# JiLiBIT/LIO-SLAM

Hardware: AMD Instinct MI355X
Metric: scan-to-map registrations/sec, 64x1800 scan vs 200-keyframe map; pose RMSE (higher is better)
Workload: dtype f32

## Files before the change

### include/liogpu.h

```cpp
#ifndef LIOGPU_H
#define LIOGPU_H

#include <stddef.h>
#include <stdint.h>

#ifdef __cplusplus
extern "C" {
#endif

#define LIO_VERSION 102
#define LIO_MAX_ITERS 32

enum {
    LIO_OK               = 0,
    LIO_TOO_FEW_POINTS   = 1,
    LIO_TOO_FEW_CORR     = 2,
    LIO_ERR_ARG          = -1,
    LIO_ERR_HIP          = -2,
    LIO_ERR_CAPACITY     = -3,
    LIO_ERR_NO_MAP       = -4,
    LIO_ERR_NO_DEVICE    = -5
};

typedef struct lio_s2m_config {
    int32_t k;
    float   max_sq_dist;
    double  plane_tol;
    double  weight;
    double  min_s;
    int32_t min_corr;
    int32_t max_iters;
    float   eig_thresh;
    double  conv_deg;
    double  conv_cm;
    int32_t min_scan_pts;
    int32_t jacobian_mode;
    int32_t force_all_iters;
    int32_t device_id;
    float   cell_size;
    int32_t max_batch;
    int32_t max_scan_pts;
    int32_t record_corr_iter;
    int32_t kernel_variant;
    int32_t profile;
    int32_t lookahead;
    int32_t use_lds;
    int32_t sort_scan;
    int32_t cell_div;
    int32_t xcd_remap;
    float   tile_size;
    int32_t use_graph;
    int32_t graph_iters;
    int32_t sort_batch;
    int32_t nn_cache;
    int32_t pipeline;
    int32_t n_devices;
    int32_t device_ids[8];
    int32_t x_sub;
    int32_t tight_rows;
} lio_s2m_config;

typedef struct lio_s2m_result {
    int32_t status;
    int32_t iters;
    int32_t converged;
    int32_t is_degenerate;
    int32_t n_corr_last;
    int32_t n_corr_iter[LIO_MAX_ITERS];
    float   matP[36];
    float   AtA[36];
    float   AtB[6];
    float   pose_iter[LIO_MAX_ITERS][6];
} lio_s2m_result;

typedef struct lio_s2m_profile {
    float   map_build_ms;
    float   map_upload_ms;
    int32_t n_launches;
    int32_t n_units;
    int32_t unit_iters;
    float   launch_ms[LIO_MAX_ITERS];
    int32_t launch_active[LIO_MAX_ITERS];
    int64_t point_iters;
    int64_t n_map;
    int64_t n_cells;
    int32_t pipeline;
    int32_t multi_iterations;
    int32_t multi_stream_syncs;
    int32_t multi_event_waits;
    int32_t multi_exchange;
    int32_t persist_fallbacks;
    int32_t map_x_sub;
    int32_t map_tight_tables;
    int32_t map_first_try;
    float   map_pts_per_cell;
} lio_s2m_profile;

typedef struct lio_s2m_handle lio_s2m_handle;

int  lio_version(void);
void lio_s2m_default_config(lio_s2m_config *cfg);
const char *lio_last_error(void);

int  lio_s2m_create(const lio_s2m_config *cfg, lio_s2m_handle **out);
void lio_s2m_destroy(lio_s2m_handle *h);

int  lio_s2m_set_map(lio_s2m_handle *h, const void *pts, size_t n, size_t stride_bytes);

int  lio_s2m_register(lio_s2m_handle *h, const void *scan, size_t n, size_t stride_bytes,
                      float pose[6], lio_s2m_result *res);

int  lio_s2m_batch_upload(lio_s2m_handle *h, int32_t n_scans, const void *const *scans,
                          const size_t *n_pts, size_t stride_bytes);
int  lio_s2m_batch_set_poses(lio_s2m_handle *h, const float *poses );
int  lio_s2m_batch_run(lio_s2m_handle *h);
int  lio_s2m_batch_sync(lio_s2m_handle *h);
int  lio_s2m_batch_results(lio_s2m_handle *h, float *poses ,
                           lio_s2m_result *results );

int   lio_s2m_share_map(lio_s2m_handle *h, lio_s2m_handle *map_owner);
int   lio_s2m_batch_upload_async(lio_s2m_handle *h, int32_t n_scans, const void *const *scans,
                                 const size_t *n_pts, size_t stride_bytes);
void *lio_host_alloc(size_t bytes);
void  lio_host_free(void *p);
int   lio_host_register(void *p, size_t bytes);
int   lio_host_unregister(void *p);
void *lio_device_alloc(int32_t device_id, size_t bytes);
void  lio_device_free(int32_t device_id, void *p);
int   lio_device_upload(int32_t device_id, void *dst, const void *src, size_t bytes);

int  lio_s2m_set_degeneracy(lio_s2m_handle *h, int32_t scan, const float matP[36], int32_t is_degenerate);

int  lio_s2m_get_correspondences(lio_s2m_handle *h, int32_t scan, uint8_t *flag,
                                 float *coeff4, int32_t *nn_idx5);

int  lio_s2m_set_corner_map(lio_s2m_handle *h, const void *pts, size_t n, size_t stride_bytes);
int  lio_s2m_batch_upload_corners(lio_s2m_handle *h, int32_t n_scans, const void *const *scans,
                                  const size_t *n_pts, size_t stride_bytes);
int  lio_s2m_register_cs(lio_s2m_handle *h, const void *corner_scan, size_t n_corner,
                         const void *surf_scan, size_t n_surf, size_t stride_bytes,
                         float pose[6], lio_s2m_result *res);
int  lio_s2m_get_corner_correspondences(lio_s2m_handle *h, int32_t scan, uint8_t *flag,
                                        float *coeff4, int32_t *nn_idx5);

int  lio_s2m_get_profile(lio_s2m_handle *h, lio_s2m_profile *out);
int  lio_s2m_kernel_variant(const lio_s2m_handle *h);
int  lio_s2m_launch_forms(const lio_s2m_handle *h, int32_t *n_full, int32_t *n_looped);
int  lio_s2m_debug_persist_spin(lio_s2m_handle *h, int32_t spin_max, int32_t withhold_wg);

int  lio_debug_plane_fit(int32_t device_id, const float *sets, size_t n, double plane_tol, uint32_t *out);
int  lio_debug_fast_f32_ops(int32_t device_id, int32_t op, int32_t raw, const uint32_t *patterns, uint64_t first, uint64_t count,
                            uint32_t *values, uint64_t *n_diff, uint32_t *first_diff, int32_t *n_first);
float lio_debug_threshold_f32(double t);
int  lio_s2m_debug_stamps(lio_s2m_handle *h, long long *out, size_t cap_entries);

int  lio_s2m_set_stream(lio_s2m_handle *h, void *hip_stream);
int  lio_s2m_set_global_grid(lio_s2m_handle *h, const float origin[3], const int32_t dims[3]);
int  lio_s2m_set_shard(lio_s2m_handle *h, int32_t axis, int32_t lo, int32_t hi);
int  lio_s2m_set_shard_plan(lio_s2m_handle *h, int32_t axis, int32_t n_ranks, int32_t rank, const int32_t *bounds,
                            int32_t halo_cells);
int  lio_s2m_set_scan_shard(lio_s2m_handle *h, int32_t rank, int32_t world);
int  lio_s2m_batch_begin(lio_s2m_handle *h);
int  lio_s2m_batch_iter_partial(lio_s2m_handle *h, double *d_sums );
int  lio_s2m_batch_iter_apply(lio_s2m_handle *h, const double *d_sums);
int  lio_s2m_batch_n_active(lio_s2m_handle *h, int32_t *n_active);
int  lio_s2m_batch_poll_active(lio_s2m_handle *h, int32_t iteration, int32_t *n_active);

void lio_transform_update(float pose[6], int32_t imu_available, int32_t imu_type,
                          float imu_roll_init, float imu_pitch_init, float imu_rpy_weight,
                          float rotation_tollerance, float z_tollerance);

typedef struct lio_deskew_config {
    int32_t N_SCAN;
    int32_t downsampleRate;
    int32_t point_filter_num;
    float   lidarMinFront, lidarMinBack, lidarMinLeft, lidarMinRight;
    float   lidarMaxRange;
    float   lidarMaxIntensity;
    int32_t deskew_flag;
    int32_t device_id;
} lio_deskew_config;

void lio_deskew_default_config(lio_deskew_config *cfg);

int  lio_imu_deskew_info(const double *stamp, const double *gyro_x, const double *gyro_y,
                         const double *gyro_z, int32_t n_imu,
                         double time_scan_cur, double time_scan_end,
                         double *imuTime, double *imuRotX, double *imuRotY, double *imuRotZ);

int  lio_deskew(const lio_deskew_config *cfg, const void *pts, size_t n, size_t stride_bytes,
                double time_scan_cur,
                const double *imuTime, const double *imuRotX, const double *imuRotY,
                const double *imuRotZ, int32_t imuPointerCur,
                void *out, size_t out_stride_bytes, size_t *n_out);

enum { LIO_PC2_UINT8 = 2, LIO_PC2_UINT16 = 4, LIO_PC2_INT32 = 5 };
enum { LIO_PC2_TIME_F32_SECONDS = 0,
       LIO_PC2_TIME_U32_NS      = 1,
       LIO_PC2_TIME_U32_RAW     = 2,
       LIO_PC2_TIME_F64_STAMP   = 3 };
typedef struct lio_pc2_layout {
    uint32_t point_step;
    uint32_t off_x;
    int32_t  off_intensity;
    int32_t  off_ring;
    int32_t  ring_type;
    int32_t  off_time;
    int32_t  time_type;
    int32_t  pin_host;
} lio_pc2_layout;

int  lio_s2m_register_pc2(lio_s2m_handle *h, const void *data, size_t n_points, const lio_pc2_layout *layout,
                          float pose[6], lio_s2m_result *res);
int  lio_s2m_register_raw(lio_s2m_handle *h, const void *data, size_t n_points, const lio_pc2_layout *layout, float leaf,
                          float pose[6], lio_s2m_result *res, void *ds_out, size_t ds_out_stride, size_t *n_ds);
int  lio_deskew_pc2(const lio_deskew_config *cfg, const void *data, size_t n_points, const lio_pc2_layout *layout,
                    double time_scan_cur,
                    const double *imuTime, const double *imuRotX, const double *imuRotY,
                    const double *imuRotZ, int32_t imuPointerCur,
                    void *out, size_t out_stride_bytes, size_t *n_out);

typedef struct lio_range_image_config {
    int32_t N_SCAN, Horizon_SCAN, downsampleRate;
    float   lidarMinRange, lidarMaxRange;
    int32_t deskew_flag;
    int32_t device_id;
} lio_range_image_config;
void lio_range_image_default_config(lio_range_image_config *cfg);
int  lio_range_image(const lio_range_image_config *cfg, const void *pts, size_t n, size_t stride_bytes,
                     double time_scan_cur,
                     const double *imuTime, const double *imuRotX, const double *imuRotY,
                     const double *imuRotZ, int32_t imuPointerCur,
                     void *out, size_t out_stride_bytes, size_t *n_out,
                     int32_t *startRingIndex, int32_t *endRingIndex,
                     int32_t *pointColInd, float *pointRange);

int  lio_curvature(int32_t device_id, const float *range, size_t n, float *curvature,
                   int32_t *neighbor_picked, int32_t *label);

typedef struct lio_feature_config {
    int32_t N_SCAN;
    float   edgeThreshold;
    float   surfThreshold;
    float   surfLeafSize;
    int32_t device_id;
} lio_feature_config;
void lio_feature_default_config(lio_feature_config *cfg);
int  lio_extract_features(const lio_feature_config *cfg, const void *cloud, size_t n, size_t stride_bytes,
                          const int32_t *startRingIndex, const int32_t *endRingIndex,
                          const int32_t *pointColInd, const float *pointRange,
                          void *corner_out, size_t *n_corner, void *surface_out, size_t *n_surface,
                          size_t out_stride_bytes, float *curvature, int32_t *neighbor_picked, int32_t *label);

int  lio_voxel_grid(int32_t device_id, const void *pts, size_t n, size_t stride_bytes, float leaf,
                    void *out, size_t out_stride_bytes, size_t *n_out);

int  lio_assemble_map(lio_s2m_handle *h, int32_t device_id, int32_t n_keyframes, const void *const *clouds,
                      const size_t *n_pts, size_t stride_bytes, const float *poses, float leaf,
                      void *out, size_t out_stride_bytes, size_t *n_out);

typedef struct lio_kf_store lio_kf_store;
int  lio_kf_store_create(int32_t device_id, lio_kf_store **out);
void lio_kf_store_destroy(lio_kf_store *s);
int  lio_kf_store_add(lio_kf_store *s, const void *cloud, size_t n, size_t stride_bytes, int32_t *id_out);
int  lio_kf_store_count(const lio_kf_store *s);
size_t lio_kf_store_points(const lio_kf_store *s, int32_t id);
int  lio_kf_store_add_device(lio_kf_store *s, const void *d_cloud, size_t n, size_t stride_bytes, int32_t *id_out);
int  lio_kf_store_add_from_handle(lio_kf_store *s, lio_s2m_handle *h, int32_t scan, int32_t *id_out);
int  lio_assemble_map_resident(lio_s2m_handle *h, lio_kf_store *s, int32_t n_selected, const int32_t *ids,
                               const float *poses, float leaf, void *out, size_t out_stride_bytes, size_t *n_out);

typedef struct lio_nearby_config {
    float  search_radius;
    float  pose_density;
    double recent_window_s;
} lio_nearby_config;
void lio_nearby_default_config(lio_nearby_config *cfg);

int  lio_kf_store_set_poses(lio_kf_store *s, int32_t first, int32_t n, const float *poses, const double *times);

int  lio_assemble_map_nearby(lio_s2m_handle *h, lio_kf_store *s, const lio_nearby_config *cfg, double time_cur, float leaf,
                             int32_t *ids_out, int32_t ids_cap, int32_t *n_ids, void *out, size_t out_stride_bytes,
                             size_t out_cap, size_t *n_out);

#define LIO_ICP_MAX_ITERS 1000
enum {
    LIO_ICP_NOT_CONVERGED      = 0,
    LIO_ICP_ITERATIONS         = 1,
    LIO_ICP_TRANSFORM          = 2,
    LIO_ICP_ABS_MSE            = 3,
    LIO_ICP_REL_MSE            = 4,
    LIO_ICP_NO_CORRESPONDENCES = 5
};
typedef struct lio_icp_config {
    double  max_corr_dist;
    double  transform_eps;
    double  fitness_eps;
    double  rel_mse_eps;
    double  rotation_threshold;
    double  fitness_max;
// ... 262 lines not shown
```

### lio-slam_amd/api.py

```python
import ctypes as C
import os
import subprocess

import numpy as np

_HERE = os.path.dirname(os.path.abspath(__file__))
LIO_MAX_ITERS = 32
STATUS_NAMES = {0: "OK", 1: "TOO_FEW_POINTS", 2: "TOO_FEW_CORR", -1: "ERR_ARG", -2: "ERR_HIP",
                -3: "ERR_CAPACITY", -4: "ERR_NO_MAP", -5: "ERR_NO_DEVICE"}


class LioError(RuntimeError):
    pass


class S2MConfig(C.Structure):
    _fields_ = [
        ("k", C.c_int32), ("max_sq_dist", C.c_float),
        ("plane_tol", C.c_double), ("weight", C.c_double), ("min_s", C.c_double),
        ("min_corr", C.c_int32), ("max_iters", C.c_int32), ("eig_thresh", C.c_float),
        ("conv_deg", C.c_double), ("conv_cm", C.c_double),
        ("min_scan_pts", C.c_int32), ("jacobian_mode", C.c_int32), ("force_all_iters", C.c_int32),
        ("device_id", C.c_int32), ("cell_size", C.c_float), ("max_batch", C.c_int32),
        ("max_scan_pts", C.c_int32), ("record_corr_iter", C.c_int32), ("kernel_variant", C.c_int32),
# ... 70 lines not shown

class IcpResult(C.Structure):
    _fields_ = [("status", C.c_int32), ("converged", C.c_int32), ("state", C.c_int32), ("iters", C.c_int32),
                ("n_corr_last", C.c_int32), ("accepted", C.c_int32), ("n_source", C.c_int32), ("n_target", C.c_int32),
                ("n_launches", C.c_int32), ("pad", C.c_int32), ("fitness", C.c_double), ("T", C.c_float * 16),
                ("pose_corrected", C.c_float * 6)]


class IcpClouds(C.Structure):
    _fields_ = [("source", C.c_void_p), ("target", C.c_void_p), ("closed", C.c_void_p),
                ("cap_source", C.c_size_t), ("cap_target", C.c_size_t), ("cap_closed", C.c_size_t),
                ("n_source", C.c_size_t), ("n_target", C.c_size_t), ("n_closed", C.c_size_t), ("stride", C.c_size_t)]


SC_MAX_CANDIDATES = 16


class ScConfig(C.Structure):
    _fields_ = [("max_radius", C.c_double), ("lidar_height", C.c_double), ("search_ratio", C.c_double), ("dist_thres", C.c_double),
                ("num_rings", C.c_int32), ("num_sectors", C.c_int32), ("num_exclude_recent", C.c_int32),
                ("num_candidates", C.c_int32), ("tree_period", C.c_int32), ("pad", C.c_int32)]


class ScResult(C.Structure):
    _fields_ = [("status", C.c_int32), ("loop_id", C.c_int32), ("align", C.c_int32), ("nn_idx", C.c_int32),
                ("n_searched", C.c_int32), ("n_candidates", C.c_int32), ("yaw_diff_rad", C.c_float), ("pad", C.c_int32),
                ("min_dist", C.c_double), ("cand_idx", C.c_int32 * SC_MAX_CANDIDATES), ("cand_ring_d2", C.c_float * SC_MAX_CANDIDATES),
                ("cand_dist", C.c_double * SC_MAX_CANDIDATES), ("cand_align", C.c_int32 * SC_MAX_CANDIDATES)]


class LocalMapConfig(C.Structure):
    _fields_ = [("n_keyframes", C.c_int32), ("front", C.c_float), ("left", C.c_float), ("back", C.c_float), ("right", C.c_float),
                ("remove_outliers", C.c_int32), ("mean_k", C.c_int32), ("stddev_mul", C.c_float), ("downsample", C.c_int32),
                ("leaf", C.c_float)]


class LocalMapInfo(C.Structure):
    _fields_ = [("first_keyframe", C.c_int32), ("n_keyframes", C.c_int32), ("n_summed", C.c_int32), ("n_cropped", C.c_int32),
                ("n_inliers", C.c_int32), ("n_out", C.c_int32), ("voxel_passthrough", C.c_int32), ("pad", C.c_int32),
                ("sor_mean", C.c_double), ("sor_stddev", C.c_double), ("sor_threshold", C.c_double)]


class HeightMapConfig(C.Structure):
    _fields_ = [("roll", C.c_float), ("pitch", C.c_float), ("level_and_ego_filter", C.c_int32), ("remove_outliers", C.c_int32),
                ("mean_k", C.c_int32), ("stddev_mul", C.c_float), ("downsample", C.c_int32), ("voxel", C.c_float * 3),
                ("resolution", C.c_double), ("min_points_per_cell", C.c_int32), ("max_points_per_cell", C.c_int32),
                ("use_cluster", C.c_int32), ("cluster_tolerance", C.c_float), ("cluster_min_points", C.c_int32),
                ("cluster_max_points", C.c_int32), ("use_max_height", C.c_int32), ("fill_holes", C.c_int32)]


class HeightMapInfo(C.Structure):
    _fields_ = [("rows", C.c_int32), ("cols", C.c_int32), ("length", C.c_double * 2), ("position", C.c_double * 2),
                ("n_in", C.c_int32), ("n_inliers", C.c_int32), ("n_filtered", C.c_int32), ("n_binned", C.c_int32),
                ("n_valid_cells", C.c_int32), ("n_filled_cells", C.c_int32), ("voxel_passthrough", C.c_int32), ("pad", C.c_int32)]


TERRAIN_LAYERS = ("smooth", "normal_x", "normal_y", "normal_z", "slope", "roughness", "edges", "traversability")


class TerrainConfig(C.Structure):
    _fields_ = [("normal_method", C.c_int32), ("normal_axis", C.c_int32), ("normal_radius", C.c_double), ("smooth_radius", C.c_double),
                ("edge_window_size", C.c_int32), ("edge_window_length", C.c_double), ("slope_critical", C.c_float),
                ("roughness_critical", C.c_float), ("slope_weight", C.c_float), ("roughness_weight", C.c_float), ("layers", C.c_uint32)]


class TerrainInfo(C.Structure):
    _fields_ = [("rows", C.c_int32), ("cols", C.c_int32), ("n_valid_cells", C.c_int32), ("normal_method_used", C.c_int32),
                ("n_normal_cells", C.c_int32), ("n_few_points", C.c_int32), ("n_degenerate", C.c_int32), ("edge_window_size", C.c_int32)]


class GlobalMapConfig(C.Structure):
    _fields_ = [("search_radius", C.c_float), ("pose_density", C.c_float), ("leaf", C.c_float)]


class GlobalMapInfo(C.Structure):
    _fields_ = [("n_keyframes", C.c_int32), ("n_summed", C.c_int32), ("n_out", C.c_int32), ("voxel_passthrough", C.c_int32)]


class ExportConfig(C.Structure):
    _fields_ = [("resolution", C.c_float), ("chunk_points", C.c_int32)]


class OgmConfig(C.Structure):
    _fields_ = [("z_min", C.c_float), ("z_max", C.c_float), ("z_negative", C.c_int32), ("remove_outliers", C.c_int32),
                ("radius", C.c_float), ("min_neighbors", C.c_int32), ("resolution", C.c_double), ("whole_box", C.c_int32)]


class OgmInfo(C.Structure):
    _fields_ = [("width", C.c_int32), ("height", C.c_int32), ("origin", C.c_double * 2), ("n_in", C.c_int32), ("n_slice", C.c_int32),
                ("n_inliers", C.c_int32), ("n_binned", C.c_int32), ("n_occupied", C.c_int32), ("pad", C.c_int32)]


class SdfConfig(C.Structure):
    _fields_ = [("min_height", C.c_double), ("max_height", C.c_double), ("nan_policy", C.c_int32), ("pad", C.c_int32)]


class SdfInfo(C.Structure):
    _fields_ = [("rows", C.c_int32), ("cols", C.c_int32), ("layers", C.c_int32), ("n_nan", C.c_int32), ("origin", C.c_double * 3),
                ("resolution", C.c_double), ("layer_min", C.c_float), ("layer_max", C.c_float), ("n_all_obstacle", C.c_int32),
                ("n_all_free", C.c_int32), ("n_mixed", C.c_int32), ("pad", C.c_int32)]


SDF_NODE_LIMIT = 1 << 25
STAGED_DS, STAGED_RAW = 0, 1

ICP_STATES = {0: "NOT_CONVERGED", 1: "ITERATIONS", 2: "TRANSFORM", 3: "ABS_MSE", 4: "REL_MSE", 5: "NO_CORRESPONDENCES"}


def lib_path():
    return os.environ.get("LIOGPU_LIB") or os.path.join(_HERE, "libliogpu.so")


def build_library(verbose=False):
    out = subprocess.run(["make", "-j8", "-C", os.path.join(_HERE, "csrc")], capture_output=True, text=True)
    if out.returncode != 0:
        raise LioError("building libliogpu.so failed:\n" + out.stdout + out.stderr)
    if verbose:
        print(out.stdout)
    return lib_path()


_LIB = None

EXPORTS = [
    "lio_version", "lio_s2m_default_config", "lio_last_error", "lio_s2m_create", "lio_s2m_destroy",
    "lio_s2m_set_map", "lio_s2m_register", "lio_s2m_batch_upload", "lio_s2m_batch_set_poses",
    "lio_s2m_batch_run", "lio_s2m_batch_sync", "lio_s2m_batch_results", "lio_s2m_set_degeneracy",
    "lio_s2m_get_correspondences", "lio_s2m_get_profile", "lio_s2m_set_stream",
    "lio_s2m_set_global_grid", "lio_s2m_set_shard", "lio_s2m_batch_begin",
    "lio_s2m_batch_iter_partial", "lio_s2m_batch_iter_apply", "lio_s2m_batch_n_active",
    "lio_transform_update", "lio_deskew_default_config", "lio_imu_deskew_info", "lio_deskew",
    "lio_curvature", "lio_s2m_debug_stamps", "lio_s2m_batch_poll_active", "lio_voxel_grid", "lio_assemble_map", "lio_kf_store_create", "lio_kf_store_destroy", "lio_kf_store_add",
    "lio_kf_store_count", "lio_kf_store_points", "lio_assemble_map_resident", "lio_s2m_set_scan_shard",
    "lio_s2m_set_corner_map", "lio_s2m_batch_upload_corners", "lio_s2m_register_cs",
    "lio_s2m_get_corner_correspondences", "lio_feature_default_config", "lio_extract_features",
    "lio_range_image_default_config", "lio_range_image",
    "lio_s2m_share_map", "lio_s2m_batch_upload_async", "lio_host_alloc", "lio_host_free", "lio_host_register",
    "lio_host_unregister", "lio_s2m_set_shard_plan", "lio_s2m_register_pc2", "lio_deskew_pc2", "lio_kf_store_add_device", "lio_kf_store_add_from_handle",
    "lio_s2m_register_raw", "lio_s2m_debug_persist_spin", "lio_device_alloc", "lio_device_free", "lio_device_upload",
    "lio_nearby_default_config", "lio_kf_store_set_poses", "lio_assemble_map_nearby", "lio_debug_plane_fit",
    "lio_icp_default_config", "lio_icp_align", "lio_kf_store_loop_icp", "lio_kf_store_detect_loop", "lio_icp_debug_trace",
    "lio_sc_default_config", "lio_sc_make", "lio_sc_distance", "lio_kf_store_sc_add", "lio_kf_store_sc_add_device",
    "lio_kf_store_sc_add_from_handle", "lio_kf_store_sc_count", "lio_kf_store_sc_geometry", "lio_kf_store_sc_get", "lio_kf_store_sc_detect",
    "lio_sor_filter", "lio_local_map_default_config", "lio_kf_store_local_map",
    "lio_height_map_default_config", "lio_height_map", "lio_kf_store_height_map",
    "lio_terrain_default_config", "lio_terrain_layers", "lio_kf_store_terrain_map",
    "lio_global_map_default_config", "lio_kf_store_global_map", "lio_kf_store_export_map", "lio_kf_store_get_keyframe",
    "lio_s2m_registered_cloud",
    "lio_radius_filter", "lio_ogm_default_config", "lio_occupancy_grid", "lio_kf_store_occupancy_grid", "lio_ogm_debug_stage_ms",
    "lio_s2m_kernel_variant", "lio_s2m_launch_forms",
    "lio_sdf_default_config", "lio_sdf_create", "lio_sdf_destroy", "lio_sdf_build", "lio_kf_store_sdf", "lio_sdf_nodes", "lio_sdf_query",
    "lio_occupancy_sdf", "lio_sdf_debug_stage_ms", "lio_sdf_memory",
    "lio_debug_fast_f32_ops", "lio_debug_threshold_f32",
]


def load_library():
    global _LIB
    if _LIB is not None:
        return _LIB
    p = lib_path()
    if not os.path.exists(p):
        raise LioError(f"{p} is missing: run __graft_entry__.build() (hipcc --offload-arch=gfx950). "
                       "There is no CPU fallback.")
    L = C.CDLL(p)
    vp, i32, f32, f64, sz = C.c_void_p, C.c_int32, C.c_float, C.c_double, C.c_size_t
    L.lio_version.restype = C.c_int
    L.lio_last_error.restype = C.c_char_p
    L.lio_s2m_default_config.argtypes = [C.POINTER(S2MConfig)]
    L.lio_s2m_default_config.restype = None
    L.lio_s2m_create.argtypes = [C.POINTER(S2MConfig), C.POINTER(vp)]
    L.lio_s2m_destroy.argtypes = [vp]
    L.lio_s2m_destroy.restype = None
    L.lio_s2m_set_map.argtypes = [vp, vp, sz, sz]
    L.lio_s2m_register.argtypes = [vp, vp, sz, sz, C.POINTER(f32), C.POINTER(S2MResult)]
    L.lio_s2m_register_pc2.argtypes = [vp, vp, sz, C.POINTER(PC2Layout), C.POINTER(f32), C.POINTER(S2MResult)]
    L.lio_s2m_register_raw.argtypes = [vp, vp, sz, C.POINTER(PC2Layout), f32, C.POINTER(f32), C.POINTER(S2MResult), vp, sz, C.POINTER(sz)]
    L.lio_s2m_debug_persist_spin.argtypes = [vp, i32, i32]
    L.lio_s2m_batch_upload.argtypes = [vp, i32, C.POINTER(vp), C.POINTER(sz), sz]
    L.lio_s2m_batch_upload_async.argtypes = [vp, i32, C.POINTER(vp), C.POINTER(sz), sz]
    L.lio_s2m_share_map.argtypes = [vp, vp]
    L.lio_host_alloc.argtypes = [sz]
    L.lio_host_alloc.restype = vp
    L.lio_host_free.argtypes = [vp]
    L.lio_host_free.restype = None
    L.lio_device_alloc.argtypes = [i32, sz]
    L.lio_device_alloc.restype = vp
    L.lio_device_free.argtypes = [i32, vp]
    L.lio_device_free.restype = None
    L.lio_device_upload.argtypes = [i32, vp, vp, sz]
    L.lio_host_register.argtypes = [vp, sz]
    L.lio_host_unregister.argtypes = [vp]
    L.lio_s2m_batch_set_poses.argtypes = [vp, C.POINTER(f32)]
    L.lio_s2m_batch_run.argtypes = [vp]
    L.lio_s2m_batch_sync.argtypes = [vp]
    L.lio_s2m_batch_results.argtypes = [vp, C.POINTER(f32), C.POINTER(S2MResult)]
    L.lio_s2m_set_degeneracy.argtypes = [vp, i32, C.POINTER(f32), i32]
    L.lio_s2m_get_correspondences.argtypes = [vp, i32, vp, vp, vp]
    L.lio_s2m_get_profile.argtypes = [vp, C.POINTER(S2MProfile)]
    L.lio_s2m_kernel_variant.argtypes = [vp]
    if hasattr(L, "lio_s2m_launch_forms"):
        L.lio_s2m_launch_forms.argtypes = [vp, C.POINTER(i32), C.POINTER(i32)]
    L.lio_s2m_set_corner_map.argtypes = [vp, vp, sz, sz]
    L.lio_s2m_batch_upload_corners.argtypes = [vp, i32, C.POINTER(vp), C.POINTER(sz), sz]
    L.lio_s2m_register_cs.argtypes = [vp, vp, sz, vp, sz, sz, C.POINTER(f32), C.POINTER(S2MResult)]
    L.lio_s2m_get_corner_correspondences.argtypes = [vp, i32, vp, vp, vp]
    L.lio_s2m_set_stream.argtypes = [vp, vp]
    L.lio_s2m_set_global_grid.argtypes = [vp, C.POINTER(f32), C.POINTER(i32)]
    L.lio_s2m_set_shard.argtypes = [vp, i32, i32, i32]
    L.lio_s2m_set_scan_shard.argtypes = [vp, i32, i32]
    L.lio_s2m_set_shard_plan.argtypes = [vp, i32, i32, i32, C.POINTER(i32), i32]
    L.lio_s2m_batch_begin.argtypes = [vp]
    L.lio_s2m_batch_iter_partial.argtypes = [vp, vp]
    L.lio_s2m_batch_iter_apply.argtypes = [vp, vp]
    L.lio_s2m_batch_n_active.argtypes = [vp, C.POINTER(i32)]
    L.lio_s2m_batch_poll_active.argtypes = [vp, i32, C.POINTER(i32)]
    L.lio_transform_update.argtypes = [C.POINTER(f32), i32, i32, f32, f32, f32, f32, f32]
    L.lio_transform_update.restype = None
    L.lio_deskew_default_config.argtypes = [C.POINTER(DeskewConfig)]
    L.lio_deskew_default_config.restype = None
    dp = C.POINTER(f64)
    L.lio_imu_deskew_info.argtypes = [dp, dp, dp, dp, i32, f64, f64, dp, dp, dp, dp]
    L.lio_deskew.argtypes = [C.POINTER(DeskewConfig), vp, sz, sz, f64, dp, dp, dp, dp, i32, vp, sz,
                             C.POINTER(sz)]
    L.lio_deskew_pc2.argtypes = [C.POINTER(DeskewConfig), vp, sz, C.POINTER(PC2Layout), f64, dp, dp, dp, dp, i32, vp, sz,
                                 C.POINTER(sz)]
    L.lio_curvature.argtypes = [i32, vp, sz, vp, vp, vp]
    L.lio_range_image_default_config.argtypes = [C.POINTER(RangeImageConfig)]
    L.lio_range_image_default_config.restype = None
    L.lio_range_image.argtypes = [C.POINTER(RangeImageConfig), vp, sz, sz, f64, dp, dp, dp, dp, i32, vp, sz, C.POINTER(sz),
                                  vp, vp, vp, vp]
    L.lio_feature_default_config.argtypes = [C.POINTER(FeatureConfig)]
    L.lio_feature_default_config.restype = None
    L.lio_extract_features.argtypes = [C.POINTER(FeatureConfig), vp, sz, sz, vp, vp, vp, vp, vp, C.POINTER(sz), vp,
                                       C.POINTER(sz), sz, vp, vp, vp]
    L.lio_s2m_debug_stamps.argtypes = [vp, vp, sz]
    L.lio_voxel_grid.argtypes = [i32, vp, sz, sz, f32, vp, sz, C.POINTER(sz)]
    L.lio_kf_store_create.argtypes = [i32, C.POINTER(vp)]
    L.lio_kf_store_destroy.argtypes = [vp]
    L.lio_kf_store_destroy.restype = None
    L.lio_kf_store_add.argtypes = [vp, vp, sz, sz, C.POINTER(i32)]
    L.lio_kf_store_count.argtypes = [vp]
    L.lio_kf_store_points.argtypes = [vp, C.c_int32]
    L.lio_kf_store_points.restype = C.c_size_t
    L.lio_kf_store_add_device.argtypes = [vp, vp, sz, sz, C.POINTER(i32)]
    L.lio_kf_store_add_from_handle.argtypes = [vp, vp, i32, C.POINTER(i32)]
    L.lio_assemble_map_resident.argtypes = [vp, vp, i32, C.POINTER(i32), C.POINTER(f32), f32, vp, sz, C.POINTER(sz)]
    L.lio_assemble_map.argtypes = [vp, i32, i32, C.POINTER(vp), C.POINTER(sz), sz, C.POINTER(f32), f32, vp, sz,
                                   C.POINTER(sz)]
    L.lio_nearby_default_config.argtypes = [C.POINTER(NearbyConfig)]
    L.lio_nearby_default_config.restype = None
    L.lio_kf_store_set_poses.argtypes = [vp, i32, i32, C.POINTER(f32), C.POINTER(f64)]
    L.lio_assemble_map_nearby.argtypes = [vp, vp, C.POINTER(NearbyConfig), f64, f32, C.POINTER(i32), i32, C.POINTER(i32), vp, sz, sz,
                                          C.POINTER(sz)]
    L.lio_icp_default_config.argtypes = [C.POINTER(IcpConfig)]
    L.lio_icp_default_config.restype = None
    L.lio_icp_align.argtypes = [i32, vp, sz, sz, vp, sz, sz, C.POINTER(IcpConfig), C.POINTER(f32), C.POINTER(IcpResult)]
    L.lio_kf_store_loop_icp.argtypes = [vp, i32, i32, i32, i32, f32, C.POINTER(IcpConfig), C.POINTER(IcpResult), C.POINTER(IcpClouds)]
    L.lio_kf_store_detect_loop.argtypes = [vp, f32, f64, f64, C.POINTER(i32), C.POINTER(i32)]
    L.lio_icp_debug_trace.argtypes = [i32, vp, sz, sz, vp, sz, sz, C.POINTER(IcpConfig), C.POINTER(f32), i32, C.POINTER(IcpResult),
                                      vp, vp, vp, vp, C.POINTER(i32)]
    scp = C.POINTER(ScConfig)
    L.lio_sc_default_config.argtypes = [scp]
    L.lio_sc_default_config.restype = None
    L.lio_sc_make.argtypes = [i32, vp, sz, sz, scp, vp, vp, vp]
    L.lio_sc_distance.argtypes = [i32, vp, vp, scp, C.POINTER(f64), C.POINTER(i32)]
    L.lio_kf_store_sc_add.argtypes = [vp, vp, sz, sz, scp, C.POINTER(i32)]
    L.lio_kf_store_sc_add_device.argtypes = [vp, vp, sz, sz, scp, C.POINTER(i32)]
    L.lio_kf_store_sc_add_from_handle.argtypes = [vp, vp, scp, C.POINTER(i32)]
    L.lio_kf_store_sc_count.argtypes = [vp]
    L.lio_kf_store_sc_geometry.argtypes = [vp, C.POINTER(i32), C.POINTER(i32)]
    L.lio_kf_store_sc_get.argtypes = [vp, i32, vp, vp, vp]
    L.lio_kf_store_sc_detect.argtypes = [vp, scp, C.POINTER(ScResult)]
    L.lio_sor_filter.argtypes = [i32, vp, sz, sz, i32, f32, vp, sz, C.POINTER(sz), vp, C.POINTER(f64)]
    L.lio_local_map_default_config.argtypes = [C.POINTER(LocalMapConfig)]
    L.lio_local_map_default_config.restype = None
    L.lio_kf_store_local_map.argtypes = [vp, C.POINTER(LocalMapConfig), C.POINTER(f32), vp, sz, sz, C.POINTER(sz), C.POINTER(LocalMapInfo)]
    L.lio_height_map_default_config.argtypes = [C.POINTER(HeightMapConfig)]
    L.lio_height_map_default_config.restype = None
    L.lio_height_map.argtypes = [i32, vp, sz, sz, C.POINTER(HeightMapConfig), vp, sz, C.POINTER(HeightMapInfo)]
    L.lio_kf_store_height_map.argtypes = [vp, C.POINTER(LocalMapConfig), C.POINTER(f32), C.POINTER(HeightMapConfig), vp, sz,
                                          C.POINTER(LocalMapInfo), C.POINTER(HeightMapInfo)]
    L.lio_terrain_default_config.argtypes = [C.POINTER(TerrainConfig)]
    L.lio_terrain_default_config.restype = None
    L.lio_terrain_layers.argtypes = [i32, vp, i32, i32, f64, C.POINTER(f64), C.POINTER(f64), C.POINTER(TerrainConfig), vp, sz,
                                     C.POINTER(TerrainInfo)]
    L.lio_kf_store_terrain_map.argtypes = [vp, C.POINTER(LocalMapConfig), C.POINTER(f32), C.POINTER(HeightMapConfig), C.POINTER(TerrainConfig),
                                           vp, sz, vp, sz, C.POINTER(LocalMapInfo), C.POINTER(HeightMapInfo), C.POINTER(TerrainInfo)]
    L.lio_global_map_default_config.argtypes = [C.POINTER(GlobalMapConfig)]
    L.lio_global_map_default_config.restype = None
    L.lio_kf_store_global_map.argtypes = [vp, C.POINTER(GlobalMapConfig), C.POINTER(i32), i32, C.POINTER(i32), vp, sz, sz, C.POINTER(sz),
                                          C.POINTER(GlobalMapInfo)]
    L.lio_kf_store_export_map.argtypes = [vp, C.POINTER(ExportConfig), vp, sz, sz, C.POINTER(sz), vp, sz, sz, C.POINTER(sz), C.POINTER(i32)]
    L.lio_kf_store_get_keyframe.argtypes = [vp, i32, C.POINTER(f32), vp, sz, sz, C.POINTER(sz)]
    L.lio_s2m_registered_cloud.argtypes = [vp, i32, C.POINTER(f32), vp, sz, sz, C.POINTER(sz)]
    L.lio_radius_filter.argtypes = [i32, vp, sz, sz, f32, i32, vp, sz, C.POINTER(sz), vp]
    L.lio_ogm_default_config.argtypes = [C.POINTER(OgmConfig)]
    L.lio_ogm_default_config.restype = None
    L.lio_occupancy_grid.argtypes = [i32, vp, sz, sz, C.POINTER(OgmConfig), vp, sz, C.POINTER(OgmInfo)]
    L.lio_kf_store_occupancy_grid.argtypes = [vp, f32, C.POINTER(OgmConfig), vp, sz, C.POINTER(sz), C.POINTER(OgmInfo)]
    L.lio_ogm_debug_stage_ms.argtypes = [i32, C.POINTER(f32)]
    L.lio_sdf_default_config.argtypes = [C.POINTER(SdfConfig)]
    L.lio_sdf_default_config.restype = None
    L.lio_sdf_create.argtypes = [i32, C.POINTER(vp)]
    L.lio_sdf_destroy.argtypes = [vp]
    L.lio_sdf_destroy.restype = None
    L.lio_sdf_build.argtypes = [vp, vp, i32, i32, f64, C.POINTER(f64), C.POINTER(f64), C.POINTER(SdfConfig), C.POINTER(SdfInfo)]
    L.lio_kf_store_sdf.argtypes = [vp, C.POINTER(LocalMapConfig), C.POINTER(f32), C.POINTER(HeightMapConfig), C.POINTER(SdfConfig), vp, sz, vp,
                                   C.POINTER(LocalMapInfo), C.POINTER(HeightMapInfo), C.POINTER(SdfInfo)]
    L.lio_sdf_nodes.argtypes = [vp, vp, sz]
    L.lio_sdf_query.argtypes = [vp, vp, sz, vp, vp]
    L.lio_occupancy_sdf.argtypes = [i32, vp, i32, i32, f32, i32, vp]
    L.lio_sdf_debug_stage_ms.argtypes = [i32, C.POINTER(f32)]
    L.lio_sdf_memory.argtypes = [vp, C.POINTER(sz), C.POINTER(sz)]
    _LIB = L
    return L


def _check(rc, what):
    if rc < 0:
        msg = load_library().lio_last_error()
        raise LioError(f"{what} failed: {STATUS_NAMES.get(rc, rc)}: {msg.decode() if msg else ''}")
    return rc


def _f32p(a):
    return a.ctypes.data_as(C.POINTER(C.c_float))


def _as_points(a):
    a = np.ascontiguousarray(a, np.float32)
    if a.ndim != 2 or a.shape[1] < 3:
        raise ValueError("points must be [n, >=3] float32")
    return a, a.shape[1] * 4


class ScanToMap:

    def __init__(self, **cfg_overrides):
        self.lib = load_library()
        self.cfg = S2MConfig()
        self.lib.lio_s2m_default_config(C.byref(self.cfg))
        for k, v in cfg_overrides.items():
            if not hasattr(self.cfg, k):
                raise AttributeError(k)
            if k == "device_ids":
                for i, d in enumerate(v):
                    self.cfg.device_ids[i] = int(d)
                continue
            setattr(self.cfg, k, v)
        self.h = C.c_void_p()
        _check(self.lib.lio_s2m_create(C.byref(self.cfg), C.byref(self.h)), "lio_s2m_create")
        self._n_scans = 0
        self._npts = []

# ... 11 lines not shown
    def set_map(self, map_pts):
        a, stride = _as_points(map_pts)
        _check(self.lib.lio_s2m_set_map(self.h, a.ctypes.data, len(a), stride), "lio_s2m_set_map")

    def scan2MapOptimization(self, scan_pts, pose):
        a, stride = _as_points(scan_pts)
        p = np.array(pose, np.float32).copy()
        res = S2MResult()
        rc = _check(self.lib.lio_s2m_register(self.h, a.ctypes.data, len(a), stride, _f32p(p), C.byref(res)),
                    "lio_s2m_register")
        self._n_scans, self._npts = 1, [len(a)]
        return p, res, rc

    def scan2MapOptimizationPC2(self, blob, n_points, layout, pose):
        b = np.ascontiguousarray(blob).view(np.uint8).reshape(-1)
        p = np.array(pose, np.float32).copy()
        res = S2MResult()
        rc = _check(self.lib.lio_s2m_register_pc2(self.h, b.ctypes.data, n_points, C.byref(layout), _f32p(p), C.byref(res)),
                    "lio_s2m_register_pc2")
        self._n_scans, self._npts = 1, [n_points]
        return p, res, rc

    def downsampleAndScan2MapOptimization(self, blob, n_points, layout, leaf, pose, want_ds=False, device_ptr=None):
        p = np.array(pose, np.float32).copy()
        res = S2MResult()
        if device_ptr is None:
            b = np.ascontiguousarray(blob).view(np.uint8).reshape(-1)
            ptr = b.ctypes.data
        else:
            ptr = int(device_ptr)
        out = np.zeros((n_points, 8), np.float32) if want_ds else None
        n_ds = C.c_size_t(0)
        rc = _check(self.lib.lio_s2m_register_raw(self.h, ptr, n_points, C.byref(layout), float(leaf), _f32p(p), C.byref(res),
                                                  out.ctypes.data if want_ds else None, 32, C.byref(n_ds)), "lio_s2m_register_raw")
        self._n_scans, self._npts = 1, [int(n_ds.value)]
        if want_ds:
            o = out[:n_ds.value]
            return p, res, rc, np.concatenate([o[:, :3], o[:, 4:5]], 1)
        return p, res, rc, int(n_ds.value)

    def registered_cloud(self, which, pose):
        p = np.ascontiguousarray(pose, np.float32).reshape(6)
        n = C.c_size_t()
        _check(self.lib.lio_s2m_registered_cloud(self.h, which, _f32p(p), None, 32, 0, C.byref(n)), "lio_s2m_registered_cloud")
        out = np.zeros((max(n.value, 1), 8), np.float32)
        _check(self.lib.lio_s2m_registered_cloud(self.h, which, _f32p(p), out.ctypes.data, 32, len(out), C.byref(n)),
               "lio_s2m_registered_cloud")
        return _from_records(out, n.value)

    def batch_upload(self, scans):
        arrs = [_as_points(s) for s in scans]
        strides = {s for _, s in arrs}
        if len(strides) != 1:
            raise ValueError("all scans of a batch must share one stride")
        n = len(arrs)
        ptrs = (C.c_void_p * n)(*[a.ctypes.data for a, _ in arrs])
        npts = (C.c_size_t * n)(*[len(a) for a, _ in arrs])
        _check(self.lib.lio_s2m_batch_upload(self.h, n, ptrs, npts, strides.pop()), "lio_s2m_batch_upload")
        self._n_scans, self._npts = n, [len(a) for a, _ in arrs]

    def share_map(self, owner):
        _check(self.lib.lio_s2m_share_map(self.h, owner.h if owner is not None else None), "lio_s2m_share_map")
        self._map_owner = owner

    def batch_upload_raw(self, base_ptr, n_pts, stride, asynchronous=True):
        n = len(n_pts)
        offs = np.concatenate([[0], np.cumsum(np.asarray(n_pts, np.int64) * stride)])
        ptrs = (C.c_void_p * n)(*[int(base_ptr) + int(o) for o in offs[:-1]])
        npts = (C.c_size_t * n)(*[int(v) for v in n_pts])
        fn = self.lib.lio_s2m_batch_upload_async if asynchronous else self.lib.lio_s2m_batch_upload
        _check(fn(self.h, n, ptrs, npts, stride), "lio_s2m_batch_upload(_async)")
        self._n_scans, self._npts = n, [int(v) for v in n_pts]

    def batch_set_poses(self, poses):
        p = np.ascontiguousarray(poses, np.float32).reshape(self._n_scans, 6)
        _check(self.lib.lio_s2m_batch_set_poses(self.h, _f32p(p)), "lio_s2m_batch_set_poses")

    def batch_run(self):
        _check(self.lib.lio_s2m_batch_run(self.h), "lio_s2m_batch_run")

    def batch_sync(self):
        _check(self.lib.lio_s2m_batch_sync(self.h), "lio_s2m_batch_sync")

    def batch_results(self, with_results=True):
        poses = np.zeros((self._n_scans, 6), np.float32)
        res = (S2MResult * self._n_scans)() if with_results else None
        _check(self.lib.lio_s2m_batch_results(self.h, _f32p(poses), res), "lio_s2m_batch_results")
        return poses, res

    def set_degeneracy(self, scan, matP, is_degenerate):
        m = np.ascontiguousarray(matP, np.float32).reshape(36)
        _check(self.lib.lio_s2m_set_degeneracy(self.h, scan, _f32p(m), int(is_degenerate)), "lio_s2m_set_degeneracy")

    def get_correspondences(self, scan=0):
        n = self._npts[scan]
        flag = np.zeros(n, np.uint8)
        coeff = np.zeros((n, 4), np.float32)
        nn = np.full((n, 5), -1, np.int32)
        _check(self.lib.lio_s2m_get_correspondences(self.h, scan, flag.ctypes.data, coeff.ctypes.data,
                                                    nn.ctypes.data), "lio_s2m_get_correspondences")
        return flag, coeff, nn

    def set_corner_map(self, map_pts):
        a, stride = _as_points(np.asarray(map_pts, np.float32).reshape(-1, 3) if len(map_pts) == 0 else map_pts)
        _check(self.lib.lio_s2m_set_corner_map(self.h, a.ctypes.data, len(a), stride), "lio_s2m_set_corner_map")

    def batch_upload_corners(self, scans):
        arrs = [_as_points(np.zeros((0, 3), np.float32) if len(s) == 0 else s) for s in scans]
        n = len(arrs)
        stride = {s for a, s in arrs if len(a)} or {12}
        if len(stride) != 1:
            raise ValueError("all scans of a batch must share one stride")
        ptrs = (C.c_void_p * n)(*[a.ctypes.data if len(a) else None for a, _ in arrs])
        npts = (C.c_size_t * n)(*[len(a) for a, _ in arrs])
        _check(self.lib.lio_s2m_batch_upload_corners(self.h, n, ptrs, npts, stride.pop()), "lio_s2m_batch_upload_corners")
        self._ncorner = [len(a) for a, _ in arrs]

    def scan2MapOptimizationCS(self, corner_pts, surf_pts, pose):
        cpts, cstride = _as_points(corner_pts)
        a, stride = _as_points(surf_pts)
        if cstride != stride:
            raise ValueError("corner and surf clouds must share one stride")
        p = np.array(pose, np.float32).copy()
        res = S2MResult()
        rc = _check(self.lib.lio_s2m_register_cs(self.h, cpts.ctypes.data, len(cpts), a.ctypes.data, len(a), stride,
                                                 _f32p(p), C.byref(res)), "lio_s2m_register_cs")
        self._n_scans, self._npts, self._ncorner = 1, [len(a)], [len(cpts)]
        return p, res, rc

    def get_corner_correspondences(self, scan=0):
        n = self._ncorner[scan]
        flag = np.zeros(n, np.uint8)
        coeff = np.zeros((n, 4), np.float32)
        nn = np.full((n, 5), -1, np.int32)
        _check(self.lib.lio_s2m_get_corner_correspondences(self.h, scan, flag.ctypes.data, coeff.ctypes.data,
                                                           nn.ctypes.data), "lio_s2m_get_corner_correspondences")
        return flag, coeff, nn

    def profile(self):
        p = S2MProfile()
        _check(self.lib.lio_s2m_get_profile(self.h, C.byref(p)), "lio_s2m_get_profile")
        return p

    def kernel_variant(self):
        v = self.lib.lio_s2m_kernel_variant(self.h)
        _check(min(v, 0), "lio_s2m_kernel_variant")
        return bool(v & 1), v >> 8

    def launch_forms(self):
        full, looped = C.c_int32(0), C.c_int32(0)
        _check(self.lib.lio_s2m_launch_forms(self.h, C.byref(full), C.byref(looped)), "lio_s2m_launch_forms")
        return full.value, looped.value

    def debug_persist_spin(self, spin_max=0, withhold_wg=-1):
        _check(self.lib.lio_s2m_debug_persist_spin(self.h, int(spin_max), int(withhold_wg)), "lio_s2m_debug_persist_spin")

    def debug_stamps(self):
        nb = self.lib.lio_s2m_debug_stamps(self.h, None, 0)
        out = np.zeros((max(nb, 0), 4, 8), np.int64)
        if nb > 0:
            self.lib.lio_s2m_debug_stamps(self.h, out.ctypes.data, out.size)
        return out

    def set_stream(self, hip_stream):
        _check(self.lib.lio_s2m_set_stream(self.h, C.c_void_p(hip_stream)), "lio_s2m_set_stream")

    def set_global_grid(self, origin, dims):
        o = (C.c_float * 3)(*origin)
        d = (C.c_int32 * 3)(*dims)
        _check(self.lib.lio_s2m_set_global_grid(self.h, o, d), "lio_s2m_set_global_grid")

    def set_shard(self, axis, lo, hi):
        _check(self.lib.lio_s2m_set_shard(self.h, axis, lo, hi), "lio_s2m_set_shard")

    def set_shard_plan(self, axis, rank, bounds, halo_cells):
        b = (C.c_int32 * len(bounds))(*[int(v) for v in bounds])
        _check(self.lib.lio_s2m_set_shard_plan(self.h, axis, len(bounds) - 1, rank, b, halo_cells), "lio_s2m_set_shard_plan")

    def set_scan_shard(self, rank, world):
        _check(self.lib.lio_s2m_set_scan_shard(self.h, rank, world), "lio_s2m_set_scan_shard")

    def batch_begin(self):
        _check(self.lib.lio_s2m_batch_begin(self.h), "lio_s2m_batch_begin")

    def batch_iter_partial(self, d_sums_ptr):
        _check(self.lib.lio_s2m_batch_iter_partial(self.h, C.c_void_p(d_sums_ptr)), "lio_s2m_batch_iter_partial")

    def batch_iter_apply(self, d_sums_ptr):
        _check(self.lib.lio_s2m_batch_iter_apply(self.h, C.c_void_p(d_sums_ptr)), "lio_s2m_batch_iter_apply")

    def batch_poll_active(self, iteration):
        v = C.c_int32()
        _check(self.lib.lio_s2m_batch_poll_active(self.h, iteration, C.byref(v)), "lio_s2m_batch_poll_active")
        return v.value

    def batch_n_active(self):
        v = C.c_int32()
        _check(self.lib.lio_s2m_batch_n_active(self.h, C.byref(v)), "lio_s2m_batch_n_active")
        return v.value


class DeviceBuffer:

    def __init__(self, array, device_id=0):
        self.lib = load_library()
        self.device_id = int(device_id)
        a = np.ascontiguousarray(array)
        self.nbytes = a.nbytes
        self.ptr = self.lib.lio_device_alloc(self.device_id, self.nbytes)
        if not self.ptr:
            raise LioError("lio_device_alloc failed")
        _check(self.lib.lio_device_upload(self.device_id, self.ptr, a.ctypes.data, self.nbytes), "lio_device_upload")

    def close(self):
        if getattr(self, "ptr", None):
            self.lib.lio_device_free(self.device_id, self.ptr)
            self.ptr = None

    def __del__(self):
        try:
            self.close()
        except Exception:
            pass


class PinnedBuffer:

    def __init__(self, nbytes):
        self.lib = load_library()
        self.nbytes = int(nbytes)
        self.ptr = self.lib.lio_host_alloc(self.nbytes)
        if not self.ptr:
            raise LioError("lio_host_alloc failed")
        self.array = np.ctypeslib.as_array((C.c_uint8 * self.nbytes).from_address(self.ptr))

    def close(self):
        if getattr(self, "ptr", None):
            self.array = None
            self.lib.lio_host_free(self.ptr)
            self.ptr = None

    def __del__(self):
        try:
            self.close()
        except Exception:
            pass


def transform_update(pose, imu_available=0, imu_type=0, imu_roll_init=0.0, imu_pitch_init=0.0,
                     imu_rpy_weight=0.01, rotation_tollerance=1000.0, z_tollerance=1000.0):
    p = np.array(pose, np.float32).copy()
    load_library().lio_transform_update(_f32p(p), imu_available, imu_type, imu_roll_init, imu_pitch_init,
                                        imu_rpy_weight, rotation_tollerance, z_tollerance)
    return p


def imu_deskew_info(stamp, gyro, t_cur, t_end):
    stamp = np.ascontiguousarray(stamp, np.float64)
    g = np.ascontiguousarray(gyro, np.float64)
    gx, gy, gz = (np.ascontiguousarray(g[:, k]) for k in range(3))
    T, RX, RY, RZ = (np.zeros(2000) for _ in range(4))
    dp = lambda a: a.ctypes.data_as(C.POINTER(C.c_double))
    cur = load_library().lio_imu_deskew_info(dp(stamp), dp(gx), dp(gy), dp(gz), len(stamp), t_cur, t_end,
                                             dp(T), dp(RX), dp(RY), dp(RZ))
    return cur, T, RX, RY, RZ


_XYZIRT = np.dtype({"names": ["x", "y", "z", "intensity", "ring", "time"],
                    "formats": ["<f4", "<f4", "<f4", "<f4", "<u2", "<f4"],
                    "offsets": [0, 4, 8, 16, 20, 24], "itemsize": 32})


def pack_xyzirt(xyz, intensity, ring, time):
    rec = np.zeros(len(xyz), _XYZIRT)
    rec["x"], rec["y"], rec["z"] = xyz[:, 0], xyz[:, 1], xyz[:, 2]
    rec["intensity"], rec["ring"], rec["time"] = intensity, ring, time
    return rec


_SCRATCH = {}


def _scratch(name, shape, dtype=np.float32):
    need = int(np.prod(shape))
    buf = _SCRATCH.get((name, np.dtype(dtype).str))
    if buf is None or buf.size < need:
        buf = np.zeros(max(need, 1), dtype)
        _SCRATCH[(name, np.dtype(dtype).str)] = buf
    return buf[:need].reshape(shape)


def deskew(dcfg, records, t_cur, imu):
    cur, T, RX, RY, RZ = imu
    L = load_library()
    n = len(records)
    out = _scratch("deskew", (n, 8))
    n_out = C.c_size_t()
    dp = lambda a: a.ctypes.data_as(C.POINTER(C.c_double))
    rec = np.ascontiguousarray(records)
    _check(L.lio_deskew(C.byref(dcfg), rec.ctypes.data, n, rec.dtype.itemsize, t_cur,
                        dp(T), dp(RX), dp(RY), dp(RZ), cur, out.ctypes.data, 32, C.byref(n_out)), "lio_deskew")
    o = out[:n_out.value]
    return np.concatenate([o[:, :3], o[:, 4:5]], axis=1).copy()


def deskew_pc2(dcfg, blob, n_points, layout, t_cur, imu):
    cur, T, RX, RY, RZ = imu
    L = load_library()
    b = np.ascontiguousarray(blob).view(np.uint8).reshape(-1)
    out = _scratch("deskew", (max(n_points, 1), 8))
    n_out = C.c_size_t()
    dp = lambda a: a.ctypes.data_as(C.POINTER(C.c_double))
    _check(L.lio_deskew_pc2(C.byref(dcfg), b.ctypes.data, n_points, C.byref(layout), t_cur,
                            dp(T), dp(RX), dp(RY), dp(RZ), cur, out.ctypes.data, 32, C.byref(n_out)), "lio_deskew_pc2")
    o = out[:n_out.value]
    return np.concatenate([o[:, :3], o[:, 4:5]], axis=1).copy()


def deskew_default_config(**kw):
    c = DeskewConfig()
    load_library().lio_deskew_default_config(C.byref(c))
    for k, v in kw.items():
        setattr(c, k, v)
    return c


def curvature(rng, device_id=0):
    r = np.ascontiguousarray(rng, np.float32)
    curv = np.zeros(len(r), np.float32)
    picked = np.full(len(r), -1, np.int32)
    label = np.full(len(r), -1, np.int32)
    _check(load_library().lio_curvature(device_id, r.ctypes.data, len(r), curv.ctypes.data,
                                        picked.ctypes.data, label.ctypes.data), "lio_curvature")
    return curv, picked, label


def debug_plane_fit(sets, plane_tol=0.2, device_id=0):
    a = np.ascontiguousarray(sets, np.float32).reshape(-1, 15)
    out = np.zeros((len(a), 8), np.uint32)
    fn = load_library().lio_debug_plane_fit
    fn.argtypes = [C.c_int32, C.c_void_p, C.c_size_t, C.c_double, C.c_void_p]
    _check(fn(device_id, a.ctypes.data, len(a), float(plane_tol), out.ctypes.data), "lio_debug_plane_fit")
    return out


def debug_fast_f32_ops(op, raw=False, patterns=None, first=0, count=0, want_values=False, device_id=0):
    fn = load_library().lio_debug_fast_f32_ops
    fn.argtypes = [C.c_int32, C.c_int32, C.c_int32, C.c_void_p, C.c_uint64, C.c_uint64, C.c_void_p,
                   C.POINTER(C.c_uint64), C.c_void_p, C.POINTER(C.c_int32)]
    pat = None
    if patterns is not None:
        pat = np.ascontiguousarray(patterns, np.uint32)
        count = len(pat)
    vals = np.zeros(count, np.uint32) if want_values else None
    n_diff, n_first = C.c_uint64(0), C.c_int32(0)
    firsts = np.zeros(8, np.uint32)
    _check(fn(device_id, int(op), 1 if raw else 0, pat.ctypes.data if pat is not None else None, int(first), int(count),
              vals.ctypes.data if vals is not None else None, C.byref(n_diff), firsts.ctypes.data, C.byref(n_first)),
           "lio_debug_fast_f32_ops")
    return int(n_diff.value), firsts[:n_first.value].copy(), vals


def debug_threshold_f32(t):
    fn = load_library().lio_debug_threshold_f32
    fn.argtypes = [C.c_double]
    fn.restype = C.c_float
    return np.float32(fn(float(t)))


def range_image(records, t_cur, imu, device_id=0, **cfg_overrides):
    L = load_library()
    cfg = RangeImageConfig()
    L.lio_range_image_default_config(C.byref(cfg))
    cfg.device_id = device_id
    for k, v in cfg_overrides.items():
        if not hasattr(cfg, k):
            raise AttributeError(k)
        setattr(cfg, k, v)
    cur, T, RX, RY, RZ = imu
    rec = np.ascontiguousarray(records)
    cells = int(cfg.N_SCAN) * int(cfg.Horizon_SCAN)
    out = _scratch("ri_cloud", (max(cells, 1), 8))
    col = _scratch("ri_col", (max(cells, 1),), np.int32)
    rng = _scratch("ri_range", (max(cells, 1),))
    start = np.zeros(cfg.N_SCAN, np.int32)
    end = np.zeros(cfg.N_SCAN, np.int32)
    n_out = C.c_size_t()
    dpp = lambda a: a.ctypes.data_as(C.POINTER(C.c_double))
    _check(L.lio_range_image(C.byref(cfg), rec.ctypes.data, len(rec), rec.dtype.itemsize, t_cur, dpp(T), dpp(RX), dpp(RY), dpp(RZ),
                             cur, out.ctypes.data, 32, C.byref(n_out), start.ctypes.data, end.ctypes.data, col.ctypes.data,
                             rng.ctypes.data), "lio_range_image")
    n = n_out.value
    return {"cloud": _from_records(out, n), "start_ring": start, "end_ring": end, "col": col[:n].copy(), "range": rng[:n].copy()}


def extract_features(cloud_xyzi, start_ring, end_ring, point_col, point_range, device_id=0, **cfg_overrides):
    L = load_library()
    cfg = FeatureConfig()
    L.lio_feature_default_config(C.byref(cfg))
    cfg.N_SCAN = len(start_ring)
    cfg.device_id = device_id
    for k, v in cfg_overrides.items():
        if not hasattr(cfg, k):
            raise AttributeError(k)
        setattr(cfg, k, v)
    rec = _as_xyzi_records(np.asarray(cloud_xyzi, np.float32).reshape(-1, 4))
    n = len(rec)
    sr = np.ascontiguousarray(start_ring, np.int32)
    er = np.ascontiguousarray(end_ring, np.int32)
    col = np.ascontiguousarray(point_col, np.int32)
    rng = np.ascontiguousarray(point_range, np.float32)
    corner = _scratch("fe_corner", (120 * max(cfg.N_SCAN, 1), 8))
    surf = _scratch("fe_surf", (max(n, 1), 8))
    curv = np.zeros(max(n, 1), np.float32)
    picked = np.zeros(max(n, 1), np.int32)
    label = np.zeros(max(n, 1), np.int32)
    nc, ns = C.c_size_t(0), C.c_size_t(0)
    _check(L.lio_extract_features(C.byref(cfg), rec.ctypes.data, n, 32, sr.ctypes.data, er.ctypes.data,
                                  col.ctypes.data, rng.ctypes.data, corner.ctypes.data, C.byref(nc),
                                  surf.ctypes.data, C.byref(ns), 32, curv.ctypes.data, picked.ctypes.data,
                                  label.ctypes.data), "lio_extract_features")
    return {"corner": _from_records(corner, nc.value), "surface": _from_records(surf, ns.value),
            "curvature": curv[:n], "picked": picked[:n], "label": label[:n]}


def _as_xyzi_records(a):
    a = np.ascontiguousarray(a, np.float32)
    rec = np.zeros((len(a), 8), np.float32)
    rec[:, :3] = a[:, :3]
    rec[:, 3] = 1.0
    rec[:, 4] = a[:, 3]
    return rec


def _from_records(rec, n):
    return np.concatenate([rec[:n, :3], rec[:n, 4:5]], axis=1).copy()


def voxel_grid(xyzi, leaf, device_id=0):
    rec = _as_xyzi_records(xyzi)
    out = _scratch("voxel", rec.shape)
    n_out = C.c_size_t()
    rc = _check(load_library().lio_voxel_grid(device_id, rec.ctypes.data, len(rec), 32, leaf, out.ctypes.data, 32,
                                              C.byref(n_out)), "lio_voxel_grid")
    return _from_records(out, n_out.value), rc


def nearby_default_config(**overrides):
    cfg = NearbyConfig()
    load_library().lio_nearby_default_config(C.byref(cfg))
    for k, v in overrides.items():
        if not hasattr(cfg, k):
            raise AttributeError(k)
        setattr(cfg, k, v)
    return cfg


def icp_default_config(**overrides):
    cfg = IcpConfig()
    load_library().lio_icp_default_config(C.byref(cfg))
    for k, v in overrides.items():
        if not hasattr(cfg, k):
            raise AttributeError(k)
        setattr(cfg, k, v)
    return cfg


def _guess_ptr(guess):
    if guess is None:
        return None, None
    g = np.ascontiguousarray(guess, np.float32).reshape(16)
    return g, _f32p(g)


def icp_align(source, target, cfg=None, guess=None, device_id=0):
    src, ss = _as_points(source)
    tgt, ts = _as_points(target)
    cfg = cfg or icp_default_config()
    g, gp = _guess_ptr(guess)
    res = IcpResult()
    rc = _check(load_library().lio_icp_align(device_id, src.ctypes.data, len(src), ss, tgt.ctypes.data, len(tgt), ts, C.byref(cfg), gp,
                                             C.byref(res)), "lio_icp_align")
    return res, rc


def icp_debug_trace(source, target, cfg=None, guess=None, rec_iter=-1, device_id=0):
    src, ss = _as_points(source)
    tgt, ts = _as_points(target)
    cfg = cfg or icp_default_config()
    g, gp = _guess_ptr(guess)
    res = IcpResult()
    steps = np.zeros((cfg.max_iters, 16), np.float32)
    n_corr = np.zeros(cfg.max_iters, np.int32)
    mse = np.zeros(cfg.max_iters, np.float64)
    corr = np.full(max(len(src), 1), -1, np.int32)
    nt = C.c_int32()
    _check(load_library().lio_icp_debug_trace(device_id, src.ctypes.data, len(src), ss, tgt.ctypes.data, len(tgt), ts, C.byref(cfg), gp,
                                              rec_iter, C.byref(res), steps.ctypes.data, n_corr.ctypes.data, mse.ctypes.data,
                                              corr.ctypes.data, C.byref(nt)), "lio_icp_debug_trace")
    k = nt.value
    return res, steps[:k].reshape(k, 4, 4).copy(), n_corr[:k].copy(), mse[:k].copy(), corr[:len(src)].copy()


def sc_default_config(**overrides):
    cfg = ScConfig()
    load_library().lio_sc_default_config(C.byref(cfg))
    for k, v in overrides.items():
        if not hasattr(cfg, k):
            raise AttributeError(k)
        setattr(cfg, k, v)
    return cfg


def sc_make(cloud, cfg=None, device_id=0):
    pts, stride = _as_points(cloud)
    cfg = cfg or sc_default_config()
    R, S = max(cfg.num_rings, 1), max(cfg.num_sectors, 1)
    desc, rk, sk = np.zeros((R, S), np.float32), np.zeros(R, np.float32), np.zeros(S, np.float64)
    _check(load_library().lio_sc_make(device_id, pts.ctypes.data, len(pts), stride, C.byref(cfg), desc.ctypes.data, rk.ctypes.data,
                                      sk.ctypes.data), "lio_sc_make")
# ... 500 lines not shown
```

### lio-slam_amd/csrc/lio_handle.h

```cpp
#pragma once
#include <hip/hip_runtime.h>
#include <stdio.h>
#include <string.h>
#include <string>
#include <vector>

#include "../../include/liogpu.h"
#include "lio_kernels.h"
#include "lio_pool.h"
#include "lio_types.h"

int lio_pc2_check_xyz(const lio_pc2_layout* L);
void lio_raw_ws_free(struct LioRawWs* ws);

int lio_s2m_set_map_device_xyzi(lio_s2m_handle* h, const float4* d_xyzi, size_t n);
int lio_s2m_set_map_device_bbox(lio_s2m_handle* h, const float4* d_xyzi, size_t n, const float box[6]);
hipStream_t lio_s2m_stream_of(lio_s2m_handle* h);
bool lio_s2m_takes_device_map(const lio_s2m_handle* h);
int lio_s2m_staged_scan(lio_s2m_handle* h, int scan, const unsigned char** d_rec, size_t* n, size_t* stride, size_t* xyz_off, int* int_off,
                        int* device_id, hipStream_t* stream);

struct lio_s2m_handle {
    ~lio_s2m_handle();
    lio_s2m_config cfg;
    LioConsts c;
    hipStream_t stream = nullptr;
    bool own_stream = true;

    bool has_map = false;
    size_t n_map = 0;
    LioDevBuf<float> d_mx, d_my, d_mz;
    LioDevBuf<float4> d_map4, d_sorted, d_nbr_pts;
    LioDevBuf<int> d_cell_of, d_cell_count, d_cell_start, d_tile_sums, d_nbr_start;
    LioDevBuf<int> d_nbr_slot;
    LioDevBuf<unsigned> d_bbox;
    LioDevBuf<unsigned char> d_stage;
    LioDevBuf<unsigned char> d_map_stage;
    LioGrid grid{};

    int n_scans = 0;
    size_t total_pts = 0;
    LioDevBuf<float> d_sx, d_sy, d_sz;
    LioDevBuf<LioScanState> d_state;
    std::vector<LioScanState> h_state;
    std::vector<LioBlockDesc> v_blocks, v_prep;
    std::vector<LioScanTiles> v_tiles;
    std::vector<LioBlockDesc> v_blocks_sorted;
    std::vector<int> v_order, v_first, v_first_orig;
    bool defer_sync = false;
    bool async_upload = false;
    LioDevBuf<float> d_poses;
    const float* reg_pose = nullptr;
    bool pose_in_state = false;
    LioDevBuf<float> d_summary;
    LioPinned<float> h_summary;
    bool host_state_stale = false;
    LioDevBuf<LioBlockDesc> d_blocks;
    int n_blocks = 0, ppt = 1, max_blk = 1;
    LioDevBuf<double> d_partials;
    LioDevBuf<unsigned> d_arrive;
    bool poses_set = false, ran = false;
    LioDevBuf<LioScanTiles> d_tiles;
    LioDevBuf<LioBlockDesc> d_prep_blocks;
    LioDevBuf<int> d_key_of, d_key_count, d_key_start, d_key_tiles, d_tmp_idx, d_perm;
    LioDevBuf<float> d_block_box;
    bool has_block_box = false;
    LioDevBuf<unsigned char> d_blk_skip;
    LioDevBuf<int> d_big_list;
    LioDevBuf<unsigned> d_scan_bbox;
    LioPinned<unsigned> h_scan_bbox;
    bool sorted = false;
    const unsigned char* last_stage = nullptr;
    size_t last_stride = 0, last_xyz_off = 0;
    size_t xyz_off = 0;
    int int_off = -2;
    int last_int_off = -1;
    struct LioRawWs* raw_ws = nullptr;
    int persist_fallbacks = 0;
    bool no_persist = false;
    unsigned persist_spin_max = 0;
    int persist_withhold = -1;
    lio_s2m_handle* map_src = nullptr;
    unsigned long long map_epoch = 0;
    LioDevBuf<float> d_nn_cache;
    LioDevBuf<long long> d_stamps;
    LioDevBuf<unsigned> d_gen;
    LioDevBuf<double> d_spec_sums;
    unsigned gen_epoch = 0;
    int n_cu = 0;
    bool run_persist = false;
    bool soa_valid = true;
    hipGraph_t graph = nullptr;
    hipGraphExec_t graph_exec = nullptr;
    bool graph_dirty = true;
    int graph_chunk = 0, graph_blocks = 0, graph_ppt = 0;
    bool graph_plain = true;
    LioIterParams graph_params;
    int units_this_run = 0, unit_iters = 1;
    bool plain_kernel = true;
    int iterate_variant = 0;
    int tail_from = LIO_TAIL_FROM_DEFAULT;
    int tail_wgs = LIO_TAIL_WGS_DEFAULT;
    int graph_tail_from = -1, graph_tail_wgs = 0;
    int graph_n_full = 0, graph_n_looped = 0;
    int run_n_full = 0, run_n_looped = 0;

    LioDevBuf<unsigned char> d_rec_flag;
    LioDevBuf<float> d_rec_coeff;
    LioDevBuf<int> d_rec_nn;

    struct LioMulti* multi = nullptr;

    bool run_pending = false, run_graph = false, run_has_c = false;
    int run_next = 0, run_units = 0, run_look = 0;
    LioIterParams run_P, run_Pc;

    LioShard shard{};
    float gorigin[3] = {0, 0, 0};
    int gdims[3] = {0, 0, 0};
    bool has_global = false;
    int block_rank = 0, block_world = 1;
    int plan_ranks = 0, plan_rank = 0, plan_halo = 1, plan_bounds[9] = {0, 0, 0, 0, 0, 0, 0, 0, 0};

    lio_s2m_handle* corner = nullptr;
    bool corner_active = false;
    LioIterParams graph_params_c;
    int graph_blocks_c = 0;

    hipEvent_t ev_beg[LIO_MAX_ITERS] = {}, ev_end[LIO_MAX_ITERS] = {}, ev_chk[LIO_MAX_ITERS] = {};
    hipEvent_t ev_map[2] = {};
    hipEvent_t ev_mapl[2] = {};
    bool map_timing_pending = false;
    LioPinned<int> h_active;
    lio_s2m_profile prof{};
    int launches_this_run = 0;
    LioDevBuf<int> d_active;
};
```

### lio-slam_amd/csrc/lio_kernels.h

```cpp
#pragma once
#include <hip/hip_runtime.h>
#include "lio_types.h"

struct LioIterParams {
    LioGrid grid;
    LioShard shard;
    LioConsts c;
    const float4* map_sorted;
    const float4* map_xyz4;
    const int* cell_start;
    const float4* nbr_pts;
    const int* nbr_start;
    const float* sx;
    const float* sy;
    const float* sz;
    const int* perm;
    LioScanState* state;
    const LioBlockDesc* blocks;
    double* partials;
    unsigned* arrive;
    int max_blk;
    int xcd_remap;
    int* n_active;
    double* sums_out;
    unsigned char* rec_flag;
    float* rec_coeff;
    int* rec_nn;
    float* d5_cache;
    long long* stamps;
    const unsigned char* blk_skip;
};

void lio_launch_aos_to_soa(const void* src, size_t stride, int n, float* x, float* y, float* z,
                           float4* xyz4, hipStream_t s);
void lio_launch_map_bbox(const float* x, const float* y, const float* z, int n, unsigned* bbox, hipStream_t s);
void lio_launch_map_build(const LioGrid& g, const float* x, const float* y, const float* z, int n,
                          int* cell_of, int* cell_count, int* cell_start, int* tile_sums,
                          float4* sorted, int* nbr_start, float4* nbr_pts, int* nbr_slot, bool with_cell_sorted, hipStream_t s);
void lio_launch_map_cell_sort(const LioGrid& g, const float* x, const float* y, const float* z, int n, int* cell_of, int* cell_count,
                              int* cell_start, int* tile_sums, float4* sorted, hipStream_t s);
void lio_launch_map_occupancy(const LioGrid& g, const float* x, const float* y, const float* z, int n, int* flags, hipStream_t s);
int  lio_scan_tiles(int n_cells);
void lio_launch_init_state(LioScanState* st, int n_scans, float* poses, bool from_state, const LioConsts& c,
                           int* n_active, hipStream_t s);
int  lio_iterate_variant(const LioIterParams& P, int ppt, bool stage, bool corner, bool allow_plain);
int  lio_launch_iterate(const LioIterParams& P, int n_blocks, int ppt, bool stage, hipStream_t s, bool corner = false, bool allow_plain = true,
                         int tail_wgs = 0, bool* looped = nullptr);
#define LIO_TAIL_FROM_DEFAULT 7
#define LIO_TAIL_WGS_DEFAULT 1536
void lio_launch_iterate_tail(const LioIterParams& P, int n_blocks, int n_wgs, hipStream_t s);
void lio_launch_persist(const LioIterParams& P, int n_blocks, unsigned* gen, unsigned epoch, const unsigned char* stage, size_t stride,
                        int n_scans, unsigned* spec, double* spec_sums, const float* poses0, unsigned spin_max, int withhold_wg, hipStream_t s);
void lio_launch_pack_summary(const LioScanState* st, int n_scans, float* out, hipStream_t s);
void lio_launch_apply(LioScanState* st, int n_scans, const double* sums, size_t slot_stride, int n_slots, const LioConsts& c,
                      int* n_active, hipStream_t s);
void lio_launch_shard_cull(const LioIterParams& P, int n_ranks, int rank, int halo, const int* bounds, const float* block_box,
                           int n_blocks, unsigned char* skip, hipStream_t s);
void lio_launch_block_boxes(const LioBlockDesc* blocks, int n_blocks, const LioScanState* st, const float* sx, const float* sy,
                            const float* sz, float* box, hipStream_t s);
void lio_launch_scan_sort_lds(const void* stage, size_t stride, const LioScanState* st, int n_scans, int max_pts, float tile0,
                              int shard_axis, int* perm, float* x, float* y, float* z, hipStream_t s);
void lio_launch_scan_bbox(const void* stage, size_t stride, const LioBlockDesc* prep_blocks, int n_prep_blocks,
                          const LioScanState* st, unsigned* bbox, hipStream_t s);
void lio_launch_scan_tile_sort(const void* stage, size_t stride, int total_pts,
                               const LioBlockDesc* prep_blocks, int n_prep_blocks,
                               const LioScanState* st, const LioScanTiles* tiles, int n_keys,
                               int* key_of, int* key_count, int* key_start, int* tile_sums,
                               int* tmp_idx, int* perm, int* big_list, int* big_cnt,
                               float* x, float* y, float* z, hipStream_t s);
void lio_launch_exclusive_scan(const int* in, int n, int* tile_sums, int* out, hipStream_t s);
void lio_launch_xyzi4_to_soa(const float4* src, int n, float* x, float* y, float* z, float4* xyz4, hipStream_t s);
void lio_launch_debug_plane_fit(const float* sets, long long n, double plane_tol, unsigned* out, hipStream_t s);
void lio_launch_debug_fast_f32_ops(int op, int raw, const unsigned* pat, unsigned long long first, unsigned long long count,
                                   unsigned* val, unsigned long long* n_diff, unsigned* diff, hipStream_t s);
```

### lio-slam_amd/csrc/lio_kernels.hip

```cpp
#include <hip/hip_runtime.h>
#include <algorithm>
#include "lio_types.h"
#include "lio_device_math.h"
#include "lio_kernels.h"

#include "lio_s2m_device.h"
#include "lio_scan2.h"
#include "lio_wg.h"
#include "lio_s2m_block.h"

__global__ void k_aos_to_soa(const unsigned char* __restrict__ src, size_t stride, int n,
                             float* __restrict__ x, float* __restrict__ y, float* __restrict__ z,
                             float4* __restrict__ xyz4 )
{
    int i = blockIdx.x * blockDim.x + threadIdx.x;
    if (i >= n) return;
    const float* p = reinterpret_cast<const float*>(src + (size_t)i * stride);
    const float a = p[0], b = p[1], c = p[2];
    x[i] = a; y[i] = b; z[i] = c;
    if (xyz4) xyz4[i] = make_float4(a, b, c, 0.0f);
}

__global__ void k_xyzi4_to_soa(const float4* __restrict__ src, int n, float* __restrict__ x, float* __restrict__ y,
                               float* __restrict__ z, float4* __restrict__ xyz4)
// ... 668 lines not shown
}

__global__ void k_s2m_pack_summary(const LioScanState* __restrict__ st, int n_scans, float* __restrict__ out)
{
    const int s = blockIdx.x * blockDim.x + threadIdx.x;
    if (s >= n_scans) return;
    float* o = out + (size_t)s * 10;
    for (int k = 0; k < 6; ++k) o[k] = st[s].pose[k];
    o[6] = __int_as_float(st[s].iter); o[7] = __int_as_float(st[s].status | (st[s].done ? 0 : 0x100));
    o[8] = __int_as_float(st[s].converged); o[9] = __int_as_float(st[s].is_degenerate);
}

__global__ void k_s2m_apply(LioScanState* __restrict__ st, int n_scans, const double* __restrict__ sums, size_t slot_stride, int n_slots,
                            LioConsts c, int* __restrict__ n_active)
{
    const int s = blockIdx.x;
    if (s >= n_scans) return;
    if (st[s].done) return;
    __shared__ LioSolveWs s_ws;
    __shared__ double s_tot[LIO_SUMS];
    const int lane = (int)threadIdx.x;
    if (lane < LIO_SUMS) {
        const double* p = sums + (size_t)s * LIO_SUMS + lane;
        double v = p[0];
        for (int d = 1; d < n_slots; ++d) v += p[(size_t)d * slot_stride];
        s_tot[lane] = v;
    }
    asm volatile("s_waitcnt lgkmcnt(0)" ::: "memory");
    lio_gn_step(&st[s], s_tot, c, &s_ws, n_active, lane);
}

void lio_launch_aos_to_soa(const void* src, size_t stride, int n, float* x, float* y, float* z,
                           float4* xyz4, hipStream_t s)
{
    if (n <= 0) return;
    hipLaunchKernelGGL(k_aos_to_soa, dim3((n + 255) / 256), dim3(256), 0, s,
                       (const unsigned char*)src, stride, n, x, y, z, xyz4);
}

void lio_launch_map_bbox(const float* x, const float* y, const float* z, int n, unsigned* bbox, hipStream_t s)
{
    int blocks = (n + 1023) / 1024;
    if (blocks > 512) blocks = 512;
    if (blocks < 1) blocks = 1;
    hipLaunchKernelGGL(k_map_bbox, dim3(blocks), dim3(256), 0, s, x, y, z, n, bbox);
}

void lio_launch_exclusive_scan(const int* in, int n, int* tile_sums, int* out, hipStream_t s)
{
    const int n_tiles = (n + LIO_SCAN_TILE - 1) / LIO_SCAN_TILE;
    hipLaunchKernelGGL(k_scan_tile_sums, dim3(n_tiles), dim3(256), 0, s, in, n, tile_sums);
    hipLaunchKernelGGL(k_scan_tile_offsets, dim3(1), dim3(256), 0, s, tile_sums, n_tiles);
    hipLaunchKernelGGL(k_scan_apply, dim3(n_tiles), dim3(256), 0, s, in, n, tile_sums, out);
}

void lio_launch_map_occupancy(const LioGrid& g, const float* x, const float* y, const float* z, int n, int* flags, hipStream_t s)
{
    (void)hipMemsetAsync(flags, 0, sizeof(int) * ((size_t)g.n_cells + 1), s);
    hipLaunchKernelGGL(k_map_occupancy, dim3((n + 255) / 256), dim3(256), 0, s, g, x, y, z, n, flags);
}

static LioGrid lio_tight_grid(const LioGrid& g, int l)
{
    LioGrid b = g;
    b.oy = g.tb_oy[l]; b.oz = g.tb_oz[l]; b.inv_cell = g.tb_inv_cell[l]; b.ny = g.tb_ny[l]; b.nz = g.tb_nz[l]; b.k = 1;
    return b;
}

void lio_launch_map_build(const LioGrid& g, const float* x, const float* y, const float* z, int n,
                          int* cell_of, int* cell_count, int* cell_start, int* tile_sums,
                          float4* sorted, int* nbr_start, float4* nbr_pts, int* nbr_slot, bool with_cell_sorted, hipStream_t s)
{
    const int nb = (n + 255) / 256;
    const int repsA = (2 * g.k + 1) * (2 * g.k + 1), repsB = 9;
    int n_tb = 0;
    while (n_tb < LIO_TB_MAX && g.tb_reach[n_tb] > 0.0f) ++n_tb;
    const int lenA = g.n_cells * g.xs;
    int len_all = lenA, rows_all = g.ny * g.nz;
    for (int l = 0; l < n_tb; ++l) { len_all += g.tb_ny[l] * g.tb_nz[l] * g.nxf; rows_all += g.tb_ny[l] * g.tb_nz[l]; }
    const unsigned nbrA = (unsigned)(((long long)n * repsA + 255) / 256), nbrB = (unsigned)(((long long)n * repsB + 255) / 256);
    int* nbr_count = cell_count + g.n_cells;
    unsigned long long* tiles64 = reinterpret_cast<unsigned long long*>(tile_sums);
    if (with_cell_sorted) (void)hipMemsetAsync(cell_count, 0, sizeof(int) * ((size_t)g.n_cells + len_all), s);
    else (void)hipMemsetAsync(nbr_count, 0, sizeof(int) * (size_t)len_all, s);
    hipLaunchKernelGGL(k_map_cell_count, dim3(nb), dim3(256), 0, s, g, x, y, z, n, cell_of, with_cell_sorted ? cell_count : (int*)nullptr);
    hipLaunchKernelGGL(k_map_nbr_count, dim3(nbrA), dim3(256), 0, s, g, cell_of, x, y, z, n, nbr_count, nbr_slot);
    hipLaunchKernelGGL(k_map_nbr_pad_rows, dim3((g.ny * g.nz + 3) / 4), dim3(256), 0, s, g, nbr_count);
    for (int l = 0; l < n_tb; ++l) {
        const LioGrid gb = lio_tight_grid(g, l);
        hipLaunchKernelGGL(k_map_nbr_count, dim3(nbrB), dim3(256), 0, s, gb, cell_of, x, y, z, n, nbr_count + g.tb_row0[l],
                           nbr_slot + (size_t)n * (repsA + repsB * l));
        hipLaunchKernelGGL(k_map_nbr_pad_rows, dim3((gb.ny * gb.nz + 3) / 4), dim3(256), 0, s, gb, nbr_count + g.tb_row0[l]);
    }
    if (with_cell_sorted && g.xs == 1 && n_tb == 0) {
        lio_launch_scan2<false>(cell_count, nbr_count, g.n_cells, tiles64, cell_start, nbr_start, s);
    } else {
        if (with_cell_sorted) lio_launch_exclusive_scan(cell_count, g.n_cells, tile_sums, cell_start, s);
        lio_launch_exclusive_scan(nbr_count, len_all, tile_sums, nbr_start, s);
    }
    if (with_cell_sorted) {
        (void)hipMemsetAsync(cell_count, 0, sizeof(int) * (size_t)g.n_cells, s);
        hipLaunchKernelGGL(k_map_scatter, dim3(nb), dim3(256), 0, s, x, y, z, n, cell_of, cell_start, cell_count, sorted);
    }
    {
        const int n_rec4 = n * (repsA + repsB * n_tb) + LIO_ROW_ALIGN * rows_all + 2 * LIO_ROW_ALIGN;
        hipLaunchKernelGGL(k_map_nbr_fill, dim3((n_rec4 + 255) / 256), dim3(256), 0, s, nbr_pts, n_rec4);
    }
    hipLaunchKernelGGL(k_map_nbr_scatter, dim3(nbrA), dim3(256), 0, s, g, x, y, z, n, nbr_start, nbr_slot, nbr_pts);
    for (int l = 0; l < n_tb; ++l)
        hipLaunchKernelGGL(k_map_nbr_scatter, dim3(nbrB), dim3(256), 0, s, lio_tight_grid(g, l), x, y, z, n, nbr_start + g.tb_row0[l],
                           nbr_slot + (size_t)n * (repsA + repsB * l), nbr_pts);
}

void lio_launch_map_cell_sort(const LioGrid& g, const float* x, const float* y, const float* z, int n, int* cell_of, int* cell_count,
                              int* cell_start, int* tile_sums, float4* sorted, hipStream_t s)
{
    const int nb = (n + 255) / 256;
    (void)hipMemsetAsync(cell_count, 0, sizeof(int) * (size_t)g.n_cells, s);
    hipLaunchKernelGGL(k_map_cell_count, dim3(nb), dim3(256), 0, s, g, x, y, z, n, cell_of, cell_count);
    lio_launch_exclusive_scan(cell_count, g.n_cells, tile_sums, cell_start, s);
    (void)hipMemsetAsync(cell_count, 0, sizeof(int) * (size_t)g.n_cells, s);
    hipLaunchKernelGGL(k_map_scatter, dim3(nb), dim3(256), 0, s, x, y, z, n, cell_of, cell_start, cell_count, sorted);
}

int lio_scan_tiles(int n_cells) { return (n_cells + LIO_SCAN_TILE - 1) / LIO_SCAN_TILE; }

void lio_launch_init_state(LioScanState* st, int n_scans, float* poses, bool from_state, const LioConsts& c,
                           int* n_active, hipStream_t s)
{
    const int fs = from_state ? 1 : 0;
    if (n_scans <= 256) {
        hipLaunchKernelGGL(k_s2m_init_state<true>, dim3(1), dim3(n_scans <= 64 ? 64 : 256), 0, s, st, n_scans, poses, fs, c, n_active);
        return;
    }
    (void)hipMemsetAsync(n_active, 0, sizeof(int), s);
    hipLaunchKernelGGL(k_s2m_init_state<false>, dim3((n_scans + 63) / 64), dim3(64), 0, s, st, n_scans, poses, fs, c, n_active);
}

int lio_iterate_variant(const LioIterParams& P, int ppt, bool stage, bool corner, bool allow_plain)
{
    const bool plain = allow_plain && ppt == 1 && !stage && !corner && P.shard.axis < 0 && P.blk_skip == nullptr &&
                       P.sums_out == nullptr && P.rec_flag == nullptr && P.stamps == nullptr;
    if (plain) return 1 | (LIO_MIN_WAVES_PLAIN << 8);
    return ((ppt == 1 && !stage && !corner) ? LIO_MIN_WAVES : 4) << 8;
}

int lio_launch_iterate(const LioIterParams& P, int n_blocks, int ppt, bool stage, hipStream_t s, bool corner, bool allow_plain,
                       int tail_wgs, bool* looped)
{
    const int variant = lio_iterate_variant(P, ppt, stage, corner, allow_plain);
    if (looped) *looped = false;
    if (n_blocks <= 0) return variant;
    if ((variant & 1) && tail_wgs >= 8 && !corner && !stage) {
        const int n_wgs = std::min(tail_wgs & ~7, (n_blocks + 7) & ~7);
        lio_launch_iterate_tail(P, n_blocks, n_wgs, s);
        if (looped) *looped = true;
        return variant;
    }
    const dim3 gr(n_blocks), bl(LIO_BLOCK);
    if (corner) {
        hipLaunchKernelGGL((k_s2m_iterate<1, false, true, false>), gr, bl, 0, s, P);
        return variant;
    }
    if (stage) {
        switch (ppt) {
        case 1: hipLaunchKernelGGL((k_s2m_iterate<1, true, false, false>), gr, bl, 0, s, P); break;
        case 2: hipLaunchKernelGGL((k_s2m_iterate<2, true, false, false>), gr, bl, 0, s, P); break;
        default: hipLaunchKernelGGL((k_s2m_iterate<4, true, false, false>), gr, bl, 0, s, P); break;
        }
    } else if (variant & 1) {
        hipLaunchKernelGGL((k_s2m_iterate<1, false, false, true>), gr, bl, 0, s, P);
    } else {
        switch (ppt) {
        case 1: hipLaunchKernelGGL((k_s2m_iterate<1, false, false, false>), gr, bl, 0, s, P); break;
        case 2: hipLaunchKernelGGL((k_s2m_iterate<2, false, false, false>), gr, bl, 0, s, P); break;
        default: hipLaunchKernelGGL((k_s2m_iterate<4, false, false, false>), gr, bl, 0, s, P); break;
        }
    }
    return variant;
}

void lio_launch_pack_summary(const LioScanState* st, int n_scans, float* out, hipStream_t s)
{
    hipLaunchKernelGGL(k_s2m_pack_summary, dim3((n_scans + 255) / 256), dim3(256), 0, s, st, n_scans, out);
}

void lio_launch_apply(LioScanState* st, int n_scans, const double* sums, size_t slot_stride, int n_slots, const LioConsts& c,
                      int* n_active, hipStream_t s)
{
    hipLaunchKernelGGL(k_s2m_apply, dim3(n_scans), dim3(64), 0, s, st, n_scans, sums, slot_stride, n_slots, c, n_active);
}

void lio_launch_shard_cull(const LioIterParams& P, int n_ranks, int rank, int halo, const int* bounds, const float* block_box,
                           int n_blocks, unsigned char* skip, hipStream_t s)
{
    if (n_blocks <= 0) return;
    LioShardPlan plan;
    plan.n_ranks = n_ranks; plan.rank = rank; plan.halo = halo;
    for (int r = 0; r < 9; ++r) plan.bounds[r] = (n_ranks > 0 && r <= n_ranks) ? bounds[r] : 0;
    hipLaunchKernelGGL(k_shard_cull, dim3((n_blocks + 31) / 32), dim3(256), 0, s, P, plan, block_box, n_blocks, skip);
}

void lio_launch_block_boxes(const LioBlockDesc* blocks, int n_blocks, const LioScanState* st, const float* sx, const float* sy,
                            const float* sz, float* box, hipStream_t s)
{
    if (n_blocks <= 0) return;
    hipLaunchKernelGGL(k_block_boxes, dim3(n_blocks), dim3(LIO_BLOCK), 0, s, blocks, st, sx, sy, sz, box);
}

void lio_launch_scan_sort_lds(const void* stage, size_t stride, const LioScanState* st, int n_scans, int max_pts, float tile0,
                              int shard_axis, int* perm, float* x, float* y, float* z, hipStream_t s)
{
    if (n_scans <= 0) return;
    if (max_pts <= 16 * LIO_SORT_THREADS)
        hipLaunchKernelGGL(k_scan_sort_radix<16>, dim3(n_scans), dim3(LIO_SORT_THREADS), 0, s,
                           (const unsigned char*)stage, stride, st, tile0, shard_axis, perm, x, y, z);
    else
        hipLaunchKernelGGL(k_scan_sort_radix<32>, dim3(n_scans), dim3(LIO_SORT_THREADS), 0, s,
                           (const unsigned char*)stage, stride, st, tile0, shard_axis, perm, x, y, z);
}

void lio_launch_scan_bbox(const void* stage, size_t stride, const LioBlockDesc* prep_blocks, int n_prep_blocks,
                          const LioScanState* st, unsigned* bbox, hipStream_t s)
{
    if (n_prep_blocks <= 0) return;
    hipLaunchKernelGGL(k_scan_bbox, dim3(n_prep_blocks), dim3(256), 0, s, (const unsigned char*)stage, stride, prep_blocks, st, bbox);
}

void lio_launch_scan_tile_sort(const void* stage, size_t stride, int total_pts,
                               const LioBlockDesc* prep_blocks, int n_prep_blocks,
                               const LioScanState* st, const LioScanTiles* tiles, int n_keys,
                               int* key_of, int* key_count, int* key_start, int* tile_sums,
                               int* tmp_idx, int* perm, int* big_list, int* big_cnt,
                               float* x, float* y, float* z, hipStream_t s)
{
    if (total_pts <= 0 || n_prep_blocks <= 0) return;
    (void)hipMemsetAsync(key_count, 0, sizeof(int) * (size_t)n_keys, s);
    (void)hipMemsetAsync(big_cnt, 0, sizeof(int), s);
    hipLaunchKernelGGL(k_scan_tile_keys, dim3(n_prep_blocks), dim3(256), 0, s,
                       (const unsigned char*)stage, stride, prep_blocks, st, tiles, key_of, key_count);
    const int n_tiles = (n_keys + LIO_SCAN_TILE - 1) / LIO_SCAN_TILE;
    hipLaunchKernelGGL(k_scan_tile_sums, dim3(n_tiles), dim3(256), 0, s, key_count, n_keys, tile_sums);
    hipLaunchKernelGGL(k_scan_tile_offsets, dim3(1), dim3(256), 0, s, tile_sums, n_tiles);
    hipLaunchKernelGGL(k_scan_apply, dim3(n_tiles), dim3(256), 0, s, key_count, n_keys, tile_sums, key_start);
    (void)hipMemsetAsync(key_count, 0, sizeof(int) * (size_t)n_keys, s);
    const int nb = (total_pts + 255) / 256;
    hipLaunchKernelGGL(k_scan_tile_scatter, dim3(nb), dim3(256), 0, s, key_of, total_pts, key_start, key_count, tmp_idx);
    hipLaunchKernelGGL(k_scan_tile_ranksort, dim3(nb), dim3(256), 0, s, key_start, key_of, total_pts, tmp_idx, perm, big_list, big_cnt);
    hipLaunchKernelGGL(k_scan_tile_bigsort, dim3(64), dim3(256), 0, s, key_start, big_list, big_cnt, perm);
    hipLaunchKernelGGL(k_scan_gather_sorted, dim3(nb), dim3(256), 0, s, (const unsigned char*)stage, stride,
                       total_pts, perm, x, y, z);
}

void lio_launch_xyzi4_to_soa(const float4* src, int n, float* x, float* y, float* z, float4* xyz4, hipStream_t s)
{
    if (n <= 0) return;
    hipLaunchKernelGGL(k_xyzi4_to_soa, dim3((n + 255) / 256), dim3(256), 0, s, src, n, x, y, z, xyz4);
}
```

### lio-slam_amd/csrc/lio_multi.hip

```cpp
#include <hip/hip_runtime.h>
#include <math.h>
#include <stdlib.h>
#include <string.h>
#include <memory>
#include <vector>

#include "lio_handle.h"
#include "lio_multi.h"

#define LIO_MULTI_HALO 16

namespace {

struct LioPeerPtrs { double* p[8]; };

__global__ void k_multi_publish(const double* __restrict__ part, int n_val, LioPeerPtrs dst, int n_dev)
{
    const int i = blockIdx.x * blockDim.x + threadIdx.x;
    if (i >= n_val) return;
    const double v = part[i];
#pragma unroll 1
    for (int d = 0; d < n_dev; ++d) dst.p[d][i] = v;
}

}

static int lio_multi_reserve(lio_s2m_handle* h, size_t n_scans)
{
    LioMulti* m = h->multi;
    if (n_scans <= m->slot_scans) return LIO_OK;
    const size_t nd = m->dev.size();
    const size_t cap = n_scans + n_scans / 4 + 16, n_val = cap * LIO_SUMS;
    for (auto& ch : m->dev) {
        HIPCHK(hipSetDevice(ch->h->cfg.device_id));
        HIPCHK(hipStreamSynchronize(ch->h->stream));
        HIPCHK(ch->d_part.grow(n_val, 1.0, 0));
        HIPCHK(ch->d_gather.grow(2 * nd * n_val, 1.0, 0));
        HIPCHK(ch->d_tot.grow(n_val, 1.0, 0));
        if (m->exchange == 2) HIPCHK(ch->h_part.grow(n_val, n_val, hipHostMallocPortable));
    }
    if (m->exchange == 2) HIPCHK(m->h_tot.grow(n_val, n_val, hipHostMallocPortable));
    m->slot_scans = cap;
    return LIO_OK;
}

int lio_multi_create(const lio_s2m_config* cfg, lio_s2m_handle** out)
{
    int ndev = 0;
    if (hipGetDeviceCount(&ndev) != hipSuccess || ndev <= 0)
        return lio_fail(LIO_ERR_NO_DEVICE, "no HIP device visible (this library has no CPU fallback)");
    if (cfg->n_devices > 8) return lio_fail(LIO_ERR_ARG, "n_devices must be <= 8");
    for (int i = 0; i < cfg->n_devices; ++i)
        if (cfg->device_ids[i] < 0 || cfg->device_ids[i] >= ndev) return lio_fail(LIO_ERR_ARG, "device_ids entry out of range");
    if (cfg->use_lds || cfg->kernel_variant > 1)
        return lio_fail(LIO_ERR_ARG, "the multi-device mode runs the default kernel only");
    std::unique_ptr<lio_s2m_handle> f(new lio_s2m_handle());
    f->cfg = *cfg;
    f->shard.axis = -1;
    LioMulti* m = f->multi = new LioMulti();
    m->join_device = cfg->device_ids[0];
    const char* ex = getenv("LIO_MULTI_EXCHANGE");
    m->exchange = (ex && !strcmp(ex, "copy")) ? 1 : ((ex && !strcmp(ex, "host")) ? 2 : 0);
    for (int i = 0; i < cfg->n_devices; ++i) {
        lio_s2m_config cc = *cfg;
        cc.n_devices = 1;
        cc.device_id = cfg->device_ids[i];
        cc.use_graph = 0;
        cc.pipeline = 1;
        std::unique_ptr<LioMultiChild> ch(new LioMultiChild());
        const int rc = lio_s2m_create(&cc, &ch->h);
        if (rc != LIO_OK) return rc;
        m->dev.push_back(std::move(ch));
    }
    for (int a = 0; a < cfg->n_devices && m->exchange == 0; ++a)
        for (int b = 0; b < cfg->n_devices; ++b) {
            const int da = cfg->device_ids[a], db = cfg->device_ids[b];
            if (da == db) continue;
            int can = 0;
            if (hipDeviceCanAccessPeer(&can, da, db) != hipSuccess || !can) { m->peer_ok = false; continue; }
            if (hipSetDevice(da) != hipSuccess) { m->peer_ok = false; continue; }
            const hipError_t e = hipDeviceEnablePeerAccess(db, 0);
            if (e != hipSuccess && e != hipErrorPeerAccessAlreadyEnabled) m->peer_ok = false;
            (void)hipGetLastError();
        }
    if (!m->peer_ok && m->exchange == 0) m->exchange = 1;
    for (auto& ch : m->dev) {
        if (hipSetDevice(ch->h->cfg.device_id) != hipSuccess) return lio_fail(LIO_ERR_HIP, "hipSetDevice");
        for (hipEvent_t& e : ch->ev_pub)
            if (hipEventCreateWithFlags(&e, hipEventDisableTiming) != hipSuccess) return lio_fail(LIO_ERR_HIP, "hipEventCreate");
    }
    if (cfg->n_devices >= 4) {
        bool ok = hipSetDevice(m->join_device) == hipSuccess && hipStreamCreateWithFlags(&m->join_stream, hipStreamNonBlocking) == hipSuccess;
        for (int i = 0; i < LIO_MAX_ITERS && ok; ++i) ok = hipEventCreateWithFlags(&m->ev_all[i], hipEventDisableTiming) == hipSuccess;
        if (!ok) return lio_fail(LIO_ERR_HIP, "hipStreamCreate / hipEventCreate (join stream)");
    }
    *out = f.release();
    return LIO_OK;
}

void lio_multi_destroy(lio_s2m_handle* h)
{
    for (auto& ch : h->multi->dev) {
        (void)hipSetDevice(ch->h->cfg.device_id);
        (void)hipStreamSynchronize(ch->h->stream);
    }
    delete h;
}

LioMultiChild::~LioMultiChild()
{
    for (hipEvent_t e : ev_pub) if (e) (void)hipEventDestroy(e);
    lio_s2m_destroy(h);
}

LioMulti::~LioMulti()
{
    for (auto& ch : dev) {
        (void)hipSetDevice(ch->h->cfg.device_id);
        ch.reset();
    }
    if (!dev.empty()) (void)hipSetDevice(join_device);
    for (hipEvent_t e : ev_all) if (e) (void)hipEventDestroy(e);
    if (join_stream) (void)hipStreamDestroy(join_stream);
}

int lio_multi_set_map(lio_s2m_handle* h, const void* pts, size_t n, size_t stride)
{
    LioMulti* m = h->multi;
    const int world = (int)m->dev.size();
    const unsigned char* src = (const unsigned char*)pts;
    const float cell = h->cfg.cell_size > 0.0f ? h->cfg.cell_size : sqrtf(h->cfg.max_sq_dist) * 1.001f;
    const float inv_cell = 1.0f / cell;
    float mn[3] = { INFINITY, INFINITY, INFINITY }, mx[3] = { -INFINITY, -INFINITY, -INFINITY };
    for (size_t i = 0; i < n; ++i) {
        const float* p = (const float*)(src + i * stride);
        for (int a = 0; a < 3; ++a)
            if (fabsf(p[a]) <= 1.0e15f) { if (p[a] < mn[a]) mn[a] = p[a]; if (p[a] > mx[a]) mx[a] = p[a]; }
    }
    float origin[3];
    int32_t dims[3];
    int axis = 0;
    for (int a = 0; a < 3; ++a) {
        if (!(mn[a] <= mx[a])) { mn[a] = 0.0f; mx[a] = 0.0f; }
        origin[a] = mn[a] - 0.5f * cell;
        dims[a] = (int32_t)floor(((double)mx[a] - origin[a]) * inv_cell) + 2;
        if (dims[a] > dims[axis]) axis = a;
    }
    auto cell_of = [&](float v) {
        float c = floorf((v - origin[axis]) * inv_cell);
        c = fminf(fmaxf(c, -4.0f), (float)(dims[axis] + 3));
        int ci = (int)c;
        return ci < 0 ? 0 : (ci > dims[axis] - 1 ? dims[axis] - 1 : ci);
    };
    std::vector<long long> cum((size_t)dims[axis], 0);
    std::vector<int> pc(n);
    for (size_t i = 0; i < n; ++i) {
        const float* p = (const float*)(src + i * stride);
        const bool ok = fabsf(p[0]) <= 1.0e15f && fabsf(p[1]) <= 1.0e15f && fabsf(p[2]) <= 1.0e15f;
        pc[i] = ok ? cell_of(p[axis]) : -1000;
        if (ok) cum[(size_t)pc[i]]++;
    }
    for (size_t c = 1; c < cum.size(); ++c) cum[c] += cum[c - 1];
    const long long total = cum.empty() ? 0 : cum.back();
    std::vector<int> bounds((size_t)world + 1, 0);
    bounds[(size_t)world] = dims[axis];
    for (int r = 1; r < world; ++r) {
        const double want = (double)total * r / world;
        size_t lo = 0;
        while (lo < cum.size() && (double)cum[lo] < want) ++lo;
        bounds[(size_t)r] = (int)lo + 1;
        if (bounds[(size_t)r] > dims[axis]) bounds[(size_t)r] = dims[axis];
        if (bounds[(size_t)r] < bounds[(size_t)r - 1]) bounds[(size_t)r] = bounds[(size_t)r - 1];
    }
    for (int r = 0; r < world; ++r) {
        const int lo = bounds[(size_t)r], hi = bounds[(size_t)r + 1];
        std::vector<int>& idx = m->dev[(size_t)r]->shard_idx;
        idx.clear();
        for (size_t i = 0; i < n; ++i)
            if (pc[i] >= lo - LIO_MULTI_HALO && pc[i] < hi + LIO_MULTI_HALO) idx.push_back((int)i);
        m->gather.resize((idx.size() ? idx.size() : 1) * stride);
        for (size_t k = 0; k < idx.size(); ++k) memcpy(m->gather.data() + k * stride, src + (size_t)idx[k] * stride, stride);
        lio_s2m_handle* ch = m->dev[(size_t)r]->h;
        int rc = lio_s2m_set_map(ch, m->gather.data(), idx.size(), stride);
        if (rc == LIO_OK) rc = lio_s2m_set_global_grid(ch, origin, dims);
        if (rc == LIO_OK) rc = lio_s2m_set_shard_plan(ch, axis, world, r, bounds.data(), LIO_MULTI_HALO);
        if (rc != LIO_OK) return rc;
    }
    h->has_map = true;
    h->n_map = n;
    h->prof = m->dev[0]->h->prof;
    h->prof.n_map = (int64_t)n;
    return LIO_OK;
}

int lio_multi_upload(lio_s2m_handle* h, int32_t n_scans, const void* const* scans, const size_t* n_pts, size_t stride)
{
    LioMulti* m = h->multi;
    for (auto& c : m->dev) {
        lio_s2m_handle* ch = c->h;
        ch->defer_sync = true;
        ch->xyz_off = h->xyz_off;
        const int rc = lio_s2m_batch_upload(ch, n_scans, scans, n_pts, stride);
        ch->defer_sync = false;
        if (rc != LIO_OK) return rc;
    }
    h->xyz_off = 0;
    for (auto& c : m->dev) { const int rc = lio_s2m_batch_sync(c->h); if (rc != LIO_OK) return rc; }
    m->n_scans = n_scans;
    h->n_scans = n_scans;
    return lio_multi_reserve(h, (size_t)n_scans);
}

int lio_multi_set_poses(lio_s2m_handle* h, const float* poses)
{
    for (auto& c : h->multi->dev) { const int rc = lio_s2m_batch_set_poses(c->h, poses); if (rc != LIO_OK) return rc; }
    h->poses_set = true;
    return LIO_OK;
}

int lio_multi_set_degeneracy(lio_s2m_handle* h, int32_t scan, const float matP[36], int32_t is_degenerate)
{
    for (auto& c : h->multi->dev) { const int rc = lio_s2m_set_degeneracy(c->h, scan, matP, is_degenerate); if (rc != LIO_OK) return rc; }
    return LIO_OK;
}
// ... 134 lines not shown
```

### lio-slam_amd/csrc/liogpu_api.hip

```cpp
#include <hip/hip_runtime.h>
#include <math.h>
#include <stdio.h>
#include <string.h>
#include <algorithm>
#include <chrono>
#include <exception>
#include <memory>
#include <mutex>
#include <vector>

#include "lio_handle.h"
#include "lio_multi.h"
#include "lio_wg.h"


static thread_local char g_last_error[512];

int lio_fail(int code, const char* what, hipError_t e)
{
    if (e != hipSuccess) snprintf(g_last_error, sizeof(g_last_error), "%s: %s", what, hipGetErrorString(e));
    else snprintf(g_last_error, sizeof(g_last_error), "%s", what);
    return code;
}

int lio_fail_exception(void)
{
    char buf[256];
    try {
        throw;
    } catch (const std::exception& e) {
        snprintf(buf, sizeof(buf), "C++ exception: %s", e.what());
    } catch (...) {
        snprintf(buf, sizeof(buf), "C++ exception of an unknown type");
    }
    return lio_fail(LIO_ERR_CAPACITY, buf);
}

extern "C" int lio_version(void) { return LIO_VERSION; }
extern "C" const char* lio_last_error(void) { return g_last_error; }

extern "C" void lio_s2m_default_config(lio_s2m_config* c)
{
    memset(c, 0, sizeof(*c));
    c->k = 5;
    c->max_sq_dist = 1.0f;
    c->plane_tol = 0.2;
    c->weight = 0.9;
    c->min_s = 0.1;
    c->min_corr = 50;
    c->max_iters = 30;
    c->eig_thresh = 100.0f;
    c->conv_deg = 0.05;
    c->conv_cm = 0.05;
    c->min_scan_pts = 30;
    c->jacobian_mode = 0;
    c->force_all_iters = 0;
    c->device_id = 0;
    c->cell_size = 0.0f;
    c->max_batch = 1;
    c->max_scan_pts = 0;
    c->record_corr_iter = -1;
    c->kernel_variant = 0;
    c->profile = 0;
    c->lookahead = -1;
    c->use_lds = 0;
    c->cell_div = 2;
    c->xcd_remap = 1;
    c->tile_size = 0.0f;
    c->use_graph = 0;
    c->sort_batch = 1;
    c->graph_iters = 4;
    c->sort_scan = 1;
    c->nn_cache = 1;
    c->pipeline = 0;
    c->n_devices = 1;
    for (int i = 0; i < 8; ++i) c->device_ids[i] = i;
    c->x_sub = 0;
    c->tight_rows = 0;
}

static void lio_fill_consts(lio_s2m_handle* h)
{
    const lio_s2m_config& g = h->cfg;
    h->c.plane_tol = g.plane_tol; h->c.weight = g.weight; h->c.min_s = g.min_s;
    h->c.plane_tol_f = lio_threshold_f32(g.plane_tol); h->c.min_s_f = lio_threshold_f32(g.min_s);
    h->c.conv_deg = g.conv_deg; h->c.conv_cm = g.conv_cm;
    h->c.max_sq_dist = g.max_sq_dist; h->c.eig_thresh = g.eig_thresh;
    {
        volatile float r = sqrtf(g.max_sq_dist);
        r = r * 1.0001f;
        r = r + 1e-6f;
        h->c.gate_reach = r;
    }
    h->c.min_corr = g.min_corr; h->c.max_iters = g.max_iters;
    h->c.jac_exact = g.jacobian_mode ? 1 : 0; h->c.force_all = g.force_all_iters ? 1 : 0;
    h->c.record_iter = g.record_corr_iter; h->c.min_scan_pts = g.min_scan_pts;
}

static int lio_s2m_init_resources(lio_s2m_handle* h)
{
    HIPCHK(hipStreamCreateWithFlags(&h->stream, hipStreamNonBlocking));
    for (int i = 0; i < LIO_MAX_ITERS; ++i) {
        HIPCHK(hipEventCreate(&h->ev_beg[i]));
        HIPCHK(hipEventCreate(&h->ev_end[i]));
        HIPCHK(hipEventCreateWithFlags(&h->ev_chk[i], hipEventDisableTiming));
    }
    HIPCHK(h->h_active.grow(LIO_MAX_ITERS, LIO_MAX_ITERS));
    HIPCHK(hipEventCreate(&h->ev_map[0]));
    HIPCHK(hipEventCreate(&h->ev_map[1]));
    HIPCHK(hipEventCreate(&h->ev_mapl[0]));
    HIPCHK(hipEventCreate(&h->ev_mapl[1]));
    HIPCHK(h->d_bbox.grow(6, 1.0, 0));
    HIPCHK(h->d_active.grow(1, 1.0, 0));
    hipDeviceProp_t prop;
    if (hipGetDeviceProperties(&prop, h->cfg.device_id) == hipSuccess) h->n_cu = prop.multiProcessorCount;
    (void)hipGetLastError();
    return LIO_OK;
}

extern "C" int lio_s2m_create(const lio_s2m_config* cfg, lio_s2m_handle** out)
try {
    if (!cfg || !out) return lio_fail(LIO_ERR_ARG, "null argument");
    if (cfg->k != 5) return lio_fail(LIO_ERR_ARG, "only k = 5 is supported (MO:1631)");
    if (cfg->max_iters < 1 || cfg->max_iters > LIO_MAX_ITERS) return lio_fail(LIO_ERR_ARG, "max_iters out of range");
    if (!(cfg->max_sq_dist > 0.0f)) return lio_fail(LIO_ERR_ARG, "max_sq_dist must be positive");
    if (cfg->x_sub != 0 && cfg->x_sub != 1 && cfg->x_sub != 2 && cfg->x_sub != 4 && cfg->x_sub != 8)
        return lio_fail(LIO_ERR_ARG, "cfg.x_sub must be 0 (auto), 1, 2, 4 or 8");
    if (cfg->tight_rows < -1 || cfg->tight_rows > LIO_TB_MAX) return lio_fail(LIO_ERR_ARG, "cfg.tight_rows must be -1 (none), 0 (auto) or 1..3 tables");
    if (cfg->pipeline != 0 && cfg->pipeline != 1 && cfg->pipeline != 4)
        return lio_fail(LIO_ERR_ARG, "cfg.pipeline must be 0 (auto), 1 (one launch per iteration) or 4 (one-launch loop)");
    int ndev = 0;
    if (hipGetDeviceCount(&ndev) != hipSuccess || ndev <= 0)
        return lio_fail(LIO_ERR_NO_DEVICE, "no HIP device visible (this library has no CPU fallback)");
    if (cfg->device_id < 0 || cfg->device_id >= ndev) return lio_fail(LIO_ERR_ARG, "device_id out of range");
    if (cfg->n_devices > 1) {
        const int rc = lio_multi_create(cfg, out);
        if (rc == LIO_OK) lio_fill_consts(*out);
        return rc;
    }
    HIPCHK(hipSetDevice(cfg->device_id));
    if (cfg->cell_size > 0.0f && cfg->cell_size < sqrtf(cfg->max_sq_dist) * 1.001f)
        return lio_fail(LIO_ERR_ARG, "cell_size must be >= sqrt(max_sq_dist)*1.001 for an exact 27-cell search");
    std::unique_ptr<lio_s2m_handle> h(new lio_s2m_handle());
    h->cfg = *cfg;
    lio_fill_consts(h.get());
    h->shard.axis = -1;
    { const char* e = getenv("LIO_PLAIN_KERNEL"); h->plain_kernel = !(e && *e && atoi(e) == 0); }
    { const char* e = getenv("LIO_TAIL_FROM"); if (e && *e) h->tail_from = atoi(e) < 0 ? -1 : atoi(e); }
    { const char* e = getenv("LIO_TAIL_WGS"); if (e && *e) h->tail_wgs = atoi(e); }
    h->tail_wgs = h->tail_wgs < 8 ? 8 : ((h->tail_wgs + 7) & ~7);
    const int rc = lio_s2m_init_resources(h.get());
    if (rc != LIO_OK) return rc;
    *out = h.release();
    return LIO_OK;
} LIO_CATCH

extern "C" void lio_s2m_destroy(lio_s2m_handle* h)
{
    if (!h) return;
    if (h->multi) { lio_multi_destroy(h); return; }
    (void)hipSetDevice(h->cfg.device_id);
    (void)hipStreamSynchronize(h->stream);
    delete h;
}

lio_s2m_handle::~lio_s2m_handle()
{
    delete multi;
    lio_s2m_destroy(corner);
    lio_raw_ws_free(raw_ws);
    for (int i = 0; i < LIO_MAX_ITERS; ++i) {
        if (ev_beg[i]) (void)hipEventDestroy(ev_beg[i]);
        if (ev_end[i]) (void)hipEventDestroy(ev_end[i]);
        if (ev_chk[i]) (void)hipEventDestroy(ev_chk[i]);
    }
    for (hipEvent_t e : { ev_map[0], ev_map[1], ev_mapl[0], ev_mapl[1] }) if (e) (void)hipEventDestroy(e);
    if (graph_exec) (void)hipGraphExecDestroy(graph_exec);
    if (graph) (void)hipGraphDestroy(graph);
    if (own_stream && stream) (void)hipStreamDestroy(stream);
}

extern "C" int lio_s2m_set_stream(lio_s2m_handle* h, void* hip_stream)
try {
    if (h && h->multi) return lio_fail(LIO_ERR_ARG, "not available on a multi-device handle (cfg.n_devices > 1 shards inside the library)");
    if (!h) return lio_fail(LIO_ERR_ARG, "null handle");
    HIPCHK(hipStreamSynchronize(h->stream));
    if (h->own_stream && h->stream) HIPCHK(hipStreamDestroy(h->stream));
    h->stream = (hipStream_t)hip_stream;
    h->own_stream = false;
    h->graph_dirty = true;
    if (h->corner) return lio_s2m_set_stream(h->corner, hip_stream);
    return LIO_OK;
} LIO_CATCH

static const lio_s2m_handle* lio_map_of(const lio_s2m_handle* h) { return h->map_src ? h->map_src : h; }

static int lio_map_reserve(lio_s2m_handle* h, size_t n)
{
    const size_t nn = n ? n : 1;
    HIPCHK(h->d_mx.grow(nn));
    HIPCHK(h->d_my.grow(nn));
    HIPCHK(h->d_mz.grow(nn));
    HIPCHK(h->d_map4.grow(nn));
    HIPCHK(h->d_sorted.grow(nn));
    HIPCHK(h->d_cell_of.grow(nn));
    return LIO_OK;
}

static int lio_map_finish(lio_s2m_handle* h, size_t n, std::chrono::steady_clock::time_point t0, const float* box = nullptr)
{
    const size_t nn = n ? n : 1;
    float mn[3], mx[3];
    for (int a = 0; a < 3 && box; ++a)
        if (!(box[a] <= box[3 + a]) || !(fabsf(box[a]) <= 1.0e15f) || !(fabsf(box[3 + a]) <= 1.0e15f)) box = nullptr;
    if (box) {
        for (int a = 0; a < 3; ++a) { mn[a] = n ? box[a] : 0.0f; mx[a] = n ? box[3 + a] : 0.0f; }
    } else {
        unsigned init[6];
        lio_ord_box_clear(init);
        HIPCHK(hipMemcpyAsync(h->d_bbox, init, sizeof(init), hipMemcpyHostToDevice, h->stream));
        if (n) lio_launch_map_bbox(h->d_mx, h->d_my, h->d_mz, (int)n, h->d_bbox, h->stream);
        unsigned hb[6];
        HIPCHK(hipMemcpyAsync(hb, h->d_bbox, sizeof(hb), hipMemcpyDeviceToHost, h->stream));
        HIPCHK(hipStreamSynchronize(h->stream));
        lio_ord_box_decode(hb, mn, mx);
        bool empty = (n == 0) || hb[0] == LIO_ORD_NO_MIN;
        for (int a = 0; a < 3 && !empty; ++a) empty = !(mn[a] <= mx[a]);
        for (int a = 0; a < 3 && empty; ++a) mn[a] = mx[a] = 0.0f;
    }

    auto t1 = std::chrono::steady_clock::now();

    int kdiv = h->cfg.cell_div;
    if (kdiv != 1 && kdiv != 2 && kdiv != 3) kdiv = 2;
    float cell = (h->cfg.cell_size > 0.0f ? h->cfg.cell_size : sqrtf(h->cfg.max_sq_dist) * 1.001f) / (float)kdiv;
    int xsub = h->cfg.x_sub > 0 ? h->cfg.x_sub : (h->cfg.max_batch >= 8 ? 4 : 1);
    { const char* e = getenv("LIO_X_SUB"); const int v = e ? atoi(e) : 0; if (v == 1 || v == 2 || v == 4 || v == 8) xsub = v; }
    auto spacing_fits = [](float far_end, float slack) { return nextafterf(far_end, INFINITY) - far_end <= 0.5f * slack; };
    LioGrid g;
    for (;;) {
        g.k = kdiv;
        g.inv_cell = 1.0f / cell;
        g.ox = mn[0] - 0.5f * cell; g.oy = mn[1] - 0.5f * cell; g.oz = mn[2] - 0.5f * cell;
        const double ex = ((double)mx[0] - g.ox) * g.inv_cell, ey = ((double)mx[1] - g.oy) * g.inv_cell,
                     ez = ((double)mx[2] - g.oz) * g.inv_cell;
        const double cells = (floor(ex) + 2.0) * (floor(ey) + 2.0) * (floor(ez) + 2.0);
        const float slack = (float)kdiv * cell - h->c.gate_reach;
        if (cells * xsub <= 256.0 * 1024.0 * 1024.0 && spacing_fits((mx[1] - g.oy) + cell, slack) && spacing_fits((mx[2] - g.oz) + cell, slack) &&
            (!h->cfg.use_lds || spacing_fits((mx[0] - g.ox) + cell, slack))) {
            g.nx = (int)floor(ex) + 2; g.ny = (int)floor(ey) + 2; g.nz = (int)floor(ez) + 2;
            g.n_cells = g.nx * g.ny * g.nz;
            break;
        }
        cell *= 1.5f;
    }
    g.xs = xsub; g.nxf = g.nx * xsub; g.inv_cell_x = g.inv_cell * (float)xsub;
    float frac[LIO_TB_MAX] = { 0.6f, 0.3f, 0.15f };
    int n_tb = h->cfg.tight_rows > 0 ? std::min(h->cfg.tight_rows, LIO_TB_MAX) : 0;
    float pts_per_cell = 0.0f;
    int try_lvl = -1;
    if (h->cfg.tight_rows == 0 && h->cfg.max_batch >= 8) {
        n_tb = 1;
        if (!box && n > 0) {
            HIPCHK(h->d_cell_count.grow((size_t)g.n_cells + 1));
            lio_launch_map_occupancy(g, h->d_mx, h->d_my, h->d_mz, (int)n, h->d_cell_count, h->stream);
            int occ = 0;
            HIPCHK(hipMemcpyAsync(&occ, h->d_cell_count + g.n_cells, sizeof(int), hipMemcpyDeviceToHost, h->stream));
            HIPCHK(hipStreamSynchronize(h->stream));
            if (occ > 0) {
                pts_per_cell = (float)n / (float)occ;
                const float spacing = cell / sqrtf(pts_per_cell);
                while (n_tb < LIO_TB_MAX && sqrtf(h->cfg.max_sq_dist) * frac[n_tb] >= 1.26f * spacing) ++n_tb;
                for (int l = 0; l < n_tb; ++l)
                    if (sqrtf(h->cfg.max_sq_dist) * frac[l] >= 2.2f * spacing) try_lvl = l;
            }
        }
    }
    if (const char* e = getenv("LIO_TIGHT")) {
        n_tb = 0;
        for (const char* p = e; *p && n_tb < LIO_TB_MAX;) {
            char* q = nullptr;
            const float v = strtof(p, &q);
            if (q == p) break;
            if (v >= 0.05f && v <= 1.0f && (n_tb == 0 || v < frac[n_tb - 1])) frac[n_tb++] = v;
            p = (*q == ',') ? q + 1 : q;
            if (*q != ',') break;
        }
    }
    if ((double)g.n_cells * xsub > 64.0 * 1024.0 * 1024.0) n_tb = 0;
    size_t len_b = 0, rows_b = 0;
    for (int l = 0; l < LIO_TB_MAX; ++l) {
        g.tb_row0[l] = 0; g.tb_ny[l] = g.tb_nz[l] = 0; g.tb_oy[l] = g.tb_oz[l] = 0.0f; g.tb_inv_cell[l] = 0.0f; g.tb_reach[l] = -1.0f;
        if (l >= n_tb) continue;
        const float reach = sqrtf(h->cfg.max_sq_dist) * frac[l], cb = reach * 1.001f;
        const float inv = 1.0f / cb, oy = mn[1] - 0.5f * cb, oz = mn[2] - 0.5f * cb;
        const double ny = floor(((double)mx[1] - oy) * inv) + 2.0, nz = floor(((double)mx[2] - oz) * inv) + 2.0;
        const double recs = (double)nn * ((2 * g.k + 1) * (2 * g.k + 1) + 9.0 * (l + 1)) + LIO_ROW_ALIGN * ((double)g.ny * g.nz + (double)rows_b + ny * nz);
        if ((double)g.n_cells * xsub + (double)len_b + ny * nz * g.nxf > 192.0 * 1024.0 * 1024.0 || recs > 2040.0 * 1024.0 * 1024.0) { n_tb = l; continue; }
        const float slack = cb - reach / 1.0001f;
        if (!spacing_fits((mx[1] - oy) + cb, slack) || !spacing_fits((mx[2] - oz) + cb, slack)) { n_tb = l; continue; }
        g.tb_inv_cell[l] = inv; g.tb_oy[l] = oy; g.tb_oz[l] = oz; g.tb_ny[l] = (int)ny; g.tb_nz[l] = (int)nz;
        g.tb_row0[l] = (int)((size_t)g.n_cells * xsub + len_b);
        g.tb_reach[l] = reach;
        rows_b += (size_t)g.tb_ny[l] * g.tb_nz[l];
        len_b += (size_t)g.tb_ny[l] * g.tb_nz[l] * g.nxf;
    }
    if (const char* e = getenv("LIO_TRY")) try_lvl = atoi(e);
    g.tb_try = (try_lvl >= 0 && try_lvl < n_tb) ? try_lvl : (try_lvl >= n_tb ? n_tb - 1 : -1);
    for (int l = 0; l < LIO_TB_MAX; ++l) {
        const float r = g.tb_reach[l] > 0.0f ? g.tb_reach[l] / 1.0002f : 0.0f;
        g.tb_try_b2[l] = r * r * 0.999999f;
    }
    h->grid = g;
    const size_t len_a = (size_t)g.n_cells * xsub, reps = (size_t)((2 * g.k + 1) * (2 * g.k + 1)) + 9 * (size_t)n_tb;
    HIPCHK(h->d_cell_count.grow((size_t)g.n_cells + len_a + len_b));
    HIPCHK(h->d_cell_start.grow((size_t)g.n_cells + 1));
    HIPCHK(h->d_nbr_start.grow(len_a + len_b + 1));
    HIPCHK(h->d_nbr_pts.grow(nn * reps + LIO_ROW_ALIGN * ((size_t)g.ny * g.nz + rows_b) + 4 * LIO_ROW_ALIGN, 1.05));
    HIPCHK(h->d_tile_sums.grow(2 * ((size_t)lio_scan_tiles((int)(len_a + len_b)) + 1)));
    HIPCHK(h->d_nbr_slot.grow(nn * reps, 1.05));

    HIPCHK(hipEventRecord(box ? h->ev_mapl[0] : h->ev_map[0], h->stream));
    if (n) {
        lio_launch_map_build(g, h->d_mx, h->d_my, h->d_mz, (int)n, h->d_cell_of, h->d_cell_count,
                             h->d_cell_start, h->d_tile_sums, h->d_sorted, h->d_nbr_start, h->d_nbr_pts, h->d_nbr_slot, h->cfg.use_lds != 0, h->stream);
    } else {
        HIPCHK(hipMemsetAsync(h->d_cell_start, 0, sizeof(int) * ((size_t)g.n_cells + 1), h->stream));
        HIPCHK(hipMemsetAsync(h->d_nbr_start, 0, sizeof(int) * (len_a + len_b + 1), h->stream));
    }
// ... 135 lines not shown
    HIPCHK(hipSetDevice(device_id));
    HIPCHK(hipMemcpy(dst, src, bytes, hipMemcpyHostToDevice));
    return LIO_OK;
} LIO_CATCH
extern "C" int lio_host_register(void* p, size_t bytes)
try {
    if (!p || !bytes) return lio_fail(LIO_ERR_ARG, "null range");
    HIPCHK(hipHostRegister(p, bytes, hipHostRegisterDefault));
    return LIO_OK;
} LIO_CATCH
extern "C" int lio_host_unregister(void* p)
try {
    if (!p) return lio_fail(LIO_ERR_ARG, "null pointer");
    HIPCHK(hipHostUnregister(p));
    return LIO_OK;
} LIO_CATCH

extern "C" int lio_s2m_batch_upload_async(lio_s2m_handle* h, int32_t n_scans, const void* const* scans,
                                          const size_t* n_pts, size_t stride)
try {
    if (!h) return lio_fail(LIO_ERR_ARG, "null handle");
    const bool keep = h->defer_sync;
    h->defer_sync = true;
    h->async_upload = true;
    const int rc = lio_s2m_batch_upload(h, n_scans, scans, n_pts, stride);
    h->defer_sync = keep;
    h->async_upload = false;
    return rc;
} LIO_CATCH

extern "C" int lio_s2m_set_shard(lio_s2m_handle* h, int32_t axis, int32_t lo, int32_t hi)
try {
    if (h && h->multi) return lio_fail(LIO_ERR_ARG, "not available on a multi-device handle (cfg.n_devices > 1 shards inside the library)");
    if (!h) return lio_fail(LIO_ERR_ARG, "null handle");
    if (axis < 0) { h->shard.axis = -1; return LIO_OK; }
    if (axis > 2 || !h->has_global) return lio_fail(LIO_ERR_ARG, "set_global_grid first; axis in 0..2");
    const float cell = h->cfg.cell_size > 0.0f ? h->cfg.cell_size : sqrtf(h->cfg.max_sq_dist) * 1.001f;
    h->shard.axis = axis;
    h->shard.gorigin = h->gorigin[axis];
    h->shard.inv_cell = 1.0f / cell;
    h->shard.gdim = h->gdims[axis];
    h->shard.lo = lo;
    h->shard.hi = hi;
    h->plan_ranks = 0;
    h->graph_dirty = true;
    return LIO_OK;
} LIO_CATCH

extern "C" int lio_s2m_set_shard_plan(lio_s2m_handle* h, int32_t axis, int32_t n_ranks, int32_t rank, const int32_t* bounds,
                                      int32_t halo_cells)
try {
    if (!h || !bounds) return lio_fail(LIO_ERR_ARG, "null argument");
    if (h->multi) return lio_fail(LIO_ERR_ARG, "not available on a multi-device handle (cfg.n_devices > 1 shards inside the library)");
    if (n_ranks < 1 || n_ranks > 8 || rank < 0 || rank >= n_ranks || halo_cells < 1)
        return lio_fail(LIO_ERR_ARG, "need 1 <= n_ranks <= 8, 0 <= rank < n_ranks, halo_cells >= 1");
    for (int r = 0; r < n_ranks; ++r)
        if (bounds[r] > bounds[r + 1]) return lio_fail(LIO_ERR_ARG, "bounds must be non-decreasing");
    const int rc = lio_s2m_set_shard(h, axis, bounds[rank], bounds[rank + 1]);
    if (rc != LIO_OK) return rc;
    h->plan_ranks = halo_cells > 1 ? n_ranks : 0;
    h->plan_rank = rank;
    h->plan_halo = halo_cells;
    for (int r = 0; r <= n_ranks; ++r) h->plan_bounds[r] = bounds[r];
    return LIO_OK;
} LIO_CATCH

static bool lio_persist_eligible(const lio_s2m_handle* h)
{
    int limit = 0;
    if (h->cfg.pipeline == 4) limit = h->n_cu;
    else if (h->cfg.pipeline == 0 && !h->cfg.use_graph && h->cfg.profile != 2) limit = h->n_cu / 2;
    return limit > 0 && !h->no_persist && !h->cfg.use_lds && h->ppt == 1 && h->shard.axis < 0 &&
           h->block_world == 1 && h->n_blocks > 0 && h->n_blocks + h->n_scans <= limit;
}

static unsigned lio_persist_spin_max(const lio_s2m_handle* h)
{
    if (h->persist_spin_max) return h->persist_spin_max;
    static const unsigned env = [] { const char* e = getenv("LIO_PERSIST_SPIN_MAX"); const long v = e ? atol(e) : 0; return v > 0 ? (unsigned)v : 4096u; }();
    return env;
}

extern "C" int lio_s2m_debug_persist_spin(lio_s2m_handle* h, int32_t spin_max, int32_t withhold_wg)
try {
    if (!h) return lio_fail(LIO_ERR_ARG, "null handle");
    h->persist_spin_max = spin_max > 0 ? (unsigned)spin_max : 0u;
    h->persist_withhold = withhold_wg;
    return LIO_OK;
} LIO_CATCH

extern "C" int lio_debug_plane_fit(int32_t device_id, const float* sets, size_t n, double plane_tol, uint32_t* out)
try {
    if ((!sets || !out) && n) return lio_fail(LIO_ERR_ARG, "null pointer");
    if (n > ((size_t)1 << 27)) return lio_fail(LIO_ERR_CAPACITY, "at most 2^27 sets per call");
    if (!n) return LIO_OK;
    HIPCHK(hipSetDevice(device_id));
    LioDevBuf<float> d_sets;
    LioDevBuf<unsigned> d_out;
    HIPCHK(d_sets.grow(n * 15, 1.0, 0));
    HIPCHK(d_out.grow(n * 8, 1.0, 0));
    HIPCHK(hipMemcpy(d_sets, sets, n * 15 * sizeof(float), hipMemcpyHostToDevice));
    lio_launch_debug_plane_fit(d_sets, (long long)n, plane_tol, d_out, nullptr);
    HIPCHK(hipGetLastError());
    HIPCHK(hipMemcpy(out, d_out, n * 8 * sizeof(unsigned), hipMemcpyDeviceToHost));
    return LIO_OK;
} LIO_CATCH

extern "C" int lio_debug_fast_f32_ops(int32_t device_id, int32_t op, int32_t raw, const uint32_t* patterns, uint64_t first, uint64_t count,
                                      uint32_t* values, uint64_t* n_diff, uint32_t* first_diff, int32_t* n_first)
try {
    if (!n_diff || !first_diff || !n_first) return lio_fail(LIO_ERR_ARG, "null pointer");
    if (op < 0 || op > 2) return lio_fail(LIO_ERR_ARG, "op must be 0 (sqrt), 1 (x / 5) or 2 (fourth root of the range)");
    if (count > ((uint64_t)1 << 32)) return lio_fail(LIO_ERR_CAPACITY, "at most 2^32 patterns per call");
    if ((patterns || values) && count > ((uint64_t)1 << 27)) return lio_fail(LIO_ERR_CAPACITY, "at most 2^27 listed patterns or returned values per call");
    *n_diff = 0; *n_first = 0;
    if (!count) return LIO_OK;
    HIPCHK(hipSetDevice(device_id));
    LioDevBuf<unsigned> d_pat, d_val, d_diff;
    LioDevBuf<unsigned long long> d_n;
    if (patterns) {
        HIPCHK(d_pat.grow(count, 1.0, 0));
        HIPCHK(hipMemcpy(d_pat, patterns, count * sizeof(uint32_t), hipMemcpyHostToDevice));
    }
    if (values) HIPCHK(d_val.grow(count, 1.0, 0));
    HIPCHK(d_diff.grow(9, 1.0, 0));
    HIPCHK(d_n.grow(1, 1.0, 0));
    HIPCHK(hipMemset(d_diff, 0, 9 * sizeof(unsigned)));
    HIPCHK(hipMemset(d_n, 0, sizeof(unsigned long long)));
    lio_launch_debug_fast_f32_ops(op, raw ? 1 : 0, patterns ? (const unsigned*)d_pat : nullptr, first, count,
                                  values ? (unsigned*)d_val : nullptr, d_n, d_diff, nullptr);
    HIPCHK(hipGetLastError());
    unsigned h_diff[9];
    unsigned long long h_n = 0;
    HIPCHK(hipMemcpy(h_diff, d_diff, sizeof(h_diff), hipMemcpyDeviceToHost));
    HIPCHK(hipMemcpy(&h_n, d_n, sizeof(h_n), hipMemcpyDeviceToHost));
    if (values) HIPCHK(hipMemcpy(values, d_val, count * sizeof(uint32_t), hipMemcpyDeviceToHost));
    *n_diff = h_n;
    *n_first = (int32_t)(h_diff[0] < 8 ? h_diff[0] : 8);
    for (int i = 0; i < 8; ++i) first_diff[i] = h_diff[1 + i];
    return LIO_OK;
} LIO_CATCH

extern "C" float lio_debug_threshold_f32(double t) { return lio_threshold_f32(t); }

static int lio_ensure_soa(lio_s2m_handle* h)
{
    if (h->soa_valid || !h->total_pts) return LIO_OK;
    lio_launch_aos_to_soa(h->last_stage + h->last_xyz_off, h->last_stride, (int)h->total_pts, h->d_sx, h->d_sy, h->d_sz, nullptr, h->stream);
    h->soa_valid = true;
    HIPCHK(hipGetLastError());
    return LIO_OK;
}

extern "C" int lio_s2m_batch_upload(lio_s2m_handle* h, int32_t n_scans, const void* const* scans,
                                    const size_t* n_pts, size_t stride)
try {
    if (!h || !scans || !n_pts) return lio_fail(LIO_ERR_ARG, "null argument");
    if (n_scans < 1) return lio_fail(LIO_ERR_ARG, "n_scans must be >= 1");
    if (stride < 12 || (stride & 3)) return lio_fail(LIO_ERR_ARG, "stride_bytes must be >= 12 and a multiple of 4");
    if (h->multi) return lio_multi_upload(h, n_scans, scans, n_pts, stride);
    HIPCHK(hipSetDevice(h->cfg.device_id));
    (void)hipGetLastError();
    size_t total = 0, max_n = 0;
    for (int s = 0; s < n_scans; ++s) {
        if (n_pts[s] && !scans[s]) return lio_fail(LIO_ERR_ARG, "null scan pointer");
        total += n_pts[s];
        if (n_pts[s] > max_n) max_n = n_pts[s];
    }
    if (total > 0x7fffffffull - 1024) return lio_fail(LIO_ERR_CAPACITY, "batch too large");
    h->run_pending = false;
    if (h->host_state_stale && h->n_scans > 0 && h->d_state) {
        HIPCHK(hipMemcpyAsync(h->h_state.data(), h->d_state, (size_t)h->n_scans * sizeof(LioScanState),
                              hipMemcpyDeviceToHost, h->stream));
        HIPCHK(hipStreamSynchronize(h->stream));
    }
    h->host_state_stale = false;
    const size_t tt = total ? total : 1;
    HIPCHK(h->d_sx.grow(tt));
    HIPCHK(h->d_sy.grow(tt));
    HIPCHK(h->d_sz.grow(tt));
    HIPCHK(h->d_stage.grow(tt * stride));
    HIPCHK(h->d_state.grow((size_t)n_scans));
    HIPCHK(h->d_poses.grow((size_t)n_scans * 6));
    {
        bool fresh = false;
        HIPCHK(h->d_arrive.grow((size_t)n_scans, 1.25, 64, false, &fresh));
        if (fresh) HIPCHK(hipMemsetAsync(h->d_arrive, 0, h->d_arrive.cap * sizeof(unsigned), h->stream));
    }
    if (h->cfg.nn_cache && !h->cfg.use_lds) HIPCHK(h->d_nn_cache.grow(tt));

    int ppt = h->cfg.kernel_variant;
    if (ppt != 1 && ppt != 2 && ppt != 4) ppt = 1;
    h->ppt = ppt;
    const size_t per_blk = (size_t)LIO_BLOCK * ppt;
    std::vector<LioBlockDesc>& blocks = h->v_blocks;
    blocks.clear();
    int max_blk = 1;
    const size_t old_scans = h->h_state.size();
    h->h_state.resize((size_t)n_scans);
    size_t off = 0;
    for (int s = 0; s < n_scans; ++s) {
        LioScanState& st = h->h_state[s];
        if ((size_t)s >= old_scans) memset(&st, 0, sizeof(st));
        st.n_pts = (int)n_pts[s];
        st.offset = (int)off;
        if (h->reg_pose && n_scans == 1) memcpy(st.pose, h->reg_pose, sizeof(float) * 6);
        st.c_n_pts = 0;
        st.c_offset = 0;
        st.done = 1;
        const int nb = (int)((n_pts[s] + per_blk - 1) / per_blk);
        const int bw = h->block_world > 1 ? h->block_world : 1, br = h->block_world > 1 ? h->block_rank : 0;
        const int part = (br + s) % bw;
        const int b0 = (int)((long long)nb * part / bw), b1 = (int)((long long)nb * (part + 1) / bw);
        const int nb_local = b1 - b0;
        if (nb_local > max_blk) max_blk = nb_local;
        for (int b = b0; b < b1; ++b) blocks.push_back({ s, (int)(b * per_blk), b - b0, nb_local });
        off += n_pts[s];
    }
    const unsigned char* stage = h->d_stage;
    bool host_copy = false;
    {
        bool contiguous = true;
        for (int s = 0; s + 1 < n_scans && contiguous; ++s)
            contiguous = (const unsigned char*)scans[s + 1] == (const unsigned char*)scans[s] + n_pts[s] * stride;
        bool in_place = false;
        if (contiguous && total) {
            hipPointerAttribute_t at;
            if (hipPointerGetAttributes(&at, scans[0]) == hipSuccess)
                in_place = at.type == hipMemoryTypeDevice && at.device == h->cfg.device_id;
            (void)hipGetLastError();
        }
        if (in_place) {
            stage = (const unsigned char*)scans[0];
        } else if (contiguous && total) {
            HIPCHK(hipMemcpyAsync(h->d_stage, scans[0], total * stride, hipMemcpyDefault, h->stream));
            host_copy = true;
        } else {
            host_copy = true;
            size_t o = 0;
            for (int s = 0; s < n_scans; ++s) {
                if (n_pts[s])
                    HIPCHK(hipMemcpyAsync(h->d_stage + o * stride, scans[s], n_pts[s] * stride, hipMemcpyDefault, h->stream));
                o += n_pts[s];
            }
        }
    }
    if (host_copy && h->async_upload) {
        HIPCHK(hipEventRecord(h->ev_map[0], h->stream));
        HIPCHK(hipEventSynchronize(h->ev_map[0]));
    }
    h->last_stage = stage; h->last_stride = stride; h->last_xyz_off = h->xyz_off;
    h->last_int_off = h->int_off != -2 ? h->int_off : ((h->xyz_off == 0 && stride >= 20) ? 16 : -1);
    h->int_off = -2;
    stage += h->xyz_off;
    h->xyz_off = 0;
    h->v_first_orig.assign((size_t)n_scans + 1, 0);
    for (const LioBlockDesc& b : blocks) h->v_first_orig[b.scan + 1]++;
    for (int s = 0; s < n_scans; ++s) h->v_first_orig[s + 1] += h->v_first_orig[s];
    h->n_scans = n_scans;
    h->total_pts = total;
    h->n_blocks = (int)blocks.size();
    h->max_blk = max_blk;
    HIPCHK(h->d_blocks.grow(blocks.size() ? blocks.size() : 1));
    HIPCHK(h->d_partials.grow((size_t)n_scans * max_blk * LIO_SUMS));
    if (h->cfg.profile == 2) {
        HIPCHK(h->d_stamps.grow(blocks.size() * (LIO_BLOCK / 64) * 8 + 8));
        HIPCHK(hipMemsetAsync(h->d_stamps, 0, (blocks.size() * (LIO_BLOCK / 64) * 8 + 8) * sizeof(long long), h->stream));
    }
    if (h->cfg.record_corr_iter >= 0) {
        HIPCHK(h->d_rec_flag.grow(tt));
        HIPCHK(h->d_rec_coeff.grow(tt * 4));
        HIPCHK(h->d_rec_nn.grow(tt * 5));
        HIPCHK(hipMemsetAsync(h->d_rec_flag, 0, tt, h->stream));
        HIPCHK(hipMemsetAsync(h->d_rec_coeff, 0, tt * 4 * sizeof(float), h->stream));
        HIPCHK(hipMemsetAsync(h->d_rec_nn, 0xff, tt * 5 * sizeof(int), h->stream));
    }
    if (!blocks.empty())
        HIPCHK(hipMemcpyAsync(h->d_blocks, blocks.data(), blocks.size() * sizeof(LioBlockDesc),
                              hipMemcpyHostToDevice, h->stream));
    HIPCHK(hipMemcpyAsync(h->d_state, h->h_state.data(), (size_t)n_scans * sizeof(LioScanState),
                          hipMemcpyHostToDevice, h->stream));
    std::vector<LioScanTiles>& tiles = h->v_tiles;
    std::vector<LioBlockDesc>& prep = h->v_prep;
    tiles.clear(); prep.clear();
    h->sorted = false;
    const bool want_sort = total && (h->cfg.sort_scan >= 2 || (h->cfg.sort_scan == 1 && total >= 65536));
    if (want_sort && max_n < 16384 && h->cfg.sort_scan != 3) {
        HIPCHK(h->d_perm.grow(tt));
        lio_launch_scan_sort_lds(stage, stride, h->d_state, n_scans, (int)max_n, h->cfg.tile_size > 0.0f ? h->cfg.tile_size : 4.0f,
                                 h->shard.axis, h->d_perm, h->d_sx, h->d_sy, h->d_sz, h->stream);
        h->sorted = true;
    } else if (want_sort) {
        for (int s = 0; s < n_scans; ++s) {
            const int nb1 = (int)((n_pts[s] + LIO_BLOCK - 1) / LIO_BLOCK);
            for (int b = 0; b < nb1; ++b) prep.push_back({ s, b * LIO_BLOCK, b, nb1 });
        }
        HIPCHK(h->d_prep_blocks.grow(prep.size()));
        HIPCHK(h->d_scan_bbox.grow((size_t)n_scans * 6));
        HIPCHK(h->h_scan_bbox.grow((size_t)n_scans * 6, (size_t)n_scans * 6 + 64));
        for (int s = 0; s < n_scans; ++s)
            lio_ord_box_clear(&h->h_scan_bbox[s * 6]);
        HIPCHK(hipMemcpyAsync(h->d_scan_bbox, h->h_scan_bbox, (size_t)n_scans * 6 * sizeof(unsigned), hipMemcpyHostToDevice, h->stream));
        HIPCHK(hipMemcpyAsync(h->d_prep_blocks, prep.data(), prep.size() * sizeof(LioBlockDesc), hipMemcpyHostToDevice, h->stream));
        lio_launch_scan_bbox(stage, stride, h->d_prep_blocks, (int)prep.size(), h->d_state, h->d_scan_bbox, h->stream);
        HIPCHK(hipMemcpyAsync(h->h_scan_bbox, h->d_scan_bbox, (size_t)n_scans * 6 * sizeof(unsigned), hipMemcpyDeviceToHost, h->stream));
        HIPCHK(hipStreamSynchronize(h->stream));
        tiles.resize((size_t)n_scans);
        long long n_keys = 0;
        for (int s = 0; s < n_scans; ++s) {
            float mn[3], mx[3];
            for (int a = 0; a < 3; ++a) {
                const unsigned lo = h->h_scan_bbox[s * 6 + a], hi = h->h_scan_bbox[s * 6 + 3 + a];
                const bool none = lo == LIO_ORD_NO_MIN;
                mn[a] = none ? 0.0f : lio_ord2f(lo);
                mx[a] = none ? 0.0f : lio_ord2f(hi);
            }
            float tile = h->cfg.tile_size > 0.0f ? h->cfg.tile_size : 4.0f;
            LioScanTiles t;
            for (;;) {
                t.inv_tile = 1.0f / tile;
                const double ex = floor(((double)mx[0] - mn[0]) * t.inv_tile) + 1.0, ey = floor(((double)mx[1] - mn[1]) * t.inv_tile) + 1.0,
                             ez = floor(((double)mx[2] - mn[2]) * t.inv_tile) + 1.0;
                if (ex * ey * ez <= 262144.0) { t.ntx = (int)ex; t.nty = (int)ey; t.ntz = (int)ez; break; }
                tile *= 2.0f;
            }
            t.ox = mn[0]; t.oy = mn[1]; t.oz = mn[2];
            t.key_offset = (int)n_keys;
            t.mx = 1; t.my = t.ntx; t.mz = t.ntx * t.nty;
            if (h->shard.axis == 0) { t.mz = 1; t.my = t.ntz; t.mx = t.ntz * t.nty; }
            else if (h->shard.axis == 1) { t.mx = 1; t.mz = t.ntx; t.my = t.ntx * t.ntz; }
            tiles[s] = t;
            n_keys += (long long)t.ntx * t.nty * t.ntz;
        }
        if (n_keys < 0x7fffffffLL - 1024) {
            HIPCHK(h->d_tiles.grow((size_t)n_scans));
            HIPCHK(h->d_key_of.grow(tt));
            HIPCHK(h->d_big_list.grow(tt / 1024 + 2));
            HIPCHK(h->d_tmp_idx.grow(tt));
            HIPCHK(h->d_perm.grow(tt));
            HIPCHK(h->d_key_count.grow((size_t)n_keys));
            HIPCHK(h->d_key_start.grow((size_t)n_keys + 1));
            HIPCHK(h->d_key_tiles.grow((size_t)lio_scan_tiles((int)n_keys) + 1));
            HIPCHK(hipMemcpyAsync(h->d_tiles, tiles.data(), tiles.size() * sizeof(LioScanTiles), hipMemcpyHostToDevice, h->stream));
            lio_launch_scan_tile_sort(stage, stride, (int)total, h->d_prep_blocks, (int)prep.size(), h->d_state,
                                      h->d_tiles, (int)n_keys, h->d_key_of, h->d_key_count, h->d_key_start,
                                      h->d_key_tiles, h->d_tmp_idx, h->d_perm, h->d_big_list, h->d_big_list + (h->d_big_list.cap - 1),
                                      h->d_sx, h->d_sy, h->d_sz, h->stream);
            h->sorted = true;
        }
    }
    h->soa_valid = true;
    if (total && !h->sorted) {
        if (lio_persist_eligible(h)) h->soa_valid = false;
        else lio_launch_aos_to_soa(stage, stride, (int)total, h->d_sx, h->d_sy, h->d_sz, nullptr, h->stream);
    }
    h->has_block_box = false;
    if (h->shard.axis >= 0 && ppt == 1 && !blocks.empty()) {
        HIPCHK(h->d_block_box.grow((tt / LIO_BLOCK + (size_t)n_scans + 2) * 6));
        HIPCHK(h->d_blk_skip.grow(blocks.size()));
        lio_launch_block_boxes(h->d_blocks, (int)blocks.size(), h->d_state, h->d_sx, h->d_sy, h->d_sz, h->d_block_box, h->stream);
        h->has_block_box = true;
    }
    if (!h->defer_sync) HIPCHK(hipStreamSynchronize(h->stream));
    HIPCHK(hipGetLastError());
    h->poses_set = false;
    h->pose_in_state = h->reg_pose != nullptr && n_scans == 1;
    h->ran = false;
    h->graph_dirty = true;
    h->corner_active = false;
    return LIO_OK;
} LIO_CATCH

extern "C" int lio_s2m_set_corner_map(lio_s2m_handle* h, const void* pts, size_t n, size_t stride)
try {
    if (!h) return lio_fail(LIO_ERR_ARG, "null handle");
    if (h->multi) return lio_fail(LIO_ERR_ARG, "the corner extension is not available on a multi-device handle");
    HIPCHK(hipSetDevice(h->cfg.device_id));
    (void)hipGetLastError();
    if (!h->corner) {
        lio_s2m_config cc = h->cfg;
        cc.kernel_variant = 1;
        cc.use_lds = 0;
        cc.profile = 0;
        cc.use_graph = 0;
        cc.pipeline = 1;
        int rc = lio_s2m_create(&cc, &h->corner);
        if (rc != LIO_OK) return rc;
        if ((rc = lio_s2m_set_stream(h->corner, h->stream)) != LIO_OK) return rc;
    }
    h->corner_active = false;
    h->graph_dirty = true;
    return lio_s2m_set_map(h->corner, pts, n, stride);
} LIO_CATCH

extern "C" int lio_s2m_batch_upload_corners(lio_s2m_handle* h, int32_t n_scans, const void* const* scans,
                                            const size_t* n_pts, size_t stride)
try {
    if (!h || !scans || !n_pts) return lio_fail(LIO_ERR_ARG, "null argument");
    if (!h->corner || !h->corner->has_map) return lio_fail(LIO_ERR_NO_MAP, "set_corner_map has not been called");
    if (h->n_scans < 1 || n_scans != h->n_scans)
        return lio_fail(LIO_ERR_ARG, "upload the surf batch first; the corner batch must have the same number of scans");
    lio_s2m_handle* ch = h->corner;
    ch->block_rank = h->block_rank;
    ch->block_world = h->block_world;
    ch->defer_sync = h->defer_sync;
    int rc = lio_s2m_batch_upload(ch, n_scans, scans, n_pts, stride);
    ch->defer_sync = false;
    if (rc != LIO_OK) return rc;
    int max_blk = 1;
    for (LioBlockDesc& b : h->v_blocks) {
        const int ns = h->v_first_orig[b.scan + 1] - h->v_first_orig[b.scan];
        const int nc = ch->v_first_orig[b.scan + 1] - ch->v_first_orig[b.scan];
        b.n_blk = ns + nc;
        if (b.n_blk > max_blk) max_blk = b.n_blk;
    }
    for (LioBlockDesc& b : ch->v_blocks) {
        const int ns = h->v_first_orig[b.scan + 1] - h->v_first_orig[b.scan];
        const int nc = ch->v_first_orig[b.scan + 1] - ch->v_first_orig[b.scan];
        b.blk += ns;
        b.n_blk = ns + nc;
        if (b.n_blk > max_blk) max_blk = b.n_blk;
    }
    h->max_blk = max_blk;
    HIPCHK(h->d_partials.grow((size_t)n_scans * max_blk * LIO_SUMS));
    if (!h->v_blocks.empty())
        HIPCHK(hipMemcpyAsync(h->d_blocks, h->v_blocks.data(), h->v_blocks.size() * sizeof(LioBlockDesc),
                              hipMemcpyHostToDevice, h->stream));
    if (!ch->v_blocks.empty())
        HIPCHK(hipMemcpyAsync(ch->d_blocks, ch->v_blocks.data(), ch->v_blocks.size() * sizeof(LioBlockDesc),
                              hipMemcpyHostToDevice, h->stream));
    for (int s = 0; s < n_scans; ++s) {
        h->h_state[s].c_n_pts = ch->h_state[s].n_pts;
        h->h_state[s].c_offset = ch->h_state[s].offset;
    }
    HIPCHK(hipMemcpyAsync(h->d_state, h->h_state.data(), (size_t)n_scans * sizeof(LioScanState),
                          hipMemcpyHostToDevice, h->stream));
    if (!h->defer_sync) HIPCHK(hipStreamSynchronize(h->stream));
    h->corner_active = true;
    h->poses_set = false;
    h->graph_dirty = true;
    return LIO_OK;
} LIO_CATCH

extern "C" int lio_s2m_get_corner_correspondences(lio_s2m_handle* h, int32_t scan, uint8_t* flag,
                                                  float* coeff4, int32_t* nn_idx5)
try {
    if (!h) return lio_fail(LIO_ERR_ARG, "null handle");
    if (!h->corner || !h->corner_active) return lio_fail(LIO_ERR_ARG, "no corner batch is resident");
    return lio_s2m_get_correspondences(h->corner, scan, flag, coeff4, nn_idx5);
} LIO_CATCH

extern "C" int lio_s2m_batch_set_poses(lio_s2m_handle* h, const float* poses)
try {
    if (!h || !poses) return lio_fail(LIO_ERR_ARG, "null argument");
    if (h->n_scans < 1) return lio_fail(LIO_ERR_ARG, "no batch uploaded");
    if (h->multi) return lio_multi_set_poses(h, poses);
    HIPCHK(hipSetDevice(h->cfg.device_id));
    (void)hipGetLastError();
    h->run_pending = false;
    h->pose_in_state = false;
    HIPCHK(hipMemcpyAsync(h->d_poses, poses, (size_t)h->n_scans * 6 * sizeof(float), hipMemcpyHostToDevice, h->stream));
    if (h->cfg.sort_batch && h->n_scans > 8 && !h->v_blocks.empty()) {
        const LioGrid& mg = lio_map_of(h)->grid;
        const float ext[3] = { (float)mg.nx, (float)mg.ny, (float)mg.nz };
        const int ax = (ext[0] >= ext[1] && ext[0] >= ext[2]) ? 0 : (ext[1] >= ext[2] ? 1 : 2);
        std::vector<int>& order = h->v_order;
        order.resize((size_t)h->n_scans);
        for (int s = 0; s < h->n_scans; ++s) order[s] = s;
        std::stable_sort(order.begin(), order.end(),
                         [&](int a, int b) { return poses[a * 6 + 3 + ax] < poses[b * 6 + 3 + ax]; });
        std::vector<int>& first = h->v_first;
        first.assign((size_t)h->n_scans + 1, 0);
        for (const LioBlockDesc& b : h->v_blocks) first[b.scan + 1]++;
        for (int s = 0; s < h->n_scans; ++s) first[s + 1] += first[s];
        std::vector<LioBlockDesc>& sorted = h->v_blocks_sorted;
        sorted.clear();
        sorted.reserve(h->v_blocks.size());
        for (int k = 0; k < h->n_scans; ++k) {
            const int s = order[k];
            for (int i = h->v_first_orig[s]; i < h->v_first_orig[s + 1]; ++i) sorted.push_back(h->v_blocks[i]);
        }
        HIPCHK(hipMemcpyAsync(h->d_blocks, sorted.data(), sorted.size() * sizeof(LioBlockDesc), hipMemcpyHostToDevice, h->stream));
    }
    if (!h->defer_sync) HIPCHK(hipStreamSynchronize(h->stream));
    h->poses_set = true;
    return LIO_OK;
} LIO_CATCH

extern "C" int lio_s2m_set_degeneracy(lio_s2m_handle* h, int32_t scan, const float matP[36], int32_t is_degenerate)
try {
    if (!h || !matP) return lio_fail(LIO_ERR_ARG, "null argument");
    if (scan < 0 || scan >= h->n_scans) return lio_fail(LIO_ERR_ARG, "scan slot out of range");
    if (h->multi) return lio_multi_set_degeneracy(h, scan, matP, is_degenerate);
    HIPCHK(hipSetDevice(h->cfg.device_id));
    (void)hipGetLastError();
    LioScanState& st = h->h_state[scan];
    memcpy(st.matP, matP, sizeof(float) * 36);
    st.is_degenerate = is_degenerate;
    char* base = (char*)(h->d_state + scan);
    HIPCHK(hipMemcpyAsync(base + offsetof(LioScanState, matP), st.matP, sizeof(float) * 36, hipMemcpyHostToDevice, h->stream));
    HIPCHK(hipMemcpyAsync(base + offsetof(LioScanState, is_degenerate), &st.is_degenerate, sizeof(int), hipMemcpyHostToDevice, h->stream));
    HIPCHK(hipStreamSynchronize(h->stream));
    return LIO_OK;
} LIO_CATCH

static void lio_fill_params(lio_s2m_handle* h, LioIterParams& P, double* sums_out)
{
    const lio_s2m_handle* m = lio_map_of(h);
    P.grid = m->grid;
    P.shard = h->shard;
    P.c = h->c;
    P.map_sorted = m->d_sorted;
    P.map_xyz4 = m->d_map4;
    P.cell_start = m->d_cell_start;
    P.nbr_pts = m->d_nbr_pts;
    P.nbr_start = m->d_nbr_start;
    P.sx = h->d_sx; P.sy = h->d_sy; P.sz = h->d_sz;
    P.perm = h->sorted ? h->d_perm : nullptr;
    P.state = h->d_state;
    P.blocks = h->d_blocks;
    P.partials = h->d_partials;
    P.arrive = h->d_arrive;
    P.max_blk = h->max_blk;
    P.xcd_remap = h->cfg.xcd_remap;
    P.n_active = h->d_active;
    P.sums_out = sums_out;
    const bool rec = h->cfg.record_corr_iter >= 0;
    P.rec_flag = rec ? h->d_rec_flag : nullptr;
    P.rec_coeff = rec ? h->d_rec_coeff : nullptr;
    P.rec_nn = rec ? h->d_rec_nn : nullptr;
    P.stamps = (h->cfg.profile == 2) ? h->d_stamps : nullptr;
    P.d5_cache = (h->cfg.nn_cache && !h->cfg.use_lds) ? h->d_nn_cache : nullptr;
    P.blk_skip = (h->shard.axis >= 0 && h->has_block_box && sums_out != nullptr && !h->cfg.use_lds && h->ppt == 1) ? h->d_blk_skip : nullptr;
    if (P.blk_skip) P.xcd_remap = 0;
}

static void lio_fill_params_corner(lio_s2m_handle* h, LioIterParams& Pc, double* sums_out)
{
    lio_fill_params(h->corner, Pc, sums_out);
    Pc.shard = h->shard;
    Pc.state = h->d_state;
    Pc.partials = h->d_partials;
    Pc.arrive = h->d_arrive;
    Pc.max_blk = h->max_blk;
    Pc.n_active = h->d_active;
    Pc.stamps = nullptr;
}

static bool lio_launch_gn(lio_s2m_handle* h, const LioIterParams& P, const LioIterParams* Pc, int index)
{
    if (Pc) lio_launch_iterate(*Pc, h->corner->n_blocks, 1, false, h->stream, true);
    const int tail_wgs = (h->tail_from >= 0 && index >= h->tail_from) ? h->tail_wgs : 0;
    bool looped = false;
    h->iterate_variant = lio_launch_iterate(P, h->n_blocks, h->ppt, h->cfg.use_lds != 0, h->stream, false, h->plain_kernel && !Pc, tail_wgs, &looped);
    return looped;
}

extern "C" int lio_s2m_batch_begin(lio_s2m_handle* h)
try {
    if (h && h->multi) return lio_fail(LIO_ERR_ARG, "not available on a multi-device handle (cfg.n_devices > 1 shards inside the library)");
    if (!h) return lio_fail(LIO_ERR_ARG, "null handle");
    if (!lio_map_of(h)->has_map) return lio_fail(LIO_ERR_NO_MAP, "set_map has not been called");
    if (h->n_scans < 1 || !h->poses_set) return lio_fail(LIO_ERR_ARG, "batch_upload and batch_set_poses first");
    HIPCHK(hipSetDevice(h->cfg.device_id));
    (void)hipGetLastError();
    if (h->map_src && h->map_epoch != h->map_src->map_epoch) {
        h->map_epoch = h->map_src->map_epoch;
        h->graph_dirty = true;
        HIPCHK(hipStreamWaitEvent(h->stream, h->map_src->ev_mapl[1], 0));
    }
    lio_launch_init_state(h->d_state, h->n_scans, h->d_poses, h->pose_in_state, h->c, h->d_active, h->stream);
    h->pose_in_state = false;
    if (h->cfg.nn_cache && !h->cfg.use_lds && h->d_nn_cache && h->shard.axis >= 0)
        HIPCHK(hipMemsetAsync(h->d_nn_cache, 0xff, (h->total_pts ? h->total_pts : 1) * sizeof(float), h->stream));
    if (h->corner_active && h->corner->d_nn_cache && h->shard.axis >= 0)
        HIPCHK(hipMemsetAsync(h->corner->d_nn_cache, 0xff, (h->corner->total_pts ? h->corner->total_pts : 1) * sizeof(float), h->stream));
    h->launches_this_run = 0;
    h->units_this_run = 0;
    h->unit_iters = 1;
    h->iterate_variant = 0;
    h->run_n_full = h->run_n_looped = 0;
    h->ran = true;
    return LIO_OK;
} LIO_CATCH

static int lio_graph_prepare(lio_s2m_handle* h, const LioIterParams& P, const LioIterParams* Pc, int chunk)
{
    const int nbc = Pc ? h->corner->n_blocks : -1;
    if (h->graph_exec && h->graph_chunk == chunk && h->graph_blocks == h->n_blocks && h->graph_ppt == h->ppt &&
        h->graph_plain == h->plain_kernel && h->graph_tail_from == h->tail_from && h->graph_tail_wgs == h->tail_wgs &&
        memcmp(&h->graph_params, &P, sizeof(P)) == 0 && h->graph_blocks_c == nbc &&
        (!Pc || memcmp(&h->graph_params_c, Pc, sizeof(P)) == 0))
        return LIO_OK;
    if (h->graph_exec) { HIPCHK(hipGraphExecDestroy(h->graph_exec)); h->graph_exec = nullptr; }
    if (h->graph) { HIPCHK(hipGraphDestroy(h->graph)); h->graph = nullptr; }
    HIPCHK(hipStreamBeginCapture(h->stream, hipStreamCaptureModeThreadLocal));
    h->graph_n_full = h->graph_n_looped = 0;
    for (int i = 0; i < chunk; ++i) {
        if (lio_launch_gn(h, P, Pc, i)) h->graph_n_looped++;
        else h->graph_n_full++;
    }
    HIPCHK(hipStreamEndCapture(h->stream, &h->graph));
    HIPCHK(hipGraphInstantiate(&h->graph_exec, h->graph, nullptr, nullptr, 0));
    h->graph_chunk = chunk; h->graph_blocks = h->n_blocks; h->graph_ppt = h->ppt; h->graph_plain = h->plain_kernel;
    h->graph_tail_from = h->tail_from; h->graph_tail_wgs = h->tail_wgs;
    memcpy(&h->graph_params, &P, sizeof(P));
    h->graph_blocks_c = nbc;
    if (Pc) memcpy(&h->graph_params_c, Pc, sizeof(P));
    h->graph_dirty = false;
    return LIO_OK;
}

static int lio_run_continue(lio_s2m_handle* h, bool blocking)
{
    if (!h->run_pending) return LIO_OK;
    const bool prof = h->cfg.profile != 0;
    const LioIterParams* Pc = h->run_has_c ? &h->run_Pc : nullptr;
    while (h->run_next < h->run_units && h->run_next < LIO_MAX_ITERS) {
        const int u = h->run_next;
        const int chk = u - 1 - h->run_look;
        if (chk >= 0) {
            if (blocking) {
                HIPCHK(hipEventSynchronize(h->ev_chk[chk]));
            } else {
                const hipError_t q = hipEventQuery(h->ev_chk[chk]);
                if (q == hipErrorNotReady) { (void)hipGetLastError(); return LIO_OK; }
                HIPCHK(q);
            }
            if (h->h_active[chk] == 0) break;
        }
        if (prof) HIPCHK(hipEventRecord(h->ev_beg[u], h->stream));
        if (h->run_persist) {
            lio_launch_persist(h->run_P, h->n_blocks, h->d_gen, h->gen_epoch, h->soa_valid ? nullptr : h->last_stage + h->last_xyz_off,
                               h->last_stride, h->n_scans, getenv("LIO_NO_SPEC") ? nullptr : h->d_gen + h->n_scans, h->d_spec_sums, h->d_poses,
                               lio_persist_spin_max(h), h->persist_withhold, h->stream);
        } else if (h->run_graph) {
            HIPCHK(hipGraphLaunch(h->graph_exec, h->stream));
            h->run_n_full += h->graph_n_full; h->run_n_looped += h->graph_n_looped;
        } else if (lio_launch_gn(h, h->run_P, Pc, u)) h->run_n_looped++;
        else h->run_n_full++;
        if (prof) HIPCHK(hipEventRecord(h->ev_end[u], h->stream));
        if (!h->run_persist) HIPCHK(hipMemcpyAsync(&h->h_active[u], h->d_active, sizeof(int), hipMemcpyDeviceToHost, h->stream));
        HIPCHK(hipEventRecord(h->ev_chk[u], h->stream));
        h->run_next = u + 1;
        h->units_this_run = u + 1;
        h->launches_this_run = (u + 1) * h->unit_iters;
    }
    h->run_pending = false;
    HIPCHK(hipGetLastError());
    return LIO_OK;
}

extern "C" int lio_s2m_batch_run(lio_s2m_handle* h)
try {
    if (h && h->multi) return lio_multi_run(h);
    int rc = lio_s2m_batch_begin(h);
    if (rc != LIO_OK) return rc;
    LioIterParams& P = h->run_P;
    memset(&P, 0, sizeof(P));
    lio_fill_params(h, P, nullptr);
    memset(&h->run_Pc, 0, sizeof(h->run_Pc));
    h->run_has_c = h->corner_active && h->corner->n_blocks > 0;
    if (h->run_has_c) lio_fill_params_corner(h, h->run_Pc, nullptr);
    int look = h->cfg.lookahead;
    if (look < 0) look = (h->total_pts >= 200000) ? 0 : 2;
    h->run_persist = lio_persist_eligible(h) && !h->run_has_c;
    if (!h->run_persist && (rc = lio_ensure_soa(h)) != LIO_OK) return rc;
    const bool graph = !h->run_persist && h->cfg.use_graph != 0 && h->cfg.profile != 2 && h->cfg.record_corr_iter < 0 && h->n_blocks > 0;
    int chunk = 1;
    if (graph) {
        chunk = h->cfg.graph_iters > 0 ? h->cfg.graph_iters : 4;
        if (chunk > h->cfg.max_iters) chunk = h->cfg.max_iters;
        if ((rc = lio_graph_prepare(h, P, h->run_has_c ? &h->run_Pc : nullptr, chunk)) != LIO_OK) return rc;
        if (h->cfg.lookahead < 0) look = 0;
    }
    if (h->run_persist) {
        bool fresh = false;
        HIPCHK(h->d_gen.grow((size_t)h->n_scans * 2, 1.25, 64, false, &fresh));
        if (fresh) {
            HIPCHK(hipMemsetAsync(h->d_gen, 0, h->d_gen.cap * sizeof(unsigned), h->stream));
            h->gen_epoch = 0;
        }
        HIPCHK(h->d_spec_sums.grow((size_t)h->n_scans * LIO_SUMS));
        h->gen_epoch += 128;
        chunk = h->cfg.max_iters;
    }
    if (!h->run_persist)
        h->iterate_variant = lio_iterate_variant(P, h->ppt, h->cfg.use_lds != 0, false, h->plain_kernel && !h->run_has_c);
    h->run_graph = graph;
    h->run_look = look;
    h->run_units = (h->cfg.max_iters + chunk - 1) / chunk;
    h->run_next = 0;
    h->unit_iters = h->run_persist ? 1 : chunk;
    h->units_this_run = 0;
    h->launches_this_run = 0;
    h->run_pending = true;
    return lio_run_continue(h, h->defer_sync);
} LIO_CATCH

extern "C" int lio_s2m_kernel_variant(const lio_s2m_handle* h)
try {
    if (!h) return lio_fail(LIO_ERR_ARG, "null handle");
    if (h->multi) return 0;
    return h->iterate_variant;
} LIO_CATCH

extern "C" int lio_s2m_launch_forms(const lio_s2m_handle* h, int32_t* n_full, int32_t* n_looped)
try {
    if (!h || !n_full || !n_looped) return lio_fail(LIO_ERR_ARG, "null argument");
    *n_full = h->multi ? 0 : h->run_n_full;
    *n_looped = h->multi ? 0 : h->run_n_looped;
    return LIO_OK;
} LIO_CATCH

extern "C" int lio_s2m_batch_iter_partial(lio_s2m_handle* h, double* d_sums)
try {
    if (!h || !d_sums) return lio_fail(LIO_ERR_ARG, "null argument");
    if (!h->ran) return lio_fail(LIO_ERR_ARG, "batch_begin first");
    HIPCHK(hipSetDevice(h->cfg.device_id));
    (void)hipGetLastError();
    { const int rcs = lio_ensure_soa(h); if (rcs != LIO_OK) return rcs; }
    LioIterParams P;
    lio_fill_params(h, P, d_sums);
    HIPCHK(hipMemsetAsync(d_sums, 0, (size_t)h->n_scans * LIO_SUMS * sizeof(double), h->stream));
    const int it = h->launches_this_run;
    const bool prof = h->cfg.profile != 0 && it < LIO_MAX_ITERS;
    if (prof) HIPCHK(hipEventRecord(h->ev_beg[it], h->stream));
    LioIterParams Pcs;
    const bool with_corners = h->corner_active && h->corner->n_blocks > 0;
    if (with_corners) lio_fill_params_corner(h, Pcs, d_sums);
    if (P.blk_skip && !getenv("LIO_NO_CULL")) {
        lio_launch_shard_cull(P, h->plan_ranks, h->plan_rank, h->plan_halo, h->plan_bounds, h->d_block_box, h->n_blocks, h->d_blk_skip,
                              h->stream);
        if (getenv("LIO_CULL_STATS")) {
            std::vector<unsigned char> sk((size_t)h->n_blocks);
            HIPCHK(hipMemcpyAsync(sk.data(), h->d_blk_skip, sk.size(), hipMemcpyDeviceToHost, h->stream));
            HIPCHK(hipStreamSynchronize(h->stream));
            size_t c = 0;
            for (unsigned char v : sk) c += v;
            size_t c2 = 0;
            for (unsigned char v : sk) c2 += (v == 2);
            c = 0;
            for (unsigned char v : sk) c += (v == 1);
            fprintf(stderr, "[liogpu] shard cull: %zu of %d workgroups skipped, %zu wholly owned (iteration %d)\n", c, h->n_blocks, c2, it);
        }
    } else {
        P.blk_skip = nullptr;
    }
    if (lio_launch_gn(h, P, with_corners ? &Pcs : nullptr, it)) h->run_n_looped++;
    else h->run_n_full++;
    if (prof) HIPCHK(hipEventRecord(h->ev_end[it], h->stream));
    h->launches_this_run++;
    h->units_this_run = h->launches_this_run;
    HIPCHK(hipGetLastError());
    return LIO_OK;
} LIO_CATCH

extern "C" int lio_s2m_batch_iter_apply(lio_s2m_handle* h, const double* d_sums)
try {
    return lio_s2m_iter_apply_slots(h, d_sums, 0, 1);
} LIO_CATCH

int lio_s2m_iter_apply_slots(lio_s2m_handle* h, const double* d_sums, size_t slot_stride, int n_slots)
{
    if (!h || !d_sums || n_slots < 1) return lio_fail(LIO_ERR_ARG, "null argument");
    if (!h->ran || h->launches_this_run < 1) return lio_fail(LIO_ERR_ARG, "batch_iter_partial first");
    HIPCHK(hipSetDevice(h->cfg.device_id));
    (void)hipGetLastError();
    lio_launch_apply(h->d_state, h->n_scans, d_sums, slot_stride, n_slots, h->c, h->d_active, h->stream);
    const int it = h->launches_this_run - 1;
    if (it < LIO_MAX_ITERS) {
        HIPCHK(hipMemcpyAsync(&h->h_active[it], h->d_active, sizeof(int), hipMemcpyDeviceToHost, h->stream));
        HIPCHK(hipEventRecord(h->ev_chk[it], h->stream));
    }
    HIPCHK(hipGetLastError());
    return LIO_OK;
}

extern "C" int lio_s2m_batch_poll_active(lio_s2m_handle* h, int32_t iteration, int32_t* n_active)
try {
    if (!h || !n_active) return lio_fail(LIO_ERR_ARG, "null argument");
    if (iteration < 0 || iteration >= h->launches_this_run || iteration >= LIO_MAX_ITERS)
        return lio_fail(LIO_ERR_ARG, "iteration has not been applied");
    HIPCHK(hipEventSynchronize(h->ev_chk[iteration]));
    *n_active = h->h_active[iteration];
    return LIO_OK;
} LIO_CATCH

extern "C" int lio_s2m_batch_n_active(lio_s2m_handle* h, int32_t* n_active)
try {
    if (!h || !n_active) return lio_fail(LIO_ERR_ARG, "null argument");
    HIPCHK(hipSetDevice(h->cfg.device_id));
    (void)hipGetLastError();
    HIPCHK(hipMemcpyAsync(&h->h_active[0], h->d_active, sizeof(int), hipMemcpyDeviceToHost, h->stream));
    HIPCHK(hipStreamSynchronize(h->stream));
    *n_active = h->h_active[0];
    return LIO_OK;
} LIO_CATCH

extern "C" int lio_s2m_batch_sync(lio_s2m_handle* h)
try {
    if (!h) return lio_fail(LIO_ERR_ARG, "null handle");
    if (h->multi) return lio_multi_sync(h);
    HIPCHK(hipSetDevice(h->cfg.device_id));
    (void)hipGetLastError();
    { const int rcc = lio_run_continue(h, true); if (rcc != LIO_OK) return rcc; }
    HIPCHK(hipStreamSynchronize(h->stream));
    HIPCHK(hipGetLastError());
    return LIO_OK;
} LIO_CATCH

extern "C" int lio_s2m_batch_results(lio_s2m_handle* h, float* poses, lio_s2m_result* results)
try {
    if (!h) return lio_fail(LIO_ERR_ARG, "null handle");
    if (h->multi) return lio_multi_results(h, poses, results);
    if (!h->ran) return lio_fail(LIO_ERR_ARG, "nothing has been run");
    HIPCHK(hipSetDevice(h->cfg.device_id));
    (void)hipGetLastError();
    { const int rcc = lio_run_continue(h, true); if (rcc != LIO_OK) return rcc; }
    if (results) {
        HIPCHK(hipMemcpyAsync(h->h_state.data(), h->d_state, (size_t)h->n_scans * sizeof(LioScanState),
                              hipMemcpyDeviceToHost, h->stream));
        HIPCHK(hipStreamSynchronize(h->stream));
        h->host_state_stale = false;
    } else {
        const size_t need = (size_t)h->n_scans * 10;
        HIPCHK(h->d_summary.grow(need));
        HIPCHK(h->h_summary.grow(need, need + 64));
        h->host_state_stale = true;
        lio_launch_pack_summary(h->d_state, h->n_scans, h->d_summary, h->stream);
        HIPCHK(hipMemcpyAsync(h->h_summary, h->d_summary, need * sizeof(float), hipMemcpyDeviceToHost, h->stream));
        HIPCHK(hipStreamSynchronize(h->stream));
        for (int s = 0; s < h->n_scans; ++s) {
            LioScanState& st = h->h_state[s];
            const float* o = h->h_summary + (size_t)s * 10;
            memcpy(st.pose, o, sizeof(float) * 6);
            memcpy(&st.iter, o + 6, 4); memcpy(&st.status, o + 7, 4);
            st.done = (st.status & 0x100) ? 0 : 1;
            st.status &= 0xff;
            memcpy(&st.converged, o + 8, 4); memcpy(&st.is_degenerate, o + 9, 4);
        }
    }
    HIPCHK(hipGetLastError());
    if (h->run_persist) {
        bool incomplete = false;
        for (int s = 0; s < h->n_scans; ++s) incomplete = incomplete || !h->h_state[s].done;
        if (incomplete) {
            h->persist_fallbacks++;
            h->prof.persist_fallbacks = h->persist_fallbacks;
            HIPCHK(hipMemsetAsync(h->d_arrive, 0, h->d_arrive.cap * sizeof(unsigned), h->stream));
            const bool keep_defer = h->defer_sync;
            h->no_persist = true; h->defer_sync = true;
            h->poses_set = true; h->pose_in_state = false;
            int rc = lio_s2m_batch_run(h);
            h->defer_sync = keep_defer;
            if (rc == LIO_OK) rc = lio_s2m_batch_results(h, poses, results);
            h->no_persist = false;
            return rc;
        }
    }
    int64_t pit = 0;
    for (int s = 0; s < h->n_scans; ++s) {
        const LioScanState& st = h->h_state[s];
        if (poses) memcpy(poses + (size_t)s * 6, st.pose, sizeof(float) * 6);
        pit += (int64_t)(st.n_pts + st.c_n_pts) * (st.status == 2 ? 1 : st.iter) * (st.status == 1 ? 0 : 1);
// ... 348 lines not shown
```

Before: 477,600.

## Build scan tables on device and update graph kernel nodes in place

Per-scan state rows and the block descriptor list are now built on the GPU by small kernels from a compact row table, uploaded through double-buffered pinned staging. This replaces the host-side state readback, the host block-list construction and the large host-to-device copies. Captured HIP graphs are also updated in place with hipGraphExecKernelNodeSetParams instead of being re-captured and re-instantiated when only parameters or block counts change. The cost is extra tiny kernel launches and an event sync on the previous graph launch, and graph node discovery relies on a linear chain.

```diff
diff --git a/include/liogpu.h b/include/liogpu.h
--- a/include/liogpu.h
+++ b/include/liogpu.h
@@ -146,6 +146,10 @@
 int  lio_s2m_get_profile(lio_s2m_handle *h, lio_s2m_profile *out);
 int  lio_s2m_kernel_variant(const lio_s2m_handle *h);
 int  lio_s2m_launch_forms(const lio_s2m_handle *h, int32_t *n_full, int32_t *n_looped);
+int  lio_s2m_graph_stats(const lio_s2m_handle *h, int32_t *n_instantiated, int32_t *n_updated);
+int  lio_s2m_debug_tables(lio_s2m_handle *h, int32_t *blocks_out, size_t cap_blocks, int32_t *state_fields_out);
+int  lio_debug_block_list(const int32_t *n_pts, int32_t n_scans, int32_t per_blk, int32_t rank, int32_t world, const int32_t *order,
+                          int32_t *blocks_out, size_t cap_blocks, int32_t *max_blk);
 int  lio_s2m_debug_persist_spin(lio_s2m_handle *h, int32_t spin_max, int32_t withhold_wg);
 
 int  lio_debug_plane_fit(int32_t device_id, const float *sets, size_t n, double plane_tol, uint32_t *out);
diff --git a/lio-slam_amd/api.py b/lio-slam_amd/api.py
--- a/lio-slam_amd/api.py
+++ b/lio-slam_amd/api.py
@@ -246,6 +246,7 @@
     "lio_sdf_default_config", "lio_sdf_create", "lio_sdf_destroy", "lio_sdf_build", "lio_kf_store_sdf", "lio_sdf_nodes", "lio_sdf_query",
     "lio_occupancy_sdf", "lio_sdf_debug_stage_ms", "lio_sdf_memory",
     "lio_debug_fast_f32_ops", "lio_debug_threshold_f32",
+    "lio_s2m_graph_stats", "lio_s2m_debug_tables", "lio_debug_block_list",
 ]
 
 
@@ -295,6 +296,10 @@
     L.lio_s2m_kernel_variant.argtypes = [vp]
     if hasattr(L, "lio_s2m_launch_forms"):
         L.lio_s2m_launch_forms.argtypes = [vp, C.POINTER(i32), C.POINTER(i32)]
+    if hasattr(L, "lio_s2m_graph_stats"):
+        L.lio_s2m_graph_stats.argtypes = [vp, C.POINTER(i32), C.POINTER(i32)]
+        L.lio_s2m_debug_tables.argtypes = [vp, vp, sz, vp]
+        L.lio_debug_block_list.argtypes = [vp, i32, i32, i32, i32, vp, vp, sz, C.POINTER(i32)]
     L.lio_s2m_set_corner_map.argtypes = [vp, vp, sz, sz]
     L.lio_s2m_batch_upload_corners.argtypes = [vp, i32, C.POINTER(vp), C.POINTER(sz), sz]
     L.lio_s2m_register_cs.argtypes = [vp, vp, sz, vp, sz, sz, C.POINTER(f32), C.POINTER(S2MResult)]
@@ -612,6 +617,19 @@
         _check(self.lib.lio_s2m_launch_forms(self.h, C.byref(full), C.byref(looped)), "lio_s2m_launch_forms")
         return full.value, looped.value
 
+    def graph_stats(self):
+        inst, upd = C.c_int32(0), C.c_int32(0)
+        _check(self.lib.lio_s2m_graph_stats(self.h, C.byref(inst), C.byref(upd)), "lio_s2m_graph_stats")
+        return inst.value, upd.value
+
+    def debug_tables(self):
+        fields = np.zeros((self._n_scans, 6), np.int32)
+        nb = self.lib.lio_s2m_debug_tables(self.h, None, 0, None)
+        _check(min(nb, 0), "lio_s2m_debug_tables")
+        blocks = np.zeros((nb, 4), np.int32)
+        _check(min(self.lib.lio_s2m_debug_tables(self.h, blocks.ctypes.data, nb, fields.ctypes.data), 0), "lio_s2m_debug_tables")
+        return blocks, fields
+
     def debug_persist_spin(self, spin_max=0, withhold_wg=-1):
         _check(self.lib.lio_s2m_debug_persist_spin(self.h, int(spin_max), int(withhold_wg)), "lio_s2m_debug_persist_spin")
 
@@ -826,6 +844,18 @@
     fn.argtypes = [C.c_double]
     fn.restype = C.c_float
     return np.float32(fn(float(t)))
+
+
+def debug_block_list(n_pts, per_blk=256, rank=0, world=1, order=None):
+    L = load_library()
+    n = np.ascontiguousarray(n_pts, np.int32)
+    o = None if order is None else np.ascontiguousarray(order, np.int32)
+    args = (n.ctypes.data, len(n), int(per_blk), int(rank), int(world), None if o is None else o.ctypes.data)
+    mb = C.c_int32(0)
+    cnt = _check(L.lio_debug_block_list(*args, None, 0, C.byref(mb)), "lio_debug_block_list")
+    blocks = np.zeros((cnt, 4), np.int32)
+    _check(L.lio_debug_block_list(*args, blocks.ctypes.data, cnt, C.byref(mb)), "lio_debug_block_list")
+    return blocks, mb.value
 
 
 def range_image(records, t_cur, imu, device_id=0, **cfg_overrides):
diff --git a/lio-slam_amd/csrc/lio_handle.h b/lio-slam_amd/csrc/lio_handle.h
--- a/lio-slam_amd/csrc/lio_handle.h
+++ b/lio-slam_amd/csrc/lio_handle.h
@@ -8,6 +8,7 @@
 #include "../../include/liogpu.h"
 #include "lio_kernels.h"
 #include "lio_pool.h"
+#include "lio_tables.h"
 #include "lio_types.h"
 
 int lio_pc2_check_xyz(const lio_pc2_layout* L);
@@ -46,7 +47,7 @@
     std::vector<LioBlockDesc> v_blocks, v_prep;
     std::vector<LioScanTiles> v_tiles;
     std::vector<LioBlockDesc> v_blocks_sorted;
-    std::vector<int> v_order, v_first, v_first_orig;
+    std::vector<int> v_order, v_first_orig;
     bool defer_sync = false;
     bool async_upload = false;
     LioDevBuf<float> d_poses;
@@ -57,6 +58,16 @@
     bool host_state_stale = false;
     LioDevBuf<LioBlockDesc> d_blocks;
     int n_blocks = 0, ppt = 1, max_blk = 1;
+    bool device_tables = true;
+    bool dev_tables_batch = false;
+    bool host_blocks_valid = false;
+    bool blocks_from_host = false;
+    LioDevBuf<LioScanRow> d_rows;
+    LioDevBuf<int> d_order;
+    LioPinned<unsigned char> h_tab[2];
+    hipEvent_t ev_tab[2] = {};
+    bool ev_tab_used[2] = { false, false };
+    int tab_slot = 0;
     LioDevBuf<double> d_partials;
     LioDevBuf<unsigned> d_arrive;
     bool poses_set = false, ran = false;
@@ -103,6 +114,13 @@
     int tail_wgs = LIO_TAIL_WGS_DEFAULT;
     int graph_tail_from = -1, graph_tail_wgs = 0;
     int graph_n_full = 0, graph_n_looped = 0;
+    bool graph_update = true;
+    struct GraphNode { hipGraphNode_t node; int form; };
+    std::vector<GraphNode> graph_nodes;
+    int graph_variant = 0;
+    bool graph_stage = false;
+    hipEvent_t graph_last_launch = nullptr;
+    int graph_instantiated = 0, graph_updated = 0;
     int run_n_full = 0, run_n_looped = 0;
 
     LioDevBuf<unsigned char> d_rec_flag;
diff --git a/lio-slam_amd/csrc/lio_kernels.h b/lio-slam_amd/csrc/lio_kernels.h
--- a/lio-slam_amd/csrc/lio_kernels.h
+++ b/lio-slam_amd/csrc/lio_kernels.h
@@ -48,6 +48,11 @@
                          int tail_wgs = 0, bool* looped = nullptr);
 #define LIO_TAIL_FROM_DEFAULT 7
 #define LIO_TAIL_WGS_DEFAULT 1536
+static inline int lio_tail_grid(int n_blocks, int tail_wgs)
+{
+    const int a = tail_wgs & ~7, b = (n_blocks + 7) & ~7;
+    return a < b ? a : b;
+}
 void lio_launch_iterate_tail(const LioIterParams& P, int n_blocks, int n_wgs, hipStream_t s);
 void lio_launch_persist(const LioIterParams& P, int n_blocks, unsigned* gen, unsigned epoch, const unsigned char* stage, size_t stride,
                         int n_scans, unsigned* spec, double* spec_sums, const float* poses0, unsigned spin_max, int withhold_wg, hipStream_t s);
diff --git a/lio-slam_amd/csrc/lio_kernels.hip b/lio-slam_amd/csrc/lio_kernels.hip
--- a/lio-slam_amd/csrc/lio_kernels.hip
+++ b/lio-slam_amd/csrc/lio_kernels.hip
@@ -844,7 +844,7 @@
     if (looped) *looped = false;
     if (n_blocks <= 0) return variant;
     if ((variant & 1) && tail_wgs >= 8 && !corner && !stage) {
-        const int n_wgs = std::min(tail_wgs & ~7, (n_blocks + 7) & ~7);
+        const int n_wgs = lio_tail_grid(n_blocks, tail_wgs);
         lio_launch_iterate_tail(P, n_blocks, n_wgs, s);
         if (looped) *looped = true;
         return variant;
diff --git a/lio-slam_amd/csrc/lio_multi.hip b/lio-slam_amd/csrc/lio_multi.hip
--- a/lio-slam_amd/csrc/lio_multi.hip
+++ b/lio-slam_amd/csrc/lio_multi.hip
@@ -70,6 +70,7 @@
         std::unique_ptr<LioMultiChild> ch(new LioMultiChild());
         const int rc = lio_s2m_create(&cc, &ch->h);
         if (rc != LIO_OK) return rc;
+        ch->h->device_tables = false;
         m->dev.push_back(std::move(ch));
     }
     for (int a = 0; a < cfg->n_devices && m->exchange == 0; ++a)
diff --git a/lio-slam_amd/csrc/lio_tables.h b/lio-slam_amd/csrc/lio_tables.h
--- /dev/null
+++ b/lio-slam_amd/csrc/lio_tables.h
@@ -0,0 +1,41 @@
+#pragma once
+#include <hip/hip_runtime.h>
+#include <vector>
+#include "lio_types.h"
+
+struct LioScanRow {
+    int32_t n_pts;
+    int32_t offset;
+    float pose[6];
+};
+
+__host__ __device__ inline void lio_block_range(long long n_pts, int per_blk, int s, int rank, int world, int* b0, int* b1)
+{
+    const int nb = (int)((n_pts + per_blk - 1) / per_blk);
+    const int bw = world > 1 ? world : 1, br = world > 1 ? rank : 0;
+    const int part = (br + s) % bw;
+    *b0 = (int)((long long)nb * part / bw);
+    *b1 = (int)((long long)nb * (part + 1) / bw);
+}
+
+template <typename N>
+inline int lio_build_block_list(const N* n_pts, int n_scans, int per_blk, int rank, int world, const int* order,
+                                std::vector<LioBlockDesc>& out)
+{
+    out.clear();
+    int max_blk = 1;
+    for (int k = 0; k < n_scans; ++k) {
+        const int s = order ? order[k] : k;
+        int b0, b1;
+        lio_block_range((long long)n_pts[s], per_blk, s, rank, world, &b0, &b1);
+        const int nb_local = b1 - b0;
+        if (nb_local > max_blk) max_blk = nb_local;
+        for (int b = b0; b < b1; ++b) out.push_back({ s, (int)((long long)b * per_blk), b - b0, nb_local });
+    }
+    return max_blk;
+}
+
+void lio_launch_state_rows(LioScanState* st, const LioScanRow* rows, int n_scans, int prev_scans, bool with_pose, hipStream_t s);
+void lio_launch_state_corner_rows(LioScanState* st, const LioScanRow* corner_rows, int n_scans, hipStream_t s);
+void lio_launch_block_list(const LioScanRow* rows, const int* order, int n_scans, int per_blk, int rank, int world,
+                           LioBlockDesc* blocks, int cap, hipStream_t s);
diff --git a/lio-slam_amd/csrc/lio_tables.hip b/lio-slam_amd/csrc/lio_tables.hip
--- /dev/null
+++ b/lio-slam_amd/csrc/lio_tables.hip
@@ -0,0 +1,85 @@
+#include <hip/hip_runtime.h>
+#include <algorithm>
+#include "lio_tables.h"
+#include "lio_wg.h"
+
+#define LIO_TAB_WAVES 4
+
+__global__ __launch_bounds__(256) void k_state_rows(LioScanState* __restrict__ st, const LioScanRow* __restrict__ rows, int n_scans,
+                                                    int prev_scans, int with_pose)
+{
+    const int s = blockIdx.x * blockDim.x + threadIdx.x;
+    if (s >= n_scans) return;
+    LioScanState& d = st[s];
+    if (s >= prev_scans) __builtin_memset(&d, 0, sizeof(LioScanState));
+    const LioScanRow r = rows[s];
+    d.n_pts = r.n_pts;
+    d.offset = r.offset;
+    if (with_pose)
+        for (int i = 0; i < 6; ++i) d.pose[i] = r.pose[i];
+    d.c_n_pts = 0;
+    d.c_offset = 0;
+    d.done = 1;
+}
+
+__global__ __launch_bounds__(256) void k_state_corner_rows(LioScanState* __restrict__ st, const LioScanRow* __restrict__ corner_rows, int n_scans)
+{
+    const int s = blockIdx.x * blockDim.x + threadIdx.x;
+    if (s >= n_scans) return;
+    st[s].c_n_pts = corner_rows[s].n_pts;
+    st[s].c_offset = corner_rows[s].offset;
+}
+
+__global__ __launch_bounds__(LIO_TAB_WAVES * 64) void k_block_list(const LioScanRow* __restrict__ rows, const int* __restrict__ order,
+                                                                   int n_scans, int per_blk, int rank, int world,
+                                                                   LioBlockDesc* __restrict__ blocks, int cap)
+{
+    __shared__ int s_wave[LIO_TAB_WAVES];
+    __shared__ int s_scan[LIO_TAB_WAVES * 64], s_b0[LIO_TAB_WAVES * 64], s_nb[LIO_TAB_WAVES * 64], s_start[LIO_TAB_WAVES * 64];
+    const int tid = threadIdx.x, lane = tid & 63, wave = tid >> 6;
+    int carry = 0;
+    for (int k0 = 0; k0 < n_scans; k0 += LIO_TAB_WAVES * 64) {
+        const int k = k0 + tid;
+        int s = 0, b0 = 0, b1 = 0;
+        if (k < n_scans) {
+            s = order ? order[k] : k;
+            if (s >= 0 && s < n_scans) lio_block_range(rows[s].n_pts, per_blk, s, rank, world, &b0, &b1);
+        }
+        int tot;
+        const int ex = lio_wg_exclusive_scan<LIO_TAB_WAVES>(b1 - b0, &tot, s_wave);
+        s_scan[tid] = s; s_b0[tid] = b0; s_nb[tid] = b1 - b0; s_start[tid] = carry + ex;
+        __syncthreads();
+        const int n_here = min(LIO_TAB_WAVES * 64, n_scans - k0);
+        for (int j = wave + LIO_TAB_WAVES * (int)blockIdx.x; j < n_here; j += LIO_TAB_WAVES * (int)gridDim.x) {
+            const int sc = s_scan[j], f0 = s_b0[j], nb = s_nb[j], at = s_start[j];
+            for (int i = lane; i < nb; i += 64) {
+                if (at + i < cap) {
+                    const long long first = (long long)(f0 + i) * per_blk;
+                    ((int4*)blocks)[at + i] = make_int4(sc, (int)first, i, nb);
+                }
+            }
+        }
+        carry += tot;
+        __syncthreads();
+    }
+}
+
+void lio_launch_state_rows(LioScanState* st, const LioScanRow* rows, int n_scans, int prev_scans, bool with_pose, hipStream_t s)
+{
+    if (n_scans <= 0) return;
+    hipLaunchKernelGGL(k_state_rows, dim3((n_scans + 255) / 256), dim3(256), 0, s, st, rows, n_scans, prev_scans, with_pose ? 1 : 0);
+}
+
+void lio_launch_state_corner_rows(LioScanState* st, const LioScanRow* corner_rows, int n_scans, hipStream_t s)
+{
+    if (n_scans <= 0) return;
+    hipLaunchKernelGGL(k_state_corner_rows, dim3((n_scans + 255) / 256), dim3(256), 0, s, st, corner_rows, n_scans);
+}
+
+void lio_launch_block_list(const LioScanRow* rows, const int* order, int n_scans, int per_blk, int rank, int world,
+                           LioBlockDesc* blocks, int cap, hipStream_t s)
+{
+    if (n_scans <= 0 || cap <= 0) return;
+    const int grid = (std::min(n_scans, LIO_TAB_WAVES * 64) + LIO_TAB_WAVES - 1) / LIO_TAB_WAVES;
+    hipLaunchKernelGGL(k_block_list, dim3(grid), dim3(LIO_TAB_WAVES * 64), 0, s, rows, order, n_scans, per_blk, rank, world, blocks, cap);
+}
diff --git a/lio-slam_amd/csrc/liogpu_api.hip b/lio-slam_amd/csrc/liogpu_api.hip
--- a/lio-slam_amd/csrc/liogpu_api.hip
+++ b/lio-slam_amd/csrc/liogpu_api.hip
@@ -110,6 +110,7 @@
     HIPCHK(hipEventCreate(&h->ev_map[1]));
     HIPCHK(hipEventCreate(&h->ev_mapl[0]));
     HIPCHK(hipEventCreate(&h->ev_mapl[1]));
+    for (hipEvent_t& e : h->ev_tab) HIPCHK(hipEventCreateWithFlags(&e, hipEventDisableTiming));
     HIPCHK(h->d_bbox.grow(6, 1.0, 0));
     HIPCHK(h->d_active.grow(1, 1.0, 0));
     hipDeviceProp_t prop;
@@ -149,6 +150,8 @@
     { const char* e = getenv("LIO_TAIL_FROM"); if (e && *e) h->tail_from = atoi(e) < 0 ? -1 : atoi(e); }
     { const char* e = getenv("LIO_TAIL_WGS"); if (e && *e) h->tail_wgs = atoi(e); }
     h->tail_wgs = h->tail_wgs < 8 ? 8 : ((h->tail_wgs + 7) & ~7);
+    { const char* e = getenv("LIO_DEVICE_TABLES"); h->device_tables = !(e && *e && atoi(e) == 0); }
+    { const char* e = getenv("LIO_GRAPH_UPDATE"); h->graph_update = !(e && *e && atoi(e) == 0); }
     const int rc = lio_s2m_init_resources(h.get());
     if (rc != LIO_OK) return rc;
     *out = h.release();
@@ -174,7 +177,7 @@
         if (ev_end[i]) (void)hipEventDestroy(ev_end[i]);
         if (ev_chk[i]) (void)hipEventDestroy(ev_chk[i]);
     }
-    for (hipEvent_t e : { ev_map[0], ev_map[1], ev_mapl[0], ev_mapl[1] }) if (e) (void)hipEventDestroy(e);
+    for (hipEvent_t e : { ev_map[0], ev_map[1], ev_mapl[0], ev_mapl[1], ev_tab[0], ev_tab[1] }) if (e) (void)hipEventDestroy(e);
     if (graph_exec) (void)hipGraphExecDestroy(graph_exec);
     if (graph) (void)hipGraphDestroy(graph);
     if (own_stream && stream) (void)hipStreamDestroy(stream);
@@ -616,6 +619,31 @@
     return LIO_OK;
 }
 
+static int lio_tab_acquire(lio_s2m_handle* h, size_t bytes, unsigned char** out)
+{
+    const int k = h->tab_slot ^= 1;
+    if (h->ev_tab_used[k]) HIPCHK(hipEventSynchronize(h->ev_tab[k]));
+    HIPCHK(h->h_tab[k].grow(bytes, bytes + bytes / 4 + 256));
+    *out = h->h_tab[k];
+    return LIO_OK;
+}
+
+static int lio_tab_sent(lio_s2m_handle* h)
+{
+    HIPCHK(hipEventRecord(h->ev_tab[h->tab_slot], h->stream));
+    h->ev_tab_used[h->tab_slot] = true;
+    return LIO_OK;
+}
+
+static void lio_ensure_host_blocks(lio_s2m_handle* h)
+{
+    if (h->host_blocks_valid) return;
+    std::vector<int> n((size_t)h->n_scans);
+    for (int s = 0; s < h->n_scans; ++s) n[s] = h->h_state[s].n_pts;
+    lio_build_block_list(n.data(), h->n_scans, LIO_BLOCK * h->ppt, 0, 1, nullptr, h->v_blocks);
+    h->host_blocks_valid = true;
+}
+
 extern "C" int lio_s2m_batch_upload(lio_s2m_handle* h, int32_t n_scans, const void* const* scans,
                                     const size_t* n_pts, size_t stride)
 try {
@@ -633,17 +661,28 @@
     }
     if (total > 0x7fffffffull - 1024) return lio_fail(LIO_ERR_CAPACITY, "batch too large");
     h->run_pending = false;
-    if (h->host_state_stale && h->n_scans > 0 && h->d_state) {
-        HIPCHK(hipMemcpyAsync(h->h_state.data(), h->d_state, (size_t)h->n_scans * sizeof(LioScanState),
-                              hipMemcpyDeviceToHost, h->stream));
-        HIPCHK(hipStreamSynchronize(h->stream));
-    }
-    h->host_state_stale = false;
+    const bool dev = h->device_tables && h->block_world <= 1;
+    const size_t old_scans = h->h_state.size();
+    if (!dev) {
+        if (h->host_state_stale && h->n_scans > 0 && h->d_state) {
+            HIPCHK(hipMemcpyAsync(h->h_state.data(), h->d_state, (size_t)h->n_scans * sizeof(LioScanState),
+                                  hipMemcpyDeviceToHost, h->stream));
+            HIPCHK(hipStreamSynchronize(h->stream));
+        }
+        h->host_state_stale = false;
+    }
     const size_t tt = total ? total : 1;
     HIPCHK(h->d_sx.grow(tt));
     HIPCHK(h->d_sy.grow(tt));
     HIPCHK(h->d_sz.grow(tt));
     HIPCHK(h->d_stage.grow(tt * stride));
+    if (dev && h->d_state && (size_t)n_scans > h->d_state.cap && old_scans > 0) {
+        LioDevBuf<LioScanState> grown;
+        HIPCHK(grown.grow((size_t)n_scans));
+        HIPCHK(hipMemcpyAsync(grown, h->d_state, std::min(old_scans, h->d_state.cap) * sizeof(LioScanState), hipMemcpyDeviceToDevice, h->stream));
+        HIPCHK(hipStreamSynchronize(h->stream));
+        h->d_state = std::move(grown);
+    }
     HIPCHK(h->d_state.grow((size_t)n_scans));
     HIPCHK(h->d_poses.grow((size_t)n_scans * 6));
     {
@@ -660,27 +699,40 @@
     std::vector<LioBlockDesc>& blocks = h->v_blocks;
     blocks.clear();
     int max_blk = 1;
-    const size_t old_scans = h->h_state.size();
     h->h_state.resize((size_t)n_scans);
+    LioScanRow* rows = nullptr;
+    if (dev) {
+        unsigned char* slot = nullptr;
+        const int rct = lio_tab_acquire(h, (size_t)n_scans * sizeof(LioScanRow), &slot);
+        if (rct != LIO_OK) return rct;
+        rows = (LioScanRow*)slot;
+    }
+    const bool with_pose = h->reg_pose && n_scans == 1;
+    h->v_first_orig.assign((size_t)n_scans + 1, 0);
     size_t off = 0;
     for (int s = 0; s < n_scans; ++s) {
         LioScanState& st = h->h_state[s];
         if ((size_t)s >= old_scans) memset(&st, 0, sizeof(st));
         st.n_pts = (int)n_pts[s];
         st.offset = (int)off;
-        if (h->reg_pose && n_scans == 1) memcpy(st.pose, h->reg_pose, sizeof(float) * 6);
+        if (with_pose) memcpy(st.pose, h->reg_pose, sizeof(float) * 6);
         st.c_n_pts = 0;
         st.c_offset = 0;
         st.done = 1;
-        const int nb = (int)((n_pts[s] + per_blk - 1) / per_blk);
-        const int bw = h->block_world > 1 ? h->block_world : 1, br = h->block_world > 1 ? h->block_rank : 0;
-        const int part = (br + s) % bw;
-        const int b0 = (int)((long long)nb * part / bw), b1 = (int)((long long)nb * (part + 1) / bw);
+        if (rows) {
+            rows[s].n_pts = st.n_pts; rows[s].offset = st.offset;
+            if (with_pose) memcpy(rows[s].pose, h->reg_pose, sizeof(float) * 6);
+            else memset(rows[s].pose, 0, sizeof(float) * 6);
+        }
+        int b0, b1;
+        lio_block_range((long long)n_pts[s], (int)per_blk, s, h->block_rank, h->block_world, &b0, &b1);
         const int nb_local = b1 - b0;
         if (nb_local > max_blk) max_blk = nb_local;
-        for (int b = b0; b < b1; ++b) blocks.push_back({ s, (int)(b * per_blk), b - b0, nb_local });
+        h->v_first_orig[s + 1] = h->v_first_orig[s] + nb_local;
         off += n_pts[s];
     }
+    const int n_blocks = h->v_first_orig[n_scans];
+    if (!dev) lio_build_block_list(n_pts, n_scans, (int)per_blk, h->block_rank, h->block_world, nullptr, blocks);
     const unsigned char* stage = h->d_stage;
     bool host_copy = false;
     {
@@ -718,18 +770,18 @@
     h->int_off = -2;
     stage += h->xyz_off;
     h->xyz_off = 0;
-    h->v_first_orig.assign((size_t)n_scans + 1, 0);
-    for (const LioBlockDesc& b : blocks) h->v_first_orig[b.scan + 1]++;
-    for (int s = 0; s < n_scans; ++s) h->v_first_orig[s + 1] += h->v_first_orig[s];
     h->n_scans = n_scans;
     h->total_pts = total;
-    h->n_blocks = (int)blocks.size();
+    h->n_blocks = n_blocks;
     h->max_blk = max_blk;
-    HIPCHK(h->d_blocks.grow(blocks.size() ? blocks.size() : 1));
+    h->dev_tables_batch = dev;
+    h->host_blocks_valid = !dev;
+    h->blocks_from_host = !dev;
+    HIPCHK(h->d_blocks.grow(n_blocks ? (size_t)n_blocks : 1));
     HIPCHK(h->d_partials.grow((size_t)n_scans * max_blk * LIO_SUMS));
     if (h->cfg.profile == 2) {
-        HIPCHK(h->d_stamps.grow(blocks.size() * (LIO_BLOCK / 64) * 8 + 8));
-        HIPCHK(hipMemsetAsync(h->d_stamps, 0, (blocks.size() * (LIO_BLOCK / 64) * 8 + 8) * sizeof(long long), h->stream));
+        HIPCHK(h->d_stamps.grow((size_t)n_blocks * (LIO_BLOCK / 64) * 8 + 8));
+        HIPCHK(hipMemsetAsync(h->d_stamps, 0, ((size_t)n_blocks * (LIO_BLOCK / 64) * 8 + 8) * sizeof(long long), h->stream));
     }
     if (h->cfg.record_corr_iter >= 0) {
         HIPCHK(h->d_rec_flag.grow(tt));
@@ -739,11 +791,19 @@
         HIPCHK(hipMemsetAsync(h->d_rec_coeff, 0, tt * 4 * sizeof(float), h->stream));
         HIPCHK(hipMemsetAsync(h->d_rec_nn, 0xff, tt * 5 * sizeof(int), h->stream));
     }
-    if (!blocks.empty())
-        HIPCHK(hipMemcpyAsync(h->d_blocks, blocks.data(), blocks.size() * sizeof(LioBlockDesc),
+    if (dev) {
+        HIPCHK(h->d_rows.grow((size_t)n_scans));
+        HIPCHK(hipMemcpyAsync(h->d_rows, rows, (size_t)n_scans * sizeof(LioScanRow), hipMemcpyHostToDevice, h->stream));
+        { const int rct = lio_tab_sent(h); if (rct != LIO_OK) return rct; }
+        lio_launch_state_rows(h->d_state, h->d_rows, n_scans, (int)std::min(old_scans, (size_t)n_scans), with_pose, h->stream);
+        lio_launch_block_list(h->d_rows, nullptr, n_scans, (int)per_blk, 0, 1, h->d_blocks, n_blocks, h->stream);
+    } else {
+        if (!blocks.empty())
+            HIPCHK(hipMemcpyAsync(h->d_blocks, blocks.data(), blocks.size() * sizeof(LioBlockDesc),
+                                  hipMemcpyHostToDevice, h->stream));
+        HIPCHK(hipMemcpyAsync(h->d_state, h->h_state.data(), (size_t)n_scans * sizeof(LioScanState),
                               hipMemcpyHostToDevice, h->stream));
-    HIPCHK(hipMemcpyAsync(h->d_state, h->h_state.data(), (size_t)n_scans * sizeof(LioScanState),
-                          hipMemcpyHostToDevice, h->stream));
+    }
     std::vector<LioScanTiles>& tiles = h->v_tiles;
     std::vector<LioBlockDesc>& prep = h->v_prep;
     tiles.clear(); prep.clear();
@@ -819,10 +879,10 @@
         else lio_launch_aos_to_soa(stage, stride, (int)total, h->d_sx, h->d_sy, h->d_sz, nullptr, h->stream);
     }
     h->has_block_box = false;
-    if (h->shard.axis >= 0 && ppt == 1 && !blocks.empty()) {
+    if (h->shard.axis >= 0 && ppt == 1 && n_blocks > 0) {
         HIPCHK(h->d_block_box.grow((tt / LIO_BLOCK + (size_t)n_scans + 2) * 6));
-        HIPCHK(h->d_blk_skip.grow(blocks.size()));
-        lio_launch_block_boxes(h->d_blocks, (int)blocks.size(), h->d_state, h->d_sx, h->d_sy, h->d_sz, h->d_block_box, h->stream);
+        HIPCHK(h->d_blk_skip.grow((size_t)n_blocks));
+        lio_launch_block_boxes(h->d_blocks, n_blocks, h->d_state, h->d_sx, h->d_sy, h->d_sz, h->d_block_box, h->stream);
         h->has_block_box = true;
     }
     if (!h->defer_sync) HIPCHK(hipStreamSynchronize(h->stream));
@@ -868,9 +928,13 @@
     ch->block_rank = h->block_rank;
     ch->block_world = h->block_world;
     ch->defer_sync = h->defer_sync;
+    ch->device_tables = h->device_tables;
     int rc = lio_s2m_batch_upload(ch, n_scans, scans, n_pts, stride);
     ch->defer_sync = false;
     if (rc != LIO_OK) return rc;
+    lio_ensure_host_blocks(h);
+    lio_ensure_host_blocks(ch);
+    h->blocks_from_host = ch->blocks_from_host = true;
     int max_blk = 1;
     for (LioBlockDesc& b : h->v_blocks) {
         const int ns = h->v_first_orig[b.scan + 1] - h->v_first_orig[b.scan];
@@ -893,12 +957,22 @@
     if (!ch->v_blocks.empty())
         HIPCHK(hipMemcpyAsync(ch->d_blocks, ch->v_blocks.data(), ch->v_blocks.size() * sizeof(LioBlockDesc),
                               hipMemcpyHostToDevice, h->stream));
+    if (!h->dev_tables_batch && h->host_state_stale) {
+        HIPCHK(hipMemcpyAsync(h->h_state.data(), h->d_state, (size_t)n_scans * sizeof(LioScanState), hipMemcpyDeviceToHost, h->stream));
+        HIPCHK(hipStreamSynchronize(h->stream));
+        h->host_state_stale = false;
+    }
     for (int s = 0; s < n_scans; ++s) {
         h->h_state[s].c_n_pts = ch->h_state[s].n_pts;
         h->h_state[s].c_offset = ch->h_state[s].offset;
     }
-    HIPCHK(hipMemcpyAsync(h->d_state, h->h_state.data(), (size_t)n_scans * sizeof(LioScanState),
-                          hipMemcpyHostToDevice, h->stream));
+    if (h->dev_tables_batch && ch->dev_tables_batch)
+        lio_launch_state_corner_rows(h->d_state, ch->d_rows, n_scans, h->stream);
+    else if (!h->dev_tables_batch)
+        HIPCHK(hipMemcpyAsync(h->d_state, h->h_state.data(), (size_t)n_scans * sizeof(LioScanState),
+                              hipMemcpyHostToDevice, h->stream));
+    else
+        return lio_fail(LIO_ERR_ARG, "the corner batch was not uploaded with the device tables of its surf batch");
     if (!h->defer_sync) HIPCHK(hipStreamSynchronize(h->stream));
     h->corner_active = true;
     h->poses_set = false;
@@ -923,8 +997,18 @@
     (void)hipGetLastError();
     h->run_pending = false;
     h->pose_in_state = false;
-    HIPCHK(hipMemcpyAsync(h->d_poses, poses, (size_t)h->n_scans * 6 * sizeof(float), hipMemcpyHostToDevice, h->stream));
-    if (h->cfg.sort_batch && h->n_scans > 8 && !h->v_blocks.empty()) {
+    const bool reorder = h->cfg.sort_batch && h->n_scans > 8 && h->n_blocks > 0;
+    const size_t pose_bytes = (size_t)h->n_scans * 6 * sizeof(float);
+    unsigned char* slot = nullptr;
+    if (h->dev_tables_batch) {
+        const int rct = lio_tab_acquire(h, pose_bytes + (size_t)h->n_scans * sizeof(int), &slot);
+        if (rct != LIO_OK) return rct;
+        memcpy(slot, poses, pose_bytes);
+        HIPCHK(hipMemcpyAsync(h->d_poses, slot, pose_bytes, hipMemcpyHostToDevice, h->stream));
+    } else {
+        HIPCHK(hipMemcpyAsync(h->d_poses, poses, pose_bytes, hipMemcpyHostToDevice, h->stream));
+    }
+    if (reorder) {
         const LioGrid& mg = lio_map_of(h)->grid;
         const float ext[3] = { (float)mg.nx, (float)mg.ny, (float)mg.nz };
         const int ax = (ext[0] >= ext[1] && ext[0] >= ext[2]) ? 0 : (ext[1] >= ext[2] ? 1 : 2);
@@ -933,19 +1017,24 @@
         for (int s = 0; s < h->n_scans; ++s) order[s] = s;
         std::stable_sort(order.begin(), order.end(),
                          [&](int a, int b) { return poses[a * 6 + 3 + ax] < poses[b * 6 + 3 + ax]; });
-        std::vector<int>& first = h->v_first;
-        first.assign((size_t)h->n_scans + 1, 0);
-        for (const LioBlockDesc& b : h->v_blocks) first[b.scan + 1]++;
-        for (int s = 0; s < h->n_scans; ++s) first[s + 1] += first[s];
-        std::vector<LioBlockDesc>& sorted = h->v_blocks_sorted;
-        sorted.clear();
-        sorted.reserve(h->v_blocks.size());
-        for (int k = 0; k < h->n_scans; ++k) {
-            const int s = order[k];
-            for (int i = h->v_first_orig[s]; i < h->v_first_orig[s + 1]; ++i) sorted.push_back(h->v_blocks[i]);
-        }
-        HIPCHK(hipMemcpyAsync(h->d_blocks, sorted.data(), sorted.size() * sizeof(LioBlockDesc), hipMemcpyHostToDevice, h->stream));
-    }
+        if (h->dev_tables_batch && !h->blocks_from_host) {
+            memcpy(slot + pose_bytes, order.data(), (size_t)h->n_scans * sizeof(int));
+            HIPCHK(h->d_order.grow((size_t)h->n_scans));
+            HIPCHK(hipMemcpyAsync(h->d_order, slot + pose_bytes, (size_t)h->n_scans * sizeof(int), hipMemcpyHostToDevice, h->stream));
+            lio_launch_block_list(h->d_rows, h->d_order, h->n_scans, LIO_BLOCK * h->ppt, 0, 1, h->d_blocks, h->n_blocks, h->stream);
+        } else {
+            lio_ensure_host_blocks(h);
+            std::vector<LioBlockDesc>& sorted = h->v_blocks_sorted;
+            sorted.clear();
+            sorted.reserve(h->v_blocks.size());
+            for (int k = 0; k < h->n_scans; ++k) {
+                const int s = order[k];
+                for (int i = h->v_first_orig[s]; i < h->v_first_orig[s + 1]; ++i) sorted.push_back(h->v_blocks[i]);
+            }
+            HIPCHK(hipMemcpyAsync(h->d_blocks, sorted.data(), sorted.size() * sizeof(LioBlockDesc), hipMemcpyHostToDevice, h->stream));
+        }
+    }
+    if (slot) { const int rct = lio_tab_sent(h); if (rct != LIO_OK) return rct; }
     if (!h->defer_sync) HIPCHK(hipStreamSynchronize(h->stream));
     h->poses_set = true;
     return LIO_OK;
@@ -1056,16 +1145,69 @@
         memcmp(&h->graph_params, &P, sizeof(P)) == 0 && h->graph_blocks_c == nbc &&
         (!Pc || memcmp(&h->graph_params_c, Pc, sizeof(P)) == 0))
         return LIO_OK;
+    const int variant = lio_iterate_variant(P, h->ppt, h->cfg.use_lds != 0, false, h->plain_kernel && !Pc);
+    const bool stage = h->cfg.use_lds != 0;
+    if (h->graph_update && h->graph_exec && !h->graph_nodes.empty() && h->graph_chunk == chunk && h->graph_ppt == h->ppt &&
+        h->graph_plain == h->plain_kernel && h->graph_tail_from == h->tail_from && h->graph_tail_wgs == h->tail_wgs &&
+        h->graph_variant == variant && h->graph_stage == stage && (h->graph_blocks_c >= 0) == (Pc != nullptr)) {
+        if (h->graph_last_launch) HIPCHK(hipEventSynchronize(h->graph_last_launch));
+        bool ok = true;
+        int nb = h->n_blocks;
+        for (const lio_s2m_handle::GraphNode& g : h->graph_nodes) {
+            hipKernelNodeParams kp;
+            memset(&kp, 0, sizeof(kp));
+            if (hipGraphKernelNodeGetParams(g.node, &kp) != hipSuccess) { ok = false; break; }
+            void* args[2] = { (void*)(g.form == 2 ? Pc : &P), (void*)&nb };
+            kp.kernelParams = args;
+            kp.extra = nullptr;
+            kp.gridDim = dim3(g.form == 2 ? h->corner->n_blocks : (g.form == 1 ? lio_tail_grid(h->n_blocks, h->tail_wgs) : h->n_blocks));
+            if (hipGraphExecKernelNodeSetParams(h->graph_exec, g.node, &kp) != hipSuccess) { ok = false; break; }
+        }
+        if (ok) {
+            h->graph_blocks = h->n_blocks; h->graph_blocks_c = nbc;
+            memcpy(&h->graph_params, &P, sizeof(P));
+            if (Pc) memcpy(&h->graph_params_c, Pc, sizeof(P));
+            h->graph_dirty = false;
+            h->graph_updated++;
+            return LIO_OK;
+        }
+        (void)hipGetLastError();
+    }
+    h->graph_nodes.clear();
     if (h->graph_exec) { HIPCHK(hipGraphExecDestroy(h->graph_exec)); h->graph_exec = nullptr; }
     if (h->graph) { HIPCHK(hipGraphDestroy(h->graph)); h->graph = nullptr; }
     HIPCHK(hipStreamBeginCapture(h->stream, hipStreamCaptureModeThreadLocal));
     h->graph_n_full = h->graph_n_looped = 0;
+    std::vector<int> forms;
     for (int i = 0; i < chunk; ++i) {
-        if (lio_launch_gn(h, P, Pc, i)) h->graph_n_looped++;
-        else h->graph_n_full++;
+        if (Pc) forms.push_back(2);
+        if (lio_launch_gn(h, P, Pc, i)) { h->graph_n_looped++; forms.push_back(1); }
+        else { h->graph_n_full++; forms.push_back(0); }
     }
     HIPCHK(hipStreamEndCapture(h->stream, &h->graph));
     HIPCHK(hipGraphInstantiate(&h->graph_exec, h->graph, nullptr, nullptr, 0));
+    h->graph_instantiated++;
+    if (h->graph_update) {
+        hipGraphNode_t node = nullptr;
+        size_t n = 0;
+        bool ok = hipGraphGetRootNodes(h->graph, nullptr, &n) == hipSuccess && n == 1;
+        if (ok) ok = hipGraphGetRootNodes(h->graph, &node, &n) == hipSuccess && n == 1;
+        while (ok) {
+            hipGraphNodeType ty;
+            ok = hipGraphNodeGetType(node, &ty) == hipSuccess && ty == hipGraphNodeTypeKernel && h->graph_nodes.size() < forms.size();
+            if (!ok) break;
+            h->graph_nodes.push_back({ node, forms[h->graph_nodes.size()] });
+            n = 0;
+            ok = hipGraphNodeGetDependentNodes(node, nullptr, &n) == hipSuccess && n <= 1;
+            if (!ok || n == 0) break;
+            hipGraphNode_t next = nullptr;
+            ok = hipGraphNodeGetDependentNodes(node, &next, &n) == hipSuccess && n == 1 && next;
+            node = next;
+        }
+        if (!ok || h->graph_nodes.size() != forms.size()) h->graph_nodes.clear();
+        (void)hipGetLastError();
+    }
+    h->graph_variant = variant; h->graph_stage = stage;
     h->graph_chunk = chunk; h->graph_blocks = h->n_blocks; h->graph_ppt = h->ppt; h->graph_plain = h->plain_kernel;
     h->graph_tail_from = h->tail_from; h->graph_tail_wgs = h->tail_wgs;
     memcpy(&h->graph_params, &P, sizeof(P));
@@ -1106,6 +1248,7 @@
         if (prof) HIPCHK(hipEventRecord(h->ev_end[u], h->stream));
         if (!h->run_persist) HIPCHK(hipMemcpyAsync(&h->h_active[u], h->d_active, sizeof(int), hipMemcpyDeviceToHost, h->stream));
         HIPCHK(hipEventRecord(h->ev_chk[u], h->stream));
+        if (h->run_graph) h->graph_last_launch = h->ev_chk[u];
         h->run_next = u + 1;
         h->units_this_run = u + 1;
         h->launches_this_run = (u + 1) * h->unit_iters;
@@ -1175,6 +1318,50 @@
     *n_full = h->multi ? 0 : h->run_n_full;
     *n_looped = h->multi ? 0 : h->run_n_looped;
     return LIO_OK;
+} LIO_CATCH
+
+extern "C" int lio_s2m_graph_stats(const lio_s2m_handle* h, int32_t* n_instantiated, int32_t* n_updated)
+try {
+    if (!h || !n_instantiated || !n_updated) return lio_fail(LIO_ERR_ARG, "null argument");
+    *n_instantiated = h->multi ? 0 : h->graph_instantiated;
+    *n_updated = h->multi ? 0 : h->graph_updated;
+    return LIO_OK;
+} LIO_CATCH
+
+extern "C" int lio_s2m_debug_tables(lio_s2m_handle* h, int32_t* blocks_out, size_t cap_blocks, int32_t* state_fields_out)
+try {
+    if (!h) return lio_fail(LIO_ERR_ARG, "null handle");
+    if (h->multi) return lio_fail(LIO_ERR_ARG, "not available on a multi-device handle");
+    if (h->n_scans < 1 || !h->d_state) return lio_fail(LIO_ERR_ARG, "no batch uploaded");
+    HIPCHK(hipSetDevice(h->cfg.device_id));
+    (void)hipGetLastError();
+    const size_t nb = std::min((size_t)h->n_blocks, cap_blocks);
+    if (blocks_out && nb)
+        HIPCHK(hipMemcpyAsync(blocks_out, h->d_blocks, nb * sizeof(LioBlockDesc), hipMemcpyDeviceToHost, h->stream));
+    std::vector<LioScanState> st;
+    if (state_fields_out) {
+        st.resize((size_t)h->n_scans);
+        HIPCHK(hipMemcpyAsync(st.data(), h->d_state, st.size() * sizeof(LioScanState), hipMemcpyDeviceToHost, h->stream));
+    }
+    HIPCHK(hipStreamSynchronize(h->stream));
+    for (size_t s = 0; s < st.size(); ++s) {
+        const int32_t f[6] = { st[s].n_pts, st[s].offset, st[s].c_n_pts, st[s].c_offset, st[s].done, st[s].is_degenerate };
+        memcpy(state_fields_out + s * 6, f, sizeof(f));
+    }
+    return h->n_blocks;
+} LIO_CATCH
+
+extern "C" int lio_debug_block_list(const int32_t* n_pts, int32_t n_scans, int32_t per_blk, int32_t rank, int32_t world, const int32_t* order,
+                                    int32_t* blocks_out, size_t cap_blocks, int32_t* max_blk)
+try {
+    if (!n_pts || n_scans < 1 || per_blk < 1) return lio_fail(LIO_ERR_ARG, "need scans and a positive workgroup size");
+    for (int s = 0; s < n_scans; ++s)
+        if (n_pts[s] < 0 || (order && (order[s] < 0 || order[s] >= n_scans))) return lio_fail(LIO_ERR_ARG, "negative length or order out of range");
+    std::vector<LioBlockDesc> v;
+    const int mb = lio_build_block_list(n_pts, n_scans, per_blk, rank, world, order, v);
+    if (max_blk) *max_blk = mb;
+    if (blocks_out) memcpy(blocks_out, v.data(), std::min(v.size(), cap_blocks) * sizeof(LioBlockDesc));
+    return (int)v.size();
 } LIO_CATCH
 
 extern "C" int lio_s2m_batch_iter_partial(lio_s2m_handle* h, double* d_sums)
```

Result: no change. 480,000, median of 6 (+0.5%).
